# QuantumLiquids/PEPS

Measured on NVIDIA B200. Metric: vmc_samples_per_s, higher is better.
Workload: dtype f64

## Files before the change

### include/peps_b200.h

```cpp
#ifndef PEPS_B200_H
#define PEPS_B200_H
#include <stddef.h>
#include <stdint.h>

#ifdef __cplusplus
extern "C" {
#endif

typedef struct peps_ctx peps_ctx;

typedef struct {
  int32_t rows, cols;
  int32_t phys;
  int32_t D;
  int32_t walkers;
  int32_t device;
  int32_t dmin, dmax;
  double trunc_err;
} peps_config;

const char *peps_backend_name(void);

int peps_create(peps_ctx **out, const peps_config *cfg);
void peps_destroy(peps_ctx *ctx);
const char *peps_last_error(peps_ctx *ctx);

size_t peps_tps_size(peps_ctx *ctx);
size_t peps_tps_site_offset(peps_ctx *ctx, int32_t row, int32_t col);
int peps_set_tps(peps_ctx *ctx, const double *host_tps, size_t n);
int peps_get_tps(peps_ctx *ctx, double *host_tps, size_t n);
int peps_set_truncation(peps_ctx *ctx, int32_t dmin, int32_t dmax, double trunc_err);
int peps_set_compress_scheme(peps_ctx *ctx, int32_t scheme, double convergence_tol, int32_t iter_max);
int peps_set_jacobi(peps_ctx *ctx, double tol, int32_t inner_sweeps, int32_t max_sweeps);
int peps_set_deflation(peps_ctx *ctx, double eps);
int peps_set_chain_deflation(peps_ctx *ctx, double eps);
int peps_set_model_xxz(peps_ctx *ctx, double jz, double jxy, double pinning00);
int peps_set_model_j1j2_xxz(peps_ctx *ctx, double jz, double jxy, double jz2, double jxy2, double pinning00);
int peps_set_model_tfim(peps_ctx *ctx, double h);

int peps_set_model_term(peps_ctx *ctx, int32_t kind, int32_t T, const double *diag, const int32_t *target, const double *coef);
int peps_clear_model_terms(peps_ctx *ctx);
int peps_set_bond_pin(peps_ctx *ctx, int32_t site1, int32_t site2, int32_t T, const double *diag, const int32_t *target, const double *coef);

int peps_set_fermion(peps_ctx *ctx, const int32_t *phys_par, const int32_t *leg_par, size_t n_leg_par);

int peps_set_complex(peps_ctx *ctx);
int peps_set_tps_c(peps_ctx *ctx, const double *re, const double *im, size_t n);
int peps_get_planar(peps_ctx *ctx, int32_t what, double *re, double *im);

int peps_set_jastrow(peps_ctx *ctx, const double *v, const int32_t *density);
int peps_clear_jastrow(peps_ctx *ctx);

int peps_set_configs(peps_ctx *ctx, const int32_t *cfg);
int peps_get_configs(peps_ctx *ctx, int32_t *cfg);
int peps_seed_rng(peps_ctx *ctx, const uint32_t *seeds);
int peps_set_rng_state(peps_ctx *ctx, const uint32_t *mt, const int32_t *idx);
int peps_get_rng_state(peps_ctx *ctx, uint32_t *mt, int32_t *idx);

int peps_init_walkers(peps_ctx *ctx);
int peps_get_amplitudes(peps_ctx *ctx, double *amp);
int peps_normalize_state_order1(peps_ctx *ctx, double max_abs_override, double *site_factor_out);

int peps_sweep(peps_ctx *ctx, int32_t nsweeps, double *accept_rates);
int peps_sweep_full_space(peps_ctx *ctx, int32_t nsweeps, double *accept_rates);
int peps_sweep_three_site(peps_ctx *ctx, int32_t nsweeps, double *accept_rates);
int peps_set_updater(peps_ctx *ctx, int32_t kind);
int peps_energy_and_holes(peps_ctx *ctx, int32_t calc_holes, double *eloc, double *psi_list);
int peps_measure(peps_ctx *ctx, double *energy, double *e_h, double *e_v, double *e_dr, double *e_ur, double *row_corr);
int peps_measure_bond_term(peps_ctx *ctx, int32_t T, const double *diag, const int32_t *target, const double *coef, double *out_h, double *out_v);
int peps_measure_site_term(peps_ctx *ctx, int32_t T, const double *diag, const int32_t *target, const double *coef, double *out);
int64_t peps_structure_factor_pairs(peps_ctx *ctx);
int peps_measure_structure_factor(peps_ctx *ctx, double *out);
size_t peps_holes_stride(peps_ctx *ctx);
int peps_get_holes(peps_ctx *ctx, double *holes);

int peps_zero_accumulators(peps_ctx *ctx);
int peps_accumulate_ostar(peps_ctx *ctx);
int peps_get_accumulators(peps_ctx *ctx, double *ostar_sum, double *eloc_ostar_sum, size_t n);
double *peps_ostar_sum_device(peps_ctx *ctx);
double *peps_eloc_ostar_sum_device(peps_ctx *ctx);
int peps_sample(peps_ctx *ctx, int32_t sweeps_between_samples, double *eloc, double *accept_rates);

int peps_sr_reserve(peps_ctx *ctx, int64_t max_walker_samples);
int peps_sr_collect(peps_ctx *ctx, int32_t on);
int peps_sr_clear(peps_ctx *ctx);
int64_t peps_sr_count(peps_ctx *ctx);
int peps_sr_matvec(peps_ctx *ctx, const double *v_host, double mean_dot_v, double *out_host, size_t n);
int peps_sr_matvec_device(peps_ctx *ctx, const double *v_dev, double mean_dot_v, double *out_dev);
int peps_sr_matvec_c(peps_ctx *ctx, const double *v_host, double mean_dot_v_re, double mean_dot_v_im, double *out_host, size_t n);

typedef int (*peps_allreduce_fn)(void *user, double *device_buf, size_t n);
typedef struct {
  int32_t max_iter;
  double relative_tolerance, absolute_tolerance;
  int32_t residual_recompute_interval;
  double orthogonality_threshold;
} peps_cg_params;
int peps_sr_natural_gradient(peps_ctx *ctx, const double *gradient, const double *ostar_mean, int64_t total_samples,
                             double diag_shift, const peps_cg_params *params, const double *init_guess,
                             peps_allreduce_fn allreduce, void *user, double *x_out, int32_t *iterations,
                             double *residual_norm, int32_t *reason);

int peps_sr_minsr_natural_gradient(peps_ctx *ctx, int64_t total_samples, double diag_shift, double *x_out, double *energy_mean_out);
int peps_sr_minsr_tmatrix(peps_ctx *ctx, double *t_out, size_t n);
int peps_sr_minsr_gram_diag(peps_ctx *ctx, double *g_out, size_t n);

int peps_probe_trace_row(peps_ctx *ctx, int32_t row, double *psi);
int peps_probe_tnn_trace(peps_ctx *ctx, int32_t row, int32_t col, int32_t orient, const int32_t *cfg3, double *psi);
int peps_probe_plaquette_trace(peps_ctx *ctx, int32_t kind, int32_t row, int32_t col, int32_t dir, int32_t orient, double *psi);
int32_t peps_bmps_stack_size(peps_ctx *ctx, int32_t position);
int peps_get_bmps_tensor(peps_ctx *ctx, int32_t position, int32_t k, int32_t i, double *out, int32_t dims[3]);
int64_t peps_stat(peps_ctx *ctx, int32_t which);
int peps_profile_enable(peps_ctx *ctx, int32_t on);
int peps_profile_get(peps_ctx *ctx, double *ms, int64_t *launches, double *flops, int32_t reset);
int peps_sync(peps_ctx *ctx);
void *peps_stream(peps_ctx *ctx);

int peps_test_qr_r(int32_t device, int32_t W, int32_t m, int32_t n, const double *a, double *r_out);
int peps_test_truncate(int32_t device, int32_t W, int32_t nr, int32_t nc, int32_t dmin, int32_t dmax, double trunc_err,
                       const double *theta, double *b_out, int32_t *kept_out, int32_t *sweeps_out);
int peps_test_einsum(int32_t device, int32_t W, const char *spec, const int32_t *dims_a, int32_t rank_a,
                     const int32_t *dims_b, int32_t rank_b, const double *a, const double *b, double *c);

#ifdef __cplusplus
}
#endif
#endif
```

### peps_b200/_lib.py

```python
import ctypes as C
import os

HERE = os.path.dirname(os.path.abspath(__file__))
LIB_PATH = os.path.join(HERE, "libpeps_b200.so")


class PepsConfig(C.Structure):
    _fields_ = [("rows", C.c_int32), ("cols", C.c_int32), ("phys", C.c_int32), ("D", C.c_int32),
                ("walkers", C.c_int32), ("device", C.c_int32), ("dmin", C.c_int32), ("dmax", C.c_int32),
                ("trunc_err", C.c_double)]


class PepsCGParams(C.Structure):
    _fields_ = [("max_iter", C.c_int32), ("relative_tolerance", C.c_double), ("absolute_tolerance", C.c_double),
                ("residual_recompute_interval", C.c_int32), ("orthogonality_threshold", C.c_double)]


ALLREDUCE_FN = C.CFUNCTYPE(C.c_int, C.c_void_p, C.c_void_p, C.c_size_t)

_P = C.c_void_p
_D = C.POINTER(C.c_double)
_I = C.POINTER(C.c_int32)
_U = C.POINTER(C.c_uint32)

SIGNATURES = {
    "peps_backend_name": (C.c_char_p, []),
    "peps_create": (C.c_int, [C.POINTER(_P), C.POINTER(PepsConfig)]),
    "peps_destroy": (None, [_P]),
    "peps_last_error": (C.c_char_p, [_P]),
    "peps_tps_size": (C.c_size_t, [_P]),
    "peps_tps_site_offset": (C.c_size_t, [_P, C.c_int32, C.c_int32]),
    "peps_set_tps": (C.c_int, [_P, _D, C.c_size_t]),
    "peps_get_tps": (C.c_int, [_P, _D, C.c_size_t]),
    "peps_set_truncation": (C.c_int, [_P, C.c_int32, C.c_int32, C.c_double]),
    "peps_set_compress_scheme": (C.c_int, [_P, C.c_int32, C.c_double, C.c_int32]),
    "peps_set_jacobi": (C.c_int, [_P, C.c_double, C.c_int32, C.c_int32]),
    "peps_set_deflation": (C.c_int, [_P, C.c_double]),
    "peps_set_model_xxz": (C.c_int, [_P, C.c_double, C.c_double, C.c_double]),
    "peps_set_chain_deflation": (C.c_int, [_P, C.c_double]),
    "peps_set_model_j1j2_xxz": (C.c_int, [_P, C.c_double, C.c_double, C.c_double, C.c_double, C.c_double]),
    "peps_set_model_term": (C.c_int, [_P, C.c_int32, C.c_int32, _D, _I, _D]),
    "peps_clear_model_terms": (C.c_int, [_P]),
    "peps_set_bond_pin": (C.c_int, [_P, C.c_int32, C.c_int32, C.c_int32, _D, _I, _D]),
    "peps_measure_bond_term": (C.c_int, [_P, C.c_int32, _D, _I, _D, _D, _D]),
    "peps_measure_site_term": (C.c_int, [_P, C.c_int32, _D, _I, _D, _D]),
    "peps_set_fermion": (C.c_int, [_P, _I, _I, C.c_size_t]),
    "peps_set_jastrow": (C.c_int, [_P, _D, _I]),
    "peps_set_complex": (C.c_int, [_P]),
    "peps_set_tps_c": (C.c_int, [_P, _D, _D, C.c_size_t]),
    "peps_get_planar": (C.c_int, [_P, C.c_int32, _D, _D]),
    "peps_clear_jastrow": (C.c_int, [_P]),
    "peps_set_configs": (C.c_int, [_P, _I]),
    "peps_get_configs": (C.c_int, [_P, _I]),
    "peps_seed_rng": (C.c_int, [_P, _U]),
    "peps_set_rng_state": (C.c_int, [_P, _U, _I]),
    "peps_get_rng_state": (C.c_int, [_P, _U, _I]),
    "peps_init_walkers": (C.c_int, [_P]),
    "peps_get_amplitudes": (C.c_int, [_P, _D]),
    "peps_normalize_state_order1": (C.c_int, [_P, C.c_double, _D]),
    "peps_sweep": (C.c_int, [_P, C.c_int32, _D]),
    "peps_sweep_full_space": (C.c_int, [_P, C.c_int32, _D]),
    "peps_sweep_three_site": (C.c_int, [_P, C.c_int32, _D]),
    "peps_measure": (C.c_int, [_P, _D, _D, _D, _D, _D, _D]),
    "peps_set_updater": (C.c_int, [_P, C.c_int32]),
    "peps_set_model_tfim": (C.c_int, [_P, C.c_double]),
    "peps_energy_and_holes": (C.c_int, [_P, C.c_int32, _D, _D]),
    "peps_structure_factor_pairs": (C.c_int64, [_P]),
    "peps_measure_structure_factor": (C.c_int, [_P, _D]),
    "peps_holes_stride": (C.c_size_t, [_P]),
    "peps_get_holes": (C.c_int, [_P, _D]),
    "peps_zero_accumulators": (C.c_int, [_P]),
    "peps_accumulate_ostar": (C.c_int, [_P]),
    "peps_get_accumulators": (C.c_int, [_P, _D, _D, C.c_size_t]),
    "peps_ostar_sum_device": (C.c_void_p, [_P]),
    "peps_eloc_ostar_sum_device": (C.c_void_p, [_P]),
    "peps_sample": (C.c_int, [_P, C.c_int32, _D, _D]),
    "peps_sr_reserve": (C.c_int, [_P, C.c_int64]),
    "peps_sr_collect": (C.c_int, [_P, C.c_int32]),
    "peps_sr_clear": (C.c_int, [_P]),
    "peps_sr_count": (C.c_int64, [_P]),
    "peps_sr_matvec": (C.c_int, [_P, _D, C.c_double, _D, C.c_size_t]),
    "peps_sr_matvec_device": (C.c_int, [_P, C.c_void_p, C.c_double, C.c_void_p]),
    "peps_sr_matvec_c": (C.c_int, [_P, _D, C.c_double, C.c_double, _D, C.c_size_t]),
    "peps_sr_natural_gradient": (C.c_int, [_P, _D, _D, C.c_int64, C.c_double, C.POINTER(PepsCGParams), _D, ALLREDUCE_FN,
                                           C.c_void_p, _D, C.POINTER(C.c_int32), _D, C.POINTER(C.c_int32)]),
    "peps_sr_minsr_natural_gradient": (C.c_int, [_P, C.c_int64, C.c_double, _D, _D]),
    "peps_sr_minsr_tmatrix": (C.c_int, [_P, _D, C.c_size_t]),
    "peps_sr_minsr_gram_diag": (C.c_int, [_P, _D, C.c_size_t]),
    "peps_probe_trace_row": (C.c_int, [_P, C.c_int32, _D]),
    "peps_probe_tnn_trace": (C.c_int, [_P, C.c_int32, C.c_int32, C.c_int32, _I, _D]),
    "peps_probe_plaquette_trace": (C.c_int, [_P, C.c_int32, C.c_int32, C.c_int32, C.c_int32, C.c_int32, _D]),
    "peps_bmps_stack_size": (C.c_int32, [_P, C.c_int32]),
    "peps_get_bmps_tensor": (C.c_int, [_P, C.c_int32, C.c_int32, C.c_int32, _D, _I]),
    "peps_stat": (C.c_int64, [_P, C.c_int32]),
    "peps_sync": (C.c_int, [_P]),
    "peps_profile_enable": (C.c_int, [_P, C.c_int32]),
    "peps_profile_get": (C.c_int, [_P, _D, C.POINTER(C.c_int64), _D, C.c_int32]),
    "peps_stream": (C.c_void_p, [_P]),
    "peps_test_qr_r": (C.c_int, [C.c_int32, C.c_int32, C.c_int32, C.c_int32, _D, _D]),
    "peps_test_truncate": (C.c_int, [C.c_int32, C.c_int32, C.c_int32, C.c_int32, C.c_int32, C.c_int32, C.c_double,
                                     _D, _D, _I, _I]),
    "peps_test_einsum": (C.c_int, [C.c_int32, C.c_int32, C.c_char_p, _I, C.c_int32, _I, C.c_int32, _D, _D, _D]),
}


def bind(path):
    lib = C.CDLL(path)
    for name, (res, args) in SIGNATURES.items():
        fn = getattr(lib, name)
        fn.restype = res
        fn.argtypes = args
    return lib


_lib = None


def load():
    global _lib
    if _lib is None:
        if not os.path.exists(LIB_PATH):
            from . import build as _build
            _build.build_cuda()
        _lib = bind(LIB_PATH)
    return _lib
```

### peps_b200/csrc/backend.h

```cpp
#pragma once
#include <cstddef>
#include <cstdint>

namespace peps {

struct Operand {
  double *p = nullptr;
  long ws = 0;
  long bs = 0;
  const int32_t *gidx = nullptr;
  int gws = 0;
  long gs = 0;
};
inline Operand mkop(double *p, long ws, long bs = 0) {
  Operand o; o.p = p; o.ws = ws; o.bs = bs; return o;
}
inline Operand mkgather(double *p, const int32_t *gidx, int gws, long gs) {
  Operand o; o.p = p; o.gidx = gidx; o.gws = gws; o.gs = gs; return o;
}

struct GettDesc {
  int M = 0, N = 0, K = 0;
  const int32_t *am = nullptr, *ak = nullptr, *bk = nullptr, *bn = nullptr, *cm = nullptr, *cn = nullptr;
  int a_kfast = 0;
  int b_nfast = 1;
  int a_vec2 = 0, b_vec2 = 0, c_vec2 = 0;
  const int32_t *klo_m = nullptr, *klo_n = nullptr;
  double work = 1.0;
  const int32_t *m_cnt = nullptr, *n_cnt = nullptr;
  int m_scale = 0, n_scale = 0;
};

struct BeCtx;
BeCtx *be_ctx_create(int device);
void be_ctx_bind(BeCtx *c);
void be_ctx_destroy(BeCtx *c);
void be_init(int device);
const char *be_name();
void *be_malloc(size_t bytes);
void be_free(void *p);
void be_memset0(void *p, size_t bytes);
void be_h2d(void *dst, const void *src, size_t bytes);
void be_d2h(void *dst, const void *src, size_t bytes);
void be_d2d(void *dst, const void *src, size_t bytes);
void be_sync();
void *be_stream();
long be_launch_count();

enum KernelClass { KC_GETT = 0, KC_DOT, KC_PANEL, KC_JACOBI, KC_SMALL, KC_APPLY, KC_COUNT };
void be_profile_enable(int on);
void be_profile_collect(double *ms, long *launches, double *flops, int reset);

void be_gett(const GettDesc &d, Operand A, Operand B, Operand C, double alpha, double beta, int W, int NB);
void be_dot(int K, const int32_t *ak, const int32_t *bk, Operand A, Operand B, double *out, int W);

void be_fill(double *p, double v, long n);
void be_copy2d(double *dst, long wd, long ldd, const double *src, long ws, long lds, int rows, int cols, int W);
void be_set_identity(double *dst, long wd, int rows, int cols, int W);

struct PanelArgs {
  double *A; long ws; int lda;
  const int32_t *rowtab; int R; int skip0; int NI;
  int col0, pw, nbw;
  double *Vw, *Tw;
  int W;
  const int32_t *row_cnt = nullptr;
  int row_scale = 0;
  const int32_t *stopped = nullptr;
};
void be_panel_qr(const PanelArgs &a);
void be_trailing_check(const double *A, long ws, int lda, int row0, int nrows, int col0, int ncols, const double *colnorm2,
                       const int32_t *colorder, int n, double thresh2, double *acc, int32_t *stopped, int W);

struct TileMap { alignas(64) unsigned char blob[128]; };
bool be_make_tile_map(TileMap *tm, const double *A, long ws, int lda, int rows, int cols, int W, int box_rows, int box_cols);
struct ApplyArgs {
  double *A; long ws; int lda;
  const int32_t *rowtab; int R; int NI;
  int col1, ntrail, nbw;
  const double *Vw, *Tw;
  int W;
  const TileMap *tmap = nullptr;
  int row0 = 0;
  const TileMap *tmap_cols = nullptr;
  int notrans = 0;
  const int32_t *row_cnt = nullptr;
  int row_scale = 0;
  const int32_t *stopped = nullptr;
};
void be_apply_reflector(const ApplyArgs &a);

struct JacobiArgs {
  double *G; long ws; int ld; int nr_pad; int nc; int bs; int nblk; int round;
  double tol; int inner_sweeps; double *offmax; const int32_t *done; int W;
  int nactive = 0;
  const int32_t *bsec = nullptr;
  const int32_t *cwin = nullptr;
};
void be_jacobi_round(const JacobiArgs &a);
void be_jacobi_flags(double *offmax, int32_t *done, double tol, int W);
void be_sector_arrange(const double *src, long ws, int ld, int nc, const int32_t *count, int bs, int nblk, double *dst, long wd,
                       int32_t *bsec, const int32_t *cord_in, int32_t *cord_out, int32_t *cwin, int W);
void be_col_norms2(const double *G, long ws, int ld, int nr, int nc, double *norms2, int W);
void be_permute_cols(const double *src, long ws, int lds, int nr, int nc, const int32_t *order, int gather,
                     double *dst, long wd, int ldd, int W);
void be_row_norms2(const double *G, long ws, int ld, int nr, int nc, double *norms2, int W);
void be_rank_rows(const double *norms2, int nr, double defl2, int32_t *order, int32_t *count, int W);
void be_gather_rows(const double *src, long ws, int ld, int nc, int nr_src, const int32_t *order, const int32_t *count,
                    double *dst, long wd, int nr_dst, int W);
void be_select_truncate(const double *norms2, int nr, int nsv, int dmin, int dmax, double trunc_err, int tcap,
                        int32_t *order, int32_t *kept, int W);
void be_gather_rows_normalized(const double *G, long ws, int ld, int nc, const double *norms2, int nr,
                               const int32_t *order, const int32_t *kept, int tcap, double *B, long wb, int W);

void be_gather_rows_transposed(const double *src, long ws, int ld, int nc, int nr_src, const int32_t *order,
                               const int32_t *count, double *dst, long wd, int n2, int W);
struct SmallSvdArgs {
  const double *Rt; long ws; int ld; int n2; const int32_t *count;
  int nsv, dmin, dmax; double trunc_err; int tcap;
  double tol; int max_sweeps;
  double *out; long wo; int32_t *kept; int32_t *sweeps; int W;
};
constexpr int kSmallSvdMaxN = 128;
void be_svd_small(const SmallSvdArgs &a);
void be_transpose_permute(const double *C0, long wc, int nc, int tcap, const int32_t *order, double *B, long wb, int W);

void be_mt_seed(uint32_t *mt, int32_t *idx, const uint32_t *seeds, int W);
void be_nn_exchange_decide(int32_t *cfg, int nsites, int s1, int s2, const double *psi_b, double *amp,
                           uint32_t *mt, int32_t *idx, int32_t *accepted, int W, const double *jastrow = nullptr);
void be_jastrow_ratio(const int32_t *cfg, int nsites, int s1, int s2, const int32_t *dens, const double *v, double *ratio, int W);
void be_scale(double *x, const double *s, int W);
void be_xxz_bond_energy(const int32_t *cfg, int nsites, int s1, int s2, const double *psi_ex, const double *psi,
                        double jz, double jxy, double *eloc, int W);
void be_ratio_accumulate(const double *psi_ex, const double *psi, double coef, double *eloc, int W);
void be_xxz_onsite_energy(const int32_t *cfg, int nsites, double h00, double *eloc, int W);
void be_term_targets(const int32_t *cfg, int nsites, int s1, int s2, int phys, const int32_t *target, const double *coef, int T,
                     int t, int32_t *idx_a, int32_t *idx_b, double *coefw, int W);
void be_term_accumulate(const int32_t *cfg, int nsites, int s1, int s2, int phys, const double *diag, const double *coefw,
                        const double *psi_ex, const double *psi, double *eloc, int W);

void be_embed_complex(const double *Ar, const double *Ai, long wa, int m, int n, double *M, long wm, int W);
void be_split_r(const double *R, long wr, int rows, int n, double *outr, double *outi, long wo, int W);
void be_complex_basis(double *Bm, long wb, int tcap2, int n, const int32_t *kept2, double *Br, double *Bi, long wo, int tcap,
                      int32_t *keptc, int W);
void be_complex_combine(const double *d0, const double *d1, const double *d2, const double *d3, double *outr, double *outi, int W);
void be_nn_exchange_decide_c(int32_t *cfg, int nsites, int s1, int s2, const double *pbr, const double *pbi, double *ampr,
                             double *ampi, uint32_t *mt, int32_t *idx, int32_t *accepted, int W, const double *jastrow = nullptr);
void be_xxz_bond_energy_c(const int32_t *cfg, int nsites, int s1, int s2, const double *exr, const double *exi, const double *pr,
                          const double *pi, double jz, double jxy, double *er, double *ei, int W);
void be_ratio_accumulate_c(const double *exr, const double *exi, const double *pr, const double *pi, double coef, double *er,
                           double *ei, int W);
void be_term_accumulate_c(const int32_t *cfg, int nsites, int s1, int s2, int phys, const double *diag, const double *coefw,
                          const double *exr, const double *exi, const double *pr, const double *pi, double *er, double *ei, int W);
void be_accumulate_ostar_c(const double *hr, const double *hi, long hole_stride, const int32_t *hole_off, const int32_t *site_size,
                           const int32_t *tps_off, const int32_t *cfg, int nsites, const double *ampr, const double *ampi,
                           const double *er, const double *ei, double *osr, double *osi, double *eor, double *eoi, int W);

constexpr int FERMION_VARIANTS = 8;
void be_fermion_gather(const int32_t *cfg, int rows, int cols, int phys, const int32_t *phys_par, int32_t *gidx_h,
                       int32_t *gidx_v, int32_t *jw_h, int32_t *jw_v, int W);
#if defined(__CUDACC__)
#define PEPS_HD __host__ __device__
#else
#define PEPS_HD
#endif
PEPS_HD inline void fermion_target_one(const int32_t *c, const int32_t *jh, const int32_t *jv, int s1, int s2, int phys,
                                       const int32_t *par, int kind, const int32_t *target, const double *coef, int T, int t,
                                       int32_t &idx_a, int32_t &idx_b, double &coefw) {
  const int c1 = c[s1], c2 = c[s2], p = c1 * phys + c2;
  int tg;
  double cf;
  if (target) { tg = target[p * T + t]; cf = tg < 0 ? 0.0 : coef[p * T + t]; }
  else { tg = c1 != c2 ? c2 * phys + c1 : -1; cf = tg < 0 ? 0.0 : 1.0; }
  const int n1 = tg < 0 ? c1 : tg / phys, n2 = tg < 0 ? c2 : tg % phys;
  const int moved = (par[c1] ^ par[n1]) & (par[c2] ^ par[n2]);
  int va, vb, neg = 0;
  if (kind == 1) { va = 6 + jv[s1]; vb = 6 + (jv[s2] ^ moved); }
  else if (kind == 0 || !moved) { va = jh[s1]; vb = jh[s2] ^ moved; }
  else if (kind == 2) { va = 2 + jh[s1]; vb = jh[s2] ^ 1; neg = jh[s2]; }
  else { va = jh[s1]; vb = 4 + jh[s2]; neg = jh[s1]; }
  idx_a = va * phys + n1;
  idx_b = vb * phys + n2;
  coefw = neg ? -cf : cf;
}
void be_fermion_targets(const int32_t *cfg, int nsites, int s1, int s2, int phys, const int32_t *phys_par,
                        const int32_t *jw_h, const int32_t *jw_v, int kind, const int32_t *target, const double *coef,
                        int T, int t, int32_t *idx_a, int32_t *idx_b, double *coefw, int W);
void be_fermion_finish_holes(double *holes, long hole_stride, const int32_t *hole_off, const int32_t *site_size,
                             const double *gtps, const int64_t *gtps_off, const int32_t *gidx_h, const int32_t *jw_h,
                             int nsites, const double *sign, const double *amp, int W);

void be_fermion_finish_holes_c(double *hr, double *hi, long hole_stride, const int32_t *hole_off, const int32_t *site_size,
                               const double *gtps, long gtps_im_off, const int64_t *gtps_off, const int32_t *gidx_h,
                               const int32_t *jw_h, int nsites, const double *sign, const double *ampr, const double *ampi, int W);

void be_accumulate_ostar(const double *holes, long hole_stride, const int32_t *hole_off, const int32_t *site_size,
                         const int32_t *tps_off, const int32_t *cfg, int nsites, int phys, const double *amp,
                         const double *eloc, double *osum, double *eosum, int W);

void be_sr_store(const double *holes, long hole_stride, const double *amp, const int32_t *cfg, int nsites,
                 double *ostar, int32_t *cfgs, long first, int W);
void be_sr_store_c(const double *hr, const double *hi, long hole_stride, const double *ampr, const double *ampi, const int32_t *cfg,
                   int nsites, double *ostar, int32_t *cfgs, long first, long cap, int W);
void be_sr_dots(const double *ostar, const int32_t *cfgs, long hole_stride, const int32_t *hole_off,
                const int32_t *site_size, const int32_t *tps_off, int nsites, const double *v, double mean_dot_v,
                double *delta, long n);
void be_sr_accumulate(const double *ostar, const int32_t *cfgs, long hole_stride, const int32_t *hole_off,
                      const int32_t *site_size, const int32_t *tps_off, int nsites, int phys, const double *delta,
                      double *out, long n);

void be_sr_gram(const double *left, const double *right, const int32_t *cfgs, long hole_stride, const int32_t *hole_off,
                const int32_t *site_size, const int32_t *site_size_host, int nsites, long n, double lower_sign, double *G);
void be_minsr_centre(const double *G, const double *a, double c, double sign, long n, double scale, double *T);
void be_minsr_embed(const double *Tr, const double *Ti, long n, double shift, double *M);
void be_chol(double *M, long m, int32_t *info);
void be_chol_solve(const double *L, long m, double *b);


void be_vec_lincomb(double *out, double ca, const double *a, double cb, const double *b, long n);
void be_vec_dot(const double *a, const double *b, long n, double *result);

}
```

### peps_b200/csrc/backend_cuda.cu

```cuda
#include <cuda.h>
#include <cuda_runtime.h>
#include <cstdint>
#include <cstdio>
#include <cstdlib>
#include <cmath>
#include <stdexcept>
#include <algorithm>
#include <string>
#include <type_traits>
#include <unordered_map>
#include <map>
#include <mutex>
#include <utility>
#include <vector>
#include "backend.h"

namespace peps {

#define CUDA_CHECK(x)                                                                              \
  do {                                                                                             \
    cudaError_t e_ = (x);                                                                          \
    if (e_ != cudaSuccess)                                                                         \
      throw std::runtime_error(std::string("CUDA error: ") + cudaGetErrorString(e_) + " at " +     \
                               __FILE__ + ":" + std::to_string(__LINE__));                         \
  } while (0)

struct Profiler {
  bool on = false;
  std::vector<std::pair<cudaEvent_t, cudaEvent_t>> pending[KC_COUNT];
  std::vector<cudaEvent_t> pool;
  double ms[KC_COUNT] = {0}, flops[KC_COUNT] = {0};
  long launches[KC_COUNT] = {0};
  cudaEvent_t get() {
    if (!pool.empty()) { cudaEvent_t e = pool.back(); pool.pop_back(); return e; }
    cudaEvent_t e;
    CUDA_CHECK(cudaEventCreate(&e));
    return e;
  }
};
struct BeCtx {
  int device = 0;
  cudaStream_t stream = nullptr;
  long launches = 0;
  Profiler prof;
  double *dot_part = nullptr;
  double *vdot_part = nullptr;
  size_t dot_part_cap = 0;
  double *gram_part = nullptr;
  size_t gram_part_cap = 0;
  int32_t *gram_split = nullptr;
  int gram_split_cap = 0;
};
static thread_local BeCtx *g_cx = nullptr;
static thread_local int g_cur_device = -1;
static inline BeCtx &cx() {
  if (!g_cx) throw std::runtime_error("peps_b200: no backend context bound to this thread");
  return *g_cx;
}
#define g_stream (cx().stream)
#define g_prof (cx().prof)

BeCtx *be_ctx_create(int device) {
  int n = 0;
  cudaError_t e = cudaGetDeviceCount(&n);
  if (e != cudaSuccess || n == 0)
    throw std::runtime_error("peps_b200: no CUDA device available; the product has no CPU fallback");
  if (device < 0 || device >= n) throw std::invalid_argument("peps_b200: CUDA device ordinal out of range");
  CUDA_CHECK(cudaSetDevice(device));
  g_cur_device = device;
  BeCtx *c = new BeCtx();
  c->device = device;
  cudaError_t se = cudaStreamCreateWithFlags(&c->stream, cudaStreamNonBlocking);
  if (se != cudaSuccess) { delete c; throw std::runtime_error(std::string("CUDA error: ") + cudaGetErrorString(se)); }
  return c;
}
void be_ctx_bind(BeCtx *c) {
  if (c && g_cur_device != c->device) { CUDA_CHECK(cudaSetDevice(c->device)); g_cur_device = c->device; }
  g_cx = c;
}
void be_ctx_destroy(BeCtx *c) {
  if (!c) return;
  if (g_cur_device != c->device) { cudaSetDevice(c->device); g_cur_device = c->device; }
  cudaStreamSynchronize(c->stream);
  for (int k = 0; k < KC_COUNT; ++k)
    for (auto &pr : c->prof.pending[k]) { cudaEventDestroy(pr.first); cudaEventDestroy(pr.second); }
  for (cudaEvent_t ev : c->prof.pool) cudaEventDestroy(ev);
  if (c->dot_part) cudaFree(c->dot_part);
  if (c->vdot_part) cudaFree(c->vdot_part);
  if (c->gram_part) cudaFree(c->gram_part);
  if (c->gram_split) cudaFree(c->gram_split);
  cudaStreamDestroy(c->stream);
  if (g_cx == c) g_cx = nullptr;
  delete c;
}
void be_init(int device) {
  static thread_local std::unordered_map<int, BeCtx *> defaults;
  auto it = defaults.find(device);
  if (it == defaults.end()) it = defaults.emplace(device, be_ctx_create(device)).first;
  be_ctx_bind(it->second);
}

static inline void post_launch() {
  ++cx().launches;
  cudaError_t e = cudaGetLastError();
  if (e != cudaSuccess) throw std::runtime_error(std::string("kernel launch failed: ") + cudaGetErrorString(e));
}
template <class K>
static inline void ensure_smem(K kern, size_t smem) {
  static std::mutex mu;
  static std::map<std::pair<int, const void *>, size_t> table;
  std::lock_guard<std::mutex> lock(mu);
  size_t &have = table[{cx().device, (const void *)kern}];
  if (smem > have) {
    CUDA_CHECK(cudaFuncSetAttribute(kern, cudaFuncAttributeMaxDynamicSharedMemorySize, (int)smem));
    have = smem;
  }
}

struct LaunchScope {
  int c; cudaEvent_t s = nullptr;
  LaunchScope(int cls, double fl) : c(cls) {
    g_prof.launches[c] += 1;
    g_prof.flops[c] += fl;
    if (g_prof.on) { s = g_prof.get(); cudaEventRecord(s, g_stream); }
  }
  ~LaunchScope() {
    if (s) { cudaEvent_t e = g_prof.get(); cudaEventRecord(e, g_stream); g_prof.pending[c].push_back({s, e}); }
  }
};
void be_profile_enable(int on) { g_prof.on = on != 0; }
void be_profile_collect(double *ms, long *launches, double *flops, int reset) {
  CUDA_CHECK(cudaStreamSynchronize(g_stream));
  for (int c = 0; c < KC_COUNT; ++c) {
    for (auto &pr : g_prof.pending[c]) {
      float t = 0.f;
      cudaEventElapsedTime(&t, pr.first, pr.second);
      g_prof.ms[c] += t;
      g_prof.pool.push_back(pr.first);
      g_prof.pool.push_back(pr.second);
    }
    g_prof.pending[c].clear();
    if (ms) ms[c] = g_prof.ms[c];
    if (launches) launches[c] = g_prof.launches[c];
    if (flops) flops[c] = g_prof.flops[c];
    if (reset) { g_prof.ms[c] = 0; g_prof.launches[c] = 0; g_prof.flops[c] = 0; }
  }
}

const char *be_name() { return "cuda-sm_100a"; }
void *be_malloc(size_t bytes) {
  void *p = nullptr;
  CUDA_CHECK(cudaMalloc(&p, bytes ? bytes : 8));
  return p;
}
// ... 370 lines not shown
          if (beta != 0.0) v1 += beta * (*cq);
          *cq = v1;
        }
      }
    }
  }
}

static inline bool op_aligned2(const Operand &o) {
  return ((reinterpret_cast<uintptr_t>(o.p) & 15) == 0) && ((o.ws & 1) == 0) && ((o.bs & 1) == 0) && (o.gidx == nullptr || (o.gs & 1) == 0);
}

void be_gett(const GettDesc &d, Operand A, Operand B, Operand C, double alpha, double beta, int W, int NB) {
  if (d.M <= 0 || d.N <= 0 || W <= 0 || NB <= 0) return;
  LaunchScope scope(KC_GETT, 2.0 * d.M * d.N * d.K * (double)W * NB * d.work);
  static const bool use_large = []() { const char *e = std::getenv("PEPS_GETT_LARGE"); return e ? std::atoi(e) != 0 : true; }();
  if (use_large && d.M > 32 && d.N > 32 && d.K >= 8) {
    const int avec = d.a_vec2 && op_aligned2(A), bvec = d.b_vec2 && op_aligned2(B), cvec = d.c_vec2 && op_aligned2(C);
    const int tn = (d.N + GL_BN - 1) / GL_BN;
    const long ctas128 = (long)((d.M + 127) / 128) * tn * NB * W;
    const bool half = ctas128 < 2L * 148 || d.M <= 96;
    const int bm = half ? 64 : 128;
    dim3 grid(((d.M + bm - 1) / bm) * tn, NB, W);
    const bool akf = d.a_kfast != 0, bkf = d.b_nfast == 0;
    const size_t smem = gl_smem(bm, akf, bkf);
    auto go = [&](auto kern) {
      ensure_smem(kern, smem);
      kern<<<grid, GL_THREADS, smem, g_stream>>>(d, A, B, C, alpha, beta, avec, bvec, cvec);
    };
    if (half) {
      if (akf && bkf) go(gett_large_kernel<true, true, 2>);
      else if (akf) go(gett_large_kernel<true, false, 2>);
      else if (bkf) go(gett_large_kernel<false, true, 2>);
      else go(gett_large_kernel<false, false, 2>);
    } else {
      if (akf && bkf) go(gett_large_kernel<true, true, 4>);
      else if (akf) go(gett_large_kernel<true, false, 4>);
      else if (bkf) go(gett_large_kernel<false, true, 4>);
      else go(gett_large_kernel<false, false, 4>);
    }
    post_launch();
    return;
  }
  auto launch = [&](auto kern, int BM, int BN) {
    int tiles = ((d.M + BM - 1) / BM) * ((d.N + BN - 1) / BN);
    dim3 grid(tiles, NB, W);
    kern<<<grid, GETT_THREADS, 0, g_stream>>>(d, A, B, C, alpha, beta);
    post_launch();
  };
  if (d.M > 32 && d.N > 32) launch(gett_kernel<4, 4>, 64, 64);
  else if (d.M > 32) launch(gett_kernel<4, 1>, 64, 16);
  else if (d.N > 32) launch(gett_kernel<1, 4>, 64 / 4, 64);
  else launch(gett_kernel<2, 2>, 32, 32);
}

__global__ void dot_kernel(int K, int kchunk, const int32_t *ak, const int32_t *bk, Operand A, Operand B, double *part) {
  const int w = blockIdx.x, sidx = blockIdx.y;
  const double *Ab = operand_base(A, w, 0);
  const double *Bb = operand_base(B, w, 0);
  __shared__ double red[256];
  double s = 0.0;
  const int k1 = min(K, (sidx + 1) * kchunk);
  for (int k = sidx * kchunk + threadIdx.x; k < k1; k += blockDim.x) s += Ab[ak[k]] * Bb[bk[k]];
  red[threadIdx.x] = s;
  __syncthreads();
  for (int h = blockDim.x / 2; h > 0; h >>= 1) {
    if (threadIdx.x < h) red[threadIdx.x] += red[threadIdx.x + h];
    __syncthreads();
  }
  if (threadIdx.x == 0) part[(long)w * gridDim.y + sidx] = red[0];
}
__global__ void dot_finish_kernel(const double *part, int nsplit, double *out, int W) {
  const int w = blockIdx.x * blockDim.x + threadIdx.x;
  if (w >= W) return;
  double s = 0.0;
  for (int i = 0; i < nsplit; ++i) s += part[(long)w * nsplit + i];
  out[w] = s;
}
void be_dot(int K, const int32_t *ak, const int32_t *bk, Operand A, Operand B, double *out, int W) {
  LaunchScope scope(KC_DOT, 2.0 * K * W);
  const int nsplit = std::max(1, std::min(32, K / 4096));
  if (nsplit == 1) {
    dot_kernel<<<dim3(W, 1), 256, 0, g_stream>>>(K, K, ak, bk, A, B, out);
    post_launch();
    return;
  }
  double *&part = cx().dot_part;
  size_t &part_cap = cx().dot_part_cap;
  if ((size_t)W * 32 > part_cap) {
    if (part) { CUDA_CHECK(cudaStreamSynchronize(g_stream)); cudaFree(part); }
    part_cap = (size_t)W * 32;
    CUDA_CHECK(cudaMalloc(&part, sizeof(double) * part_cap));
  }
  const int kchunk = (K + nsplit - 1) / nsplit;
  dot_kernel<<<dim3(W, nsplit), 256, 0, g_stream>>>(K, kchunk, ak, bk, A, B, part);
  ++cx().launches;
  dot_finish_kernel<<<(W + 127) / 128, 128, 0, g_stream>>>(part, nsplit, out, W);
  post_launch();
}

__global__ void fill_kernel(double *p, double v, long n) {
  long i = blockIdx.x * (long)blockDim.x + threadIdx.x;
  long stride = (long)gridDim.x * blockDim.x;
  for (; i < n; i += stride) p[i] = v;
}
void be_fill(double *p, double v, long n) {
  if (n <= 0) return;
  int blocks = (int)((n + 255) / 256 < 148L * 8 ? (n + 255) / 256 : 148L * 8);
  LaunchScope scope(KC_SMALL, 0.0);
  fill_kernel<<<blocks, 256, 0, g_stream>>>(p, v, n);
  post_launch();
}
__global__ void copy2d_kernel(double *dst, long wd, long ldd, const double *src, long ws, long lds, int rows,
                              int cols) {
  const int w = blockIdx.y;
  long n = (long)rows * cols;
  for (long i = blockIdx.x * (long)blockDim.x + threadIdx.x; i < n; i += (long)gridDim.x * blockDim.x) {
    int r = (int)(i / cols), c = (int)(i % cols);
    dst[w * wd + r * ldd + c] = src[w * ws + r * lds + c];
  }
}
void be_copy2d(double *dst, long wd, long ldd, const double *src, long ws, long lds, int rows, int cols, int W) {
  long n = (long)rows * cols;
  if (n <= 0) return;
  int bx = (int)((n + 255) / 256 < 64 ? (n + 255) / 256 : 64);
  LaunchScope scope(KC_SMALL, 0.0);
  copy2d_kernel<<<dim3(bx, W), 256, 0, g_stream>>>(dst, wd, ldd, src, ws, lds, rows, cols);
  post_launch();
}
__global__ void identity_kernel(double *dst, long wd, int rows, int cols) {
  const int w = blockIdx.y;
  long n = (long)rows * cols;
  for (long i = blockIdx.x * (long)blockDim.x + threadIdx.x; i < n; i += (long)gridDim.x * blockDim.x) {
    int r = (int)(i / cols), c = (int)(i % cols);
    dst[w * wd + i] = (r == c) ? 1.0 : 0.0;
  }
}
void be_set_identity(double *dst, long wd, int rows, int cols, int W) {
  long n = (long)rows * cols;
  int bx = (int)((n + 255) / 256 < 64 ? (n + 255) / 256 : 64);
  LaunchScope scope(KC_SMALL, 0.0);
  identity_kernel<<<dim3(bx, W), 256, 0, g_stream>>>(dst, wd, rows, cols);
  post_launch();
}

__device__ __forceinline__ double warp_sum(double v) {
#pragma unroll
  for (int o = 16; o > 0; o >>= 1) v += __shfl_xor_sync(0xffffffffu, v, o);
  return v;
}

constexpr int PQR_THREADS = 256;

__global__ void __launch_bounds__(PQR_THREADS) panel_qr_kernel(PanelArgs a) {
  extern __shared__ double sm[];
  const int it = blockIdx.x, w = blockIdx.y;
  if (a.row_cnt && a.rowtab[(long)it * a.R] >= a.row_cnt[w] * a.row_scale) return;
  if (a.stopped && a.stopped[w]) return;
  const int R = a.R, pw = a.pw, nbw = a.nbw;
  const int skip = (it == 0) ? a.skip0 : 0;
  const int nact = R - skip;
  const int LDP = R + 1;
  double *P = sm;
  double *S = P + (size_t)nbw * LDP;
  double *T = S + nbw * nbw;
  double *tau = T + nbw * nbw;
  double *scal = tau + nbw;
  double *beta = scal + nbw;
  const int t = threadIdx.x, lane = t & 31, warp = t >> 5, nwarp = PQR_THREADS / 32;
  double *Aw = a.A + (long)w * a.ws;
  const int32_t *rows = a.rowtab + (long)it * R;

  for (int e = t; e < nact * pw; e += PQR_THREADS) {
    int r = e / pw, c = e % pw;
    P[c * LDP + r] = Aw[(long)rows[skip + r] * a.lda + a.col0 + c];
  }
  __syncthreads();

  for (int j = 0; j < pw; ++j) {
    double tj = 0.0, sj = 0.0, bj = 0.0;
    if (j < nact) {
      const double *x = P + j * LDP;
      double part = 0.0;
      for (int r = j + 1 + lane; r < nact; r += 32) part += x[r] * x[r];
      double xn2 = warp_sum(part);
      double alpha = x[j];
      bj = alpha;
      if (xn2 > 0.0) {
        double nrm = sqrt(alpha * alpha + xn2);
        bj = (alpha >= 0.0) ? -nrm : nrm;
        tj = (bj - alpha) / bj;
        sj = 1.0 / (alpha - bj);
      }
      if (tj != 0.0) {
        for (int c = j + 1 + warp; c < pw; c += nwarp) {
          double *y = P + c * LDP;
          double pr = 0.0;
          for (int r = j + 1 + lane; r < nact; r += 32) pr += x[r] * y[r];
          double wv = warp_sum(pr) * sj + y[j];
          double f = tj * wv;
          for (int r = j + 1 + lane; r < nact; r += 32) y[r] -= f * sj * x[r];
          if (lane == 0) y[j] -= f;
        }
      }
    }
    if (t == 0) { tau[j] = tj; scal[j] = sj; beta[j] = bj; }
    __syncthreads();
  }

  for (int e = t; e < nbw * nbw; e += PQR_THREADS) {
    int r = e / nbw, c = e % nbw;
    double v = 0.0;
    if (c < pw && r <= c && r < nact) v = (r == c) ? beta[c] : P[c * LDP + r];
    T[e] = v;
  }
  __syncthreads();
  for (int e = t; e < nact * pw; e += PQR_THREADS) {
    int r = e / pw, c = e % pw;
    double v = (r < nbw && r <= c) ? T[r * nbw + c] : 0.0;
    Aw[(long)rows[skip + r] * a.lda + a.col0 + c] = v;
  }
  __syncthreads();
  for (int e = t; e < nact * pw; e += PQR_THREADS) {
    int c = e / nact, r = e % nact;
    double v;
    if (r < c) v = 0.0;
    else if (r == c) v = 1.0;
    else v = P[c * LDP + r] * scal[c];
    P[c * LDP + r] = v;
  }
  __syncthreads();
  for (int pidx = warp; pidx < pw * pw; pidx += nwarp) {
    int ca = pidx / pw, cb = pidx % pw;
    if (ca >= cb) continue;
    const double *x = P + ca * LDP, *y = P + cb * LDP;
    double pr = 0.0;
    for (int r = cb + lane; r < nact; r += 32) pr += x[r] * y[r];
    pr = warp_sum(pr);
    if (lane == 0) S[ca * nbw + cb] = pr;
  }
  __syncthreads();
  for (int e = t; e < nbw * nbw; e += PQR_THREADS) T[e] = 0.0;
  __syncthreads();
  if (warp == 0) {
    for (int j = 0; j < pw; ++j) {
      double tj = tau[j];
      double v = 0.0;
      if (lane < j) {
        for (int b2 = lane; b2 < j; ++b2) v += T[lane * nbw + b2] * S[b2 * nbw + j];
        v *= -tj;
      }
      __syncwarp();
      if (lane < j) T[lane * nbw + j] = v;
      if (lane == j) T[j * nbw + j] = tj;
      __syncwarp();
    }
  }
  __syncthreads();
  double *Vo = a.Vw + ((long)w * a.NI + it) * (long)R * nbw;
  double *To = a.Tw + ((long)w * a.NI + it) * (long)nbw * nbw;
  for (int e = t; e < skip * nbw; e += PQR_THREADS) Vo[e] = 0.0;
  for (int e = t; e < nact * nbw; e += PQR_THREADS) {
    int r = e / nbw, c = e % nbw;
    Vo[(long)(skip + r) * nbw + c] = (c < pw) ? P[c * LDP + r] : 0.0;
  }
  for (int e = t; e < nbw * nbw; e += PQR_THREADS) To[e] = T[e];
}

static size_t panel_smem_bytes(int R, int nbw) {
  return ((size_t)nbw * (R + 1) + 2 * (size_t)nbw * nbw + 3 * nbw) * sizeof(double);
}

#ifdef PEPS_KERNEL_CLOCKS
__device__ long long g_panel_clk[8 + 32 * 8];
#define PANEL_CLK(i) do { if (blockIdx.x == 0 && blockIdx.y == 0 && threadIdx.x == 0) g_panel_clk[i] = clock64(); } while (0)
#define COL_CLK(j, k) do { if (blockIdx.x == 0 && blockIdx.y == 0 && lane == 0) g_panel_clk[8 + (j) * 8 + (k)] = clock64(); } while (0)
#else
#define PANEL_CLK(i) do { } while (0)
#define COL_CLK(j, k) do { } while (0)
#endif
template <int NBW, int RPL, int MINB>
__global__ void __launch_bounds__(PQR_THREADS, MINB) panel_qr_reg_kernel(PanelArgs a) {
  extern __shared__ double sm[];
  PANEL_CLK(0);
  constexpr int CPW = NBW / 8;
  constexpr int LDT = NBW + 1, LDSS = NBW + 1;
  constexpr int RP = RPL * 32;
  const int it = blockIdx.x, w = blockIdx.y;
  if (a.row_cnt && a.rowtab[(long)it * a.R] >= a.row_cnt[w] * a.row_scale) return;
  if (a.stopped && a.stopped[w]) return;
  const int R = a.R, pw = a.pw, nbw = a.nbw;
  const int skip = (it == 0) ? a.skip0 : 0;
  const int nact = R - skip;
  double *vcols = sm;
  double *S = vcols + (size_t)NBW * RP;
  double *Tt = S + NBW * LDSS;
  volatile double *tau_s = Tt + NBW * LDT;
  double *Rd = const_cast<double *>(tau_s) + NBW;
  long *roff = reinterpret_cast<long *>(Rd + NBW);
  volatile int *ready = reinterpret_cast<volatile int *>(roff + RP);
  const int t = threadIdx.x, lane = t & 31, warp = t >> 5;
  double *Aw = a.A + (long)w * a.ws;
  const int32_t *rows = a.rowtab + (long)it * R;
  for (int r = t; r < RP; r += PQR_THREADS) roff[r] = (r < nact) ? (long)rows[skip + r] * a.lda + a.col0 : 0;
  for (int e = t; e < NBW * LDSS; e += PQR_THREADS) S[e] = 0.0;
  for (int e = t; e < NBW * LDT; e += PQR_THREADS) Tt[e] = 0.0;
  if (t < NBW) { tau_s[t] = 0.0; Rd[t] = 0.0; ready[t] = 0; }
  __syncthreads();

  double *stage = vcols;
  constexpr int RPI = 32 / NBW;
  for (int r0 = warp * RPI; r0 < RP; r0 += 8 * RPI) {
    const int r = r0 + lane / NBW, c = lane % NBW;
    double *dstp = stage + (size_t)r * NBW + (c ^ (r & (NBW - 1)));
    if (r < nact && c < pw) {
      const unsigned saddr = (unsigned)__cvta_generic_to_shared(dstp);
      asm volatile("cp.async.ca.shared.global [%0], [%1], 8;\n" ::"r"(saddr), "l"(Aw + roff[r] + c));
    } else {
      *dstp = 0.0;
    }
  }
  asm volatile("cp.async.commit_group;\n" ::);
  asm volatile("cp.async.wait_group 0;\n" ::);
  __syncthreads();
  double P[CPW][RPL];
#pragma unroll
  for (int i = 0; i < RPL; ++i) {
    const int r = lane + 32 * i;
#pragma unroll
    for (int cc = 0; cc < CPW; ++cc) P[cc][i] = stage[(size_t)r * NBW + ((warp + 8 * cc) ^ (r & (NBW - 1)))];
  }
  __syncthreads();

  auto build = [&](int j, auto cj_c) {
    constexpr int CJ = decltype(cj_c)::value;
    double *vb = vcols + (size_t)j * RP;
    double n0 = 0.0, n1 = 0.0, n2 = 0.0, n3 = 0.0, alpha = 0.0;
#pragma unroll
    for (int i = 0; i < RPL; ++i) {
      const double v = P[CJ][i];
      const int r = lane + 32 * i;
      alpha = (r == j) ? v : alpha;
      const double vm = (r > j) ? v : 0.0;
      if ((i & 3) == 0) n0 = fma(vm, vm, n0); else if ((i & 3) == 1) n1 = fma(vm, vm, n1);
      else if ((i & 3) == 2) n2 = fma(vm, vm, n2); else n3 = fma(vm, vm, n3);
    }
    double xn2 = (n0 + n1) + (n2 + n3);
#pragma unroll
    for (int o = 16; o > 0; o >>= 1) {
      xn2 += __shfl_xor_sync(0xffffffffu, xn2, o);
      alpha += __shfl_xor_sync(0xffffffffu, alpha, o);
    }
    COL_CLK(j, 3);
    double bj = alpha, tj = 0.0, sj = 0.0;
    if (xn2 > 0.0) {
      const double s2 = alpha * alpha + xn2;
      const double rs = rsqrt(s2);
      const double nrm = s2 * rs;
      bj = (alpha >= 0.0) ? -nrm : nrm;
      const double inv_b = (alpha >= 0.0) ? -rs : rs;
      tj = 1.0 - alpha * inv_b;
      sj = 1.0 / (alpha - bj);
    }
    COL_CLK(j, 4);
#pragma unroll
    for (int i = 0; i < RPL; ++i) {
      const int r = lane + 32 * i;
      const double pm = P[CJ][i] * sj;
      const double v = (r > j) ? pm : ((r == j) ? 1.0 : 0.0);
      vb[r] = v;
      P[CJ][i] = (r >= j) ? v : P[CJ][i];
    }
    if (lane == 0) { tau_s[j] = tj; Rd[j] = bj; }
    COL_CLK(j, 5);
    __syncwarp();
    __threadfence_block();
    if (lane == 0) ready[j] = 1;
  };
  auto lookahead = [&](int jn, const double (&v)[RPL], double tj, auto cn_c) {
    constexpr int CN = decltype(cn_c)::value;
    double d0 = 0.0, d1 = 0.0, d2 = 0.0, d3 = 0.0;
#pragma unroll
    for (int i = 0; i < RPL; ++i) {
      const double q = v[i] * P[CN][i];
      if ((i & 3) == 0) d0 += q; else if ((i & 3) == 1) d1 += q; else if ((i & 3) == 2) d2 += q; else d3 += q;
    }
    const double f = tj * warp_sum((d0 + d1) + (d2 + d3));
    COL_CLK(jn, 1);
#pragma unroll
    for (int i = 0; i < RPL; ++i) P[CN][i] -= f * v[i];
    COL_CLK(jn, 2);
    build(jn, cn_c);
    COL_CLK(jn, 6);
  };

  PANEL_CLK(1);
  if (warp == 0 && pw > 0) build(0, std::integral_constant<int, 0>{});
  for (int j = 0; j < pw; ++j) {
    while (ready[j] == 0) __nanosleep(40);
    __threadfence_block();
    const double *vb = vcols + (size_t)j * RP;
    const double tj = tau_s[j];
    double v[RPL];
#pragma unroll
    for (int i = 0; i < RPL; ++i) v[i] = vb[lane + 32 * i];
    const int jn = j + 1;
    const bool own_next = (jn < pw) && (warp == (jn & 7));
    if (own_next) {
      COL_CLK(jn, 7);
      switch (jn >> 3) {
        case 0: lookahead(jn, v, tj, std::integral_constant<int, 0>{}); break;
        case 1: if constexpr (CPW > 1) lookahead(jn, v, tj, std::integral_constant<int, 1>{}); break;
        case 2: if constexpr (CPW > 2) lookahead(jn, v, tj, std::integral_constant<int, 2>{}); break;
        default: if constexpr (CPW > 3) lookahead(jn, v, tj, std::integral_constant<int, 3>{}); break;
      }
    }
    double d[CPW][2];
#pragma unroll
    for (int cc = 0; cc < CPW; ++cc) d[cc][0] = d[cc][1] = 0.0;
#pragma unroll
    for (int i = 0; i < RPL; ++i) {
#pragma unroll
      for (int cc = 0; cc < CPW; ++cc) d[cc][i & 1] += v[i] * P[cc][i];
    }
    double dot[CPW];
#pragma unroll
    for (int cc = 0; cc < CPW; ++cc) dot[cc] = d[cc][0] + d[cc][1];
#pragma unroll
    for (int o = 16; o > 0; o >>= 1) {
#pragma unroll
      for (int cc = 0; cc < CPW; ++cc) dot[cc] += __shfl_xor_sync(0xffffffffu, dot[cc], o);
    }
#pragma unroll
    for (int cc = 0; cc < CPW; ++cc) {
      const int c = warp + 8 * cc;
      if (c >= pw || c == j || (own_next && c == jn)) continue;
      if (c > j) {
        const double f = tj * dot[cc];
        if (f != 0.0) {
#pragma unroll
          for (int i = 0; i < RPL; ++i) P[cc][i] -= f * v[i];
        }
      } else if (lane == 0) {
// ... 2 lines not shown
    }
  }
  PANEL_CLK(2);
  __syncthreads();
  PANEL_CLK(3);

  {
    if (warp < NBW / 8 && lane < 8) {
      const int base = warp * 8;
      double trow[8];
#pragma unroll
      for (int j = 0; j < 8; ++j) {
        const double tj = (base + j < pw) ? tau_s[base + j] : 0.0;
        double acc = 0.0;
#pragma unroll
        for (int b2 = 0; b2 < j; ++b2) acc += trow[b2] * S[(base + b2) * LDSS + base + j];
        trow[j] = (j == lane) ? tj : ((j > lane) ? -tj * acc : 0.0);
      }
#pragma unroll
      for (int j = 0; j < 8; ++j) Tt[(base + lane) * LDT + base + j] = trow[j];
    }
    __syncthreads();
    double *X = vcols;
#pragma unroll 1
    for (int bs = 8; bs < NBW; bs *= 2) {
      const int nel = (NBW / (2 * bs)) * bs * bs;
      for (int e = t; e < nel; e += PQR_THREADS) {
        const int m = e / (bs * bs), aa = (e / bs) % bs, c = e % bs, base = m * 2 * bs;
        const double *Sr = S + (base + aa) * LDSS + base + bs, *Tc = Tt + (base + bs) * LDT + base + bs + c;
        double x0 = 0.0, x1 = 0.0;
        int k = 0;
        for (; k + 1 <= c; k += 2) { x0 += Sr[k] * Tc[k * LDT]; x1 += Sr[k + 1] * Tc[(k + 1) * LDT]; }
        if (k <= c) x0 += Sr[k] * Tc[k * LDT];
        X[(base + aa) * LDT + c] = x0 + x1;
      }
      __syncthreads();
      for (int e = t; e < nel; e += PQR_THREADS) {
        const int m = e / (bs * bs), aa = (e / bs) % bs, c = e % bs, base = m * 2 * bs;
        const double *Tr = Tt + (base + aa) * LDT + base, *Xc = X + base * LDT + c;
        double x0 = 0.0, x1 = 0.0;
        int k = aa;
        for (; k + 1 < bs; k += 2) { x0 += Tr[k] * Xc[k * LDT]; x1 += Tr[k + 1] * Xc[(k + 1) * LDT]; }
        if (k < bs) x0 += Tr[k] * Xc[k * LDT];
        Tt[(base + aa) * LDT + base + bs + c] = -(x0 + x1);
      }
      __syncthreads();
    }
  }
  PANEL_CLK(4);
#pragma unroll
  for (int i = 0; i < RPL; ++i) {
    const int r = lane + 32 * i;
#pragma unroll
    for (int cc = 0; cc < CPW; ++cc) stage[(size_t)r * NBW + ((warp + 8 * cc) ^ (r & (NBW - 1)))] = P[cc][i];
  }
  __syncthreads();
  double *Vo = a.Vw + ((long)w * a.NI + it) * (long)R * nbw;
  for (int e = t; e < skip * nbw; e += PQR_THREADS) Vo[e] = 0.0;
  for (int e = t; e < nact * NBW; e += PQR_THREADS) {
    const int r = e / NBW, c = e % NBW;
    const double pv = stage[(size_t)r * NBW + (c ^ (r & (NBW - 1)))];
    Vo[(long)(skip + r) * nbw + c] = (c < pw && r >= c) ? pv : 0.0;
    if (c < pw) Aw[roff[r] + c] = (r < c) ? pv : ((r == c) ? Rd[c] : 0.0);
  }
  double *To = a.Tw + ((long)w * a.NI + it) * (long)nbw * nbw;
  for (int e = t; e < NBW * NBW; e += PQR_THREADS) To[e] = Tt[(e / NBW) * LDT + (e % NBW)];
  PANEL_CLK(5);
}

template <int NBW, int RPL>
static size_t panel_reg_smem_bytes(int nact_max) {
  (void)nact_max;
  return ((size_t)(NBW + 1) * RPL * 32 + 2 * (size_t)NBW * (NBW + 1) + 2 * NBW) * sizeof(double) + NBW * sizeof(int) + 16;
}

void be_panel_qr(const PanelArgs &a) {
  LaunchScope scope(KC_PANEL, 4.0 * a.R * a.pw * a.pw * (double)a.NI * a.W);
  auto launch_reg = [&](auto kern, size_t smem) {
    ensure_smem(kern, smem);
    kern<<<dim3(a.NI, a.W), PQR_THREADS, smem, g_stream>>>(a);
  };
  const int R = a.R;
  if (a.nbw == 32 && R <= 128) launch_reg(panel_qr_reg_kernel<32, 4, 4>, panel_reg_smem_bytes<32, 4>(R));
  else if (a.nbw == 32 && R <= 256) launch_reg(panel_qr_reg_kernel<32, 8, 2>, panel_reg_smem_bytes<32, 8>(R));
  else if (a.nbw == 32 && R <= 512) launch_reg(panel_qr_reg_kernel<32, 16, 1>, panel_reg_smem_bytes<32, 16>(R));
  else if (a.nbw == 32 && R <= 576) launch_reg(panel_qr_reg_kernel<32, 18, 1>, panel_reg_smem_bytes<32, 18>(R));
  else if (a.nbw == 16 && R <= 512) launch_reg(panel_qr_reg_kernel<16, 16, 1>, panel_reg_smem_bytes<16, 16>(R));
  else if (a.nbw == 16 && R <= 1184) launch_reg(panel_qr_reg_kernel<16, 37, 1>, panel_reg_smem_bytes<16, 37>(R));
  else {
    size_t smem = panel_smem_bytes(a.R, a.nbw);
    ensure_smem(panel_qr_kernel, smem);
    panel_qr_kernel<<<dim3(a.NI, a.W), PQR_THREADS, smem, g_stream>>>(a);
  }
  post_launch();
#ifdef PEPS_KERNEL_CLOCKS
  static const int dbg = std::getenv("PEPS_PANEL_CLK") ? std::atoi(std::getenv("PEPS_PANEL_CLK")) : 0;
  static int shown = 0;
  if (dbg && a.nbw == 32 && R > 256 && R <= 512 && shown < dbg) {
    ++shown;
    long long h[8 + 32 * 8];
    CUDA_CHECK(cudaStreamSynchronize(g_stream));
    CUDA_CHECK(cudaMemcpyFromSymbol(h, g_panel_clk, sizeof(h)));
    if (shown == 1)
      for (int j = 2; j < 32; ++j) {
        const long long *c = h + 8 + j * 8, *pc = h + 8 + (j - 1) * 8;
        fprintf(stderr, "[col %2d] since prev publish: vload=%lld dot+sum=%lld upd=%lld norm=%lld rsq/div=%lld scale+sts=%lld fence=%lld | period=%lld\n",
                j, c[7] - pc[6], c[1] - c[7], c[2] - c[1], c[3] - c[2], c[4] - c[3], c[5] - c[4], c[6] - c[5], c[6] - pc[6]);
      }
    fprintf(stderr, "[panel clk] R=%d pw=%d NI=%d W=%d load=%lld cols=%lld wait=%lld T=%lld emit=%lld\n", R, a.pw, a.NI, a.W,
            h[1] - h[0], h[2] - h[1], h[3] - h[2], h[4] - h[3], h[5] - h[4]);
  }
#endif
}

#ifdef PEPS_KERNEL_CLOCKS
__device__ long long g_apply_clk[8];
#define APPLY_CLK(i) do { if (blockIdx.x == gridDim.x - 1 && blockIdx.y == gridDim.y - 1 && blockIdx.z == gridDim.z - 1 && threadIdx.x == 0) g_apply_clk[i] = clock64(); } while (0)
#else
#define APPLY_CLK(i) do { } while (0)
#endif
__device__ __forceinline__ void mbar_init(uint64_t *bar, unsigned count) {
  asm volatile("mbarrier.init.shared::cta.b64 [%0], %1;\n" ::"r"((unsigned)__cvta_generic_to_shared(bar)), "r"(count));
}
__device__ __forceinline__ void mbar_expect_tx(uint64_t *bar, unsigned bytes) {
  asm volatile("mbarrier.arrive.expect_tx.shared::cta.b64 _, [%0], %1;\n" ::"r"((unsigned)__cvta_generic_to_shared(bar)), "r"(bytes) : "memory");
}
__device__ __forceinline__ void mbar_wait(uint64_t *bar, unsigned parity) {
  asm volatile(
      "{\n.reg .pred p;\nWAIT_%=:\n"
      "mbarrier.try_wait.parity.shared::cta.b64 p, [%0], %1;\n"
      "@p bra DONE_%=;\nbra WAIT_%=;\nDONE_%=:\n}\n" ::"r"((unsigned)__cvta_generic_to_shared(bar)), "r"(parity) : "memory");
}
__device__ __forceinline__ void bulk_g2s(void *dst, const void *src, unsigned bytes, uint64_t *bar) {
  asm volatile("cp.async.bulk.shared::cluster.global.mbarrier::complete_tx::bytes [%0], [%1], %2, [%3];\n" ::"r"(
                   (unsigned)__cvta_generic_to_shared(dst)), "l"(src), "r"(bytes), "r"((unsigned)__cvta_generic_to_shared(bar)) : "memory");
}

__device__ __forceinline__ void bulk_s2g(void *dst, const void *src, unsigned bytes) {
  asm volatile("cp.async.bulk.global.shared::cta.bulk_group [%0], [%1], %2;\n" ::"l"(dst), "r"((unsigned)__cvta_generic_to_shared(src)),
               "r"(bytes) : "memory");
}

__device__ __forceinline__ void tma_load_3d(void *dst, const void *tmap, int x, int y, int z, uint64_t *bar) {
  asm volatile("cp.async.bulk.tensor.3d.shared::cluster.global.tile.mbarrier::complete_tx::bytes [%0], [%1, {%2, %3, %4}], [%5];\n" ::"r"(
                   (unsigned)__cvta_generic_to_shared(dst)), "l"(tmap), "r"(x), "r"(y), "r"(z), "r"((unsigned)__cvta_generic_to_shared(bar)) : "memory");
}

template <int NBW, int MINB, bool TM>
__global__ void __launch_bounds__(256, MINB) apply_reflector_kernel(ApplyArgs a, const __grid_constant__ TileMap tm) {
  extern __shared__ __align__(16) double sm[];
  APPLY_CLK(0);
  constexpr int TN = NBW, MT = NBW / 8, NT = NBW / 8, LDC = TN + 4, LDW = TN + 4, NTILE = MT * NT;
  const int ct = blockIdx.x, it = blockIdx.y, w = blockIdx.z;
  if (a.row_cnt && a.rowtab[(long)it * a.R] >= a.row_cnt[w] * a.row_scale) return;
  if (a.stopped && a.stopped[w]) return;
  const int R = a.R, R8 = (R + 7) & ~7, nbw = a.nbw;
  double *Cs = sm;
  auto csi = [&](int r, int c) -> size_t {
    if constexpr (TM) return ((size_t)(c >> 3) * R8 + r) * 8 + (c & 7);
    else return (size_t)r * LDC + c;
  };
  double *part = Cs + (size_t)R8 * LDC;
  double *Wsm = part + 4 * NTILE * 64;
  long *roff = reinterpret_cast<long *>(Wsm + NBW * LDW);
  uint64_t *bars = reinterpret_cast<uint64_t *>(roff + R8);
  const int t = threadIdx.x, lane = t & 31, warp = t >> 5;
  double *Aw = a.A + (long)w * a.ws;
  const int32_t *rows = a.rowtab + (long)it * R;
  const double *V = a.Vw + ((long)w * a.NI + it) * (long)R * nbw;
  const double *Tg = a.Tw + ((long)w * a.NI + it) * (long)nbw * nbw;
  const int cbase = a.col1 + ct * TN;
  const int ncols = min(TN, a.ntrail - ct * TN);
  const int kslice = ((R8 / 8) + 7) & ~7;
  const int k0 = min(R8, warp * kslice), k1 = min(R8, k0 + kslice);
  const bool wide = (((a.lda | cbase | ncols) & 1) == 0) && ((a.ws & 1) == 0) && ((reinterpret_cast<uintptr_t>(a.A) & 15) == 0);

  double tpre[(NBW * NBW + 255) / 256];
#pragma unroll
  for (int u = 0; u < (NBW * NBW + 255) / 256; ++u) tpre[u] = (t + u * 256 < NBW * NBW) ? __ldg(Tg + t + u * 256) : 0.0;

  if (lane == 0) mbar_init(&bars[warp], 1);
  if constexpr (!TM) { for (int r = k0 + lane; r < k1; r += 32) roff[r] = (r < R) ? (long)rows[r] * a.lda + cbase : -1; }
  APPLY_CLK(6);
  asm volatile("fence.mbarrier_init.release.cluster;\n" ::: "memory");
  __syncwarp();
  APPLY_CLK(7);
  if constexpr (TM) {
    if (lane == 0 && k1 > k0) {
      mbar_expect_tx(&bars[warp], (unsigned)((k1 - k0) * NBW * 8));
#pragma unroll
      for (int j = 0; j < NBW / 8; ++j)
        tma_load_3d(Cs + ((size_t)j * R8 + k0) * 8, &tm, cbase + 8 * j, a.row0 + it * R + k0, w, &bars[warp]);
    }
    APPLY_CLK(1);
    if (k1 > k0) mbar_wait(&bars[warp], 0);
  } else if (wide) {
    const int nvalid = max(0, min(k1, R) - k0);
    if (lane == 0) mbar_expect_tx(&bars[warp], (unsigned)(nvalid * ncols * 8));
    __syncwarp();
    for (int r = k0 + lane; r < k1; r += 32) {
      double *dstp = Cs + (size_t)r * LDC;
      if (r < R) {
        bulk_g2s(dstp, Aw + roff[r], (unsigned)(ncols * 8), &bars[warp]);
        for (int c = ncols; c < LDC; ++c) dstp[c] = 0.0;
      } else {
        for (int c = 0; c < LDC; ++c) dstp[c] = 0.0;
      }
    }
    APPLY_CLK(1);
    mbar_wait(&bars[warp], 0);
  } else {
    for (int r = k0; r < k1; ++r) {
      const long o = roff[r];
      double *dstp = Cs + (size_t)r * LDC + lane;
      if (lane < TN) {
        if (o >= 0 && lane < ncols) {
          const unsigned saddr = (unsigned)__cvta_generic_to_shared(dstp);
          asm volatile("cp.async.ca.shared.global [%0], [%1], 8;\n" ::"r"(saddr), "l"(Aw + o + lane));
        } else {
          *dstp = 0.0;
        }
      }
      if (lane < LDC - TN) Cs[(size_t)r * LDC + TN + lane] = 0.0;
    }
    asm volatile("cp.async.commit_group;\n" ::);
    APPLY_CLK(1);
    asm volatile("cp.async.wait_group 0;\n" ::);
  }
  __syncwarp();
  APPLY_CLK(2);

  double *Wraw = part;
  {
    double acc[MT][NT][2];
#pragma unroll
    for (int i = 0; i < MT; ++i)
#pragma unroll
      for (int j = 0; j < NT; ++j) acc[i][j][0] = acc[i][j][1] = 0.0;
#pragma unroll 4
    for (int k = k0; k < k1; k += 4) {
      const int kr = k + (lane & 3);
      double af[MT], bf[NT];
#pragma unroll
      for (int i = 0; i < MT; ++i) af[i] = (kr < R) ? __ldg(V + (long)kr * nbw + i * 8 + (lane >> 2)) : 0.0;
#pragma unroll
      for (int j = 0; j < NT; ++j) bf[j] = Cs[csi(kr, j * 8 + (lane >> 2))];
#pragma unroll
      for (int i = 0; i < MT; ++i)
#pragma unroll
        for (int j = 0; j < NT; ++j) dmma8x8x4(acc[i][j][0], acc[i][j][1], af[i], bf[j]);
    }
    APPLY_CLK(3);
    const int eo = (lane >> 2) * 8 + 2 * (lane & 3);
    if (warp >= 4) {
#pragma unroll
      for (int i = 0; i < MT; ++i)
#pragma unroll
        for (int j = 0; j < NT; ++j) {
          double *g = part + ((size_t)(warp - 4) * NTILE + i * NT + j) * 64 + eo;
          g[0] = acc[i][j][0]; g[1] = acc[i][j][1];
        }
    }
    __syncthreads();
    if (warp < 4) {
#pragma unroll
      for (int i = 0; i < MT; ++i)
#pragma unroll
        for (int j = 0; j < NT; ++j) {
          double *g = part + ((size_t)warp * NTILE + i * NT + j) * 64 + eo;
          acc[i][j][0] += g[0]; acc[i][j][1] += g[1];
        }
      __syncwarp();
#pragma unroll
      for (int i = 0; i < MT; ++i)
#pragma unroll
        for (int j = 0; j < NT; ++j) {
          double *g = part + ((size_t)warp * NTILE + i * NT + j) * 64 + eo;
          g[0] = acc[i][j][0]; g[1] = acc[i][j][1];
        }
    }
    __syncthreads();
    double wv[(NTILE * 64 + 255) / 256];
#pragma unroll
    for (int u = 0; u < (NTILE * 64 + 255) / 256; ++u) {
      const int e = t + u * 256;
      double v = 0.0;
      if (e < NTILE * 64) {
#pragma unroll
        for (int g = 0; g < 4; ++g) v += part[((size_t)g * NTILE + (e >> 6)) * 64 + (e & 63)];
      }
      wv[u] = v;
    }
    __syncthreads();
#pragma unroll
    for (int u = 0; u < (NTILE * 64 + 255) / 256; ++u) {
      const int e = t + u * 256;
      if (e < NTILE * 64) {
        const int tile = e >> 6, rr = (e >> 3) & 7, cc = e & 7;
        Wraw[((tile / NT) * 8 + rr) * LDW + (tile % NT) * 8 + cc] = wv[u];
      }
    }
  }
  {
    double *Tsm = Wraw + NBW * LDW;
#pragma unroll
    for (int u = 0; u < (NBW * NBW + 255) / 256; ++u) {
      const int e = t + u * 256;
      if (e < NBW * NBW) Tsm[(e / NBW) * LDW + (e % NBW)] = tpre[u];
    }
    __syncthreads();
    for (int e = t; e < NBW * TN; e += 256) {
      const int aa = e / TN, c = e % TN;
      double v0 = 0.0, v1 = 0.0;
      if (a.notrans) {
        for (int b2 = aa; b2 < NBW; ++b2) v0 += Tsm[aa * LDW + b2] * Wraw[b2 * LDW + c];
      } else {
        int b2 = 0;
        for (; b2 + 1 <= aa; b2 += 2) {
          v0 += Tsm[b2 * LDW + aa] * Wraw[b2 * LDW + c];
          v1 += Tsm[(b2 + 1) * LDW + aa] * Wraw[(b2 + 1) * LDW + c];
        }
        if (b2 <= aa) v0 += Tsm[b2 * LDW + aa] * Wraw[b2 * LDW + c];
      }
      Wsm[aa * LDW + c] = -(v0 + v1);
    }
    __syncthreads();
  }

  APPLY_CLK(4);
  {
    double bw[NBW / 4][NT];
#pragma unroll
    for (int ks = 0; ks < NBW / 4; ++ks)
#pragma unroll
      for (int j = 0; j < NT; ++j) bw[ks][j] = Wsm[(ks * 4 + (lane & 3)) * LDW + j * 8 + (lane >> 2)];
    double afn[NBW / 4];
    auto fetch = [&](int rt) {
      const int r = rt * 8 + (lane >> 2);
      const double *vt = V + (long)r * nbw + (lane & 3);
#pragma unroll
      for (int ks = 0; ks < NBW / 4; ++ks) afn[ks] = (r < R) ? __ldg(vt + ks * 4) : 0.0;
    };
    if (k0 < k1) fetch(k0 / 8);
    for (int rt = k0 / 8; rt < k1 / 8; ++rt) {
      const int r = rt * 8 + (lane >> 2);
      double af[NBW / 4];
#pragma unroll
      for (int ks = 0; ks < NBW / 4; ++ks) af[ks] = afn[ks];
      if (rt + 1 < k1 / 8) fetch(rt + 1);
      double acc[NT][2];
#pragma unroll
      for (int j = 0; j < NT; ++j) {
        acc[j][0] = Cs[csi(r, j * 8 + 2 * (lane & 3))];
        acc[j][1] = Cs[csi(r, j * 8 + 2 * (lane & 3) + 1)];
      }
#pragma unroll
      for (int ks = 0; ks < NBW / 4; ++ks)
#pragma unroll
        for (int j = 0; j < NT; ++j) dmma8x8x4(acc[j][0], acc[j][1], af[ks], bw[ks][j]);
      if (r < R) {
        double *dst;
        if constexpr (TM) dst = Aw + (long)(a.row0 + it * R + r) * a.lda + cbase; else dst = Aw + roff[r];
#pragma unroll
        for (int j = 0; j < NT; ++j) {
          const int c = j * 8 + 2 * (lane & 3);
          if (wide) {
            if (c < ncols) *reinterpret_cast<double2 *>(dst + c) = make_double2(acc[j][0], acc[j][1]);
          } else {
            if (c < ncols) dst[c] = acc[j][0];
            if (c + 1 < ncols) dst[c + 1] = acc[j][1];
          }
        }
      }
    }
  }
  APPLY_CLK(5);
}

constexpr int AC_LDV = 36, AC_LDT = 36;
static size_t apply_cols_smem_bytes(int R) {
  return ((size_t)R * AC_LDV + 32 * AC_LDT + 8 * ((size_t)R * 8 + 256)) * sizeof(double) + 9 * sizeof(uint64_t);
}
__global__ void __launch_bounds__(256, 1) apply_cols_kernel(ApplyArgs a, const __grid_constant__ TileMap tm, int nchunk, int cper) {
  extern __shared__ __align__(128) double acs[];
  const int R = a.R;
  double *Vs = acs;
  double *Ts = Vs + (size_t)R * AC_LDV;
  double *wbase = Ts + 32 * AC_LDT;
  const int wstride = R * 8 + 256;
  const int t = threadIdx.x, lane = t & 31, warp = t >> 5, fr = lane >> 2, fk = lane & 3;
  double *Cw = wbase + (size_t)warp * wstride;
  double *Ww = Cw + (size_t)R * 8;
  uint64_t *bars = reinterpret_cast<uint64_t *>(wbase + (size_t)8 * wstride);
  const int cs = blockIdx.x, it = blockIdx.y, w = blockIdx.z;
  if (a.row_cnt && a.row0 + it * R >= a.row_cnt[w] * a.row_scale) return;
  if (a.stopped && a.stopped[w]) return;
  const double *V = a.Vw + ((long)w * a.NI + it) * (long)R * 32;
  const double *Tg = a.Tw + ((long)w * a.NI + it) * 1024L;
  double *Aw = a.A + (long)w * a.ws;
  const int row_base = a.row0 + it * R;
  const int c_lo = cs * cper, c_hi = min(nchunk, c_lo + cper);
  if (lane == 0) mbar_init(&bars[warp], 1);
  if (t == 0) mbar_init(&bars[8], 1);
  asm volatile("fence.mbarrier_init.release.cluster;\n" ::: "memory");
  __syncthreads();
  if (t == 0) mbar_expect_tx(&bars[8], (unsigned)(R * 256));
  int chunk = c_lo + warp;
  if (chunk < c_hi && lane == 0) {
    mbar_expect_tx(&bars[warp], (unsigned)(R * 64));
    tma_load_3d(Cw, &tm, a.col1 + 8 * chunk, row_base, w, &bars[warp]);
  }
  __syncthreads();
  for (int r = t; r < R; r += 256) bulk_g2s(Vs + (size_t)r * AC_LDV, V + (long)r * 32, 256u, &bars[8]);
  for (int e = t; e < 1024; e += 256) Ts[(e >> 5) * AC_LDT + (e & 31)] = __ldg(Tg + e);
  __syncthreads();
  mbar_wait(&bars[8], 0);
  unsigned ph = 0;
  for (; chunk < c_hi; chunk += 8) {
    mbar_wait(&bars[warp], ph);
    ph ^= 1;
    double acc[4][2];
#pragma unroll
    for (int i = 0; i < 4; ++i) acc[i][0] = acc[i][1] = 0.0;
#pragma unroll 4
    for (int k = 0; k < R; k += 4) {
      const int kr = k + fk;
      const double bf = Cw[kr * 8 + fr];
      const double *vr = Vs + (size_t)kr * AC_LDV + fr;
#pragma unroll
      for (int i = 0; i < 4; ++i) dmma8x8x4(acc[i][0], acc[i][1], vr[8 * i], bf);
    }
#pragma unroll
    for (int i = 0; i < 4; ++i) *reinterpret_cast<double2 *>(Ww + (i * 8 + fr) * 8 + 2 * fk) = make_double2(acc[i][0], acc[i][1]);
    __syncwarp();
#pragma unroll
    for (int i = 0; i < 4; ++i) acc[i][0] = acc[i][1] = 0.0;
#pragma unroll
    for (int ks = 0; ks < 8; ++ks) {
      const double bf = Ww[(ks * 4 + fk) * 8 + fr];
#pragma unroll
      for (int i = 0; i < 4; ++i) {
        const double af = a.notrans ? Ts[(i * 8 + fr) * AC_LDT + ks * 4 + fk] : Ts[(ks * 4 + fk) * AC_LDT + i * 8 + fr];
        dmma8x8x4(acc[i][0], acc[i][1], af, bf);
      }
    }
    __syncwarp();
#pragma unroll
    for (int i = 0; i < 4; ++i) *reinterpret_cast<double2 *>(Ww + (i * 8 + fr) * 8 + 2 * fk) = make_double2(-acc[i][0], -acc[i][1]);
    __syncwarp();
    double bw[8];
#pragma unroll
    for (int ks = 0; ks < 8; ++ks) bw[ks] = Ww[(ks * 4 + fk) * 8 + fr];
    const int gcol = a.col1 + 8 * chunk + 2 * fk;
    const bool colok = gcol < a.col1 + a.ntrail;
    for (int rt = 0; rt < R / 8; rt += 2) {
      const int r0 = rt * 8 + fr, r1 = r0 + 8;
      double2 c0 = *reinterpret_cast<const double2 *>(Cw + r0 * 8 + 2 * fk);
      double2 c1 = *reinterpret_cast<const double2 *>(Cw + r1 * 8 + 2 * fk);
      const double *v0 = Vs + (size_t)r0 * AC_LDV + fk, *v1 = Vs + (size_t)r1 * AC_LDV + fk;
#pragma unroll
      for (int ks = 0; ks < 8; ++ks) {
        dmma8x8x4(c0.x, c0.y, v0[4 * ks], bw[ks]);
        dmma8x8x4(c1.x, c1.y, v1[4 * ks], bw[ks]);
      }
      if (colok) {
        *reinterpret_cast<double2 *>(Aw + (long)(row_base + r0) * a.lda + gcol) = c0;
        *reinterpret_cast<double2 *>(Aw + (long)(row_base + r1) * a.lda + gcol) = c1;
      }
    }
    __syncwarp();
    if (chunk + 8 < c_hi && lane == 0) {
      asm volatile("fence.proxy.async.shared::cta;\n" ::: "memory");
      mbar_expect_tx(&bars[warp], (unsigned)(R * 64));
      tma_load_3d(Cw, &tm, a.col1 + 8 * (chunk + 8), row_base, w, &bars[warp]);
    }
  }
}

template <int NBW>
static size_t apply_smem_bytes(int R) {
  int R8 = (R + 7) & ~7;
  return ((size_t)R8 * (NBW + 4) + 4 * (size_t)(NBW / 8) * (NBW / 8) * 64 + (size_t)NBW * (NBW + 4) + (size_t)R8 + 8) * sizeof(double);
}
bool be_make_tile_map(TileMap *tm, const double *A, long ws, int lda, int rows, int cols, int W, int box_rows, int box_cols) {
  typedef CUresult (*EncodeFn)(CUtensorMap *, CUtensorMapDataType, cuuint32_t, void *, const cuuint64_t *, const cuuint64_t *,
                               const cuuint32_t *, const cuuint32_t *, CUtensorMapInterleave, CUtensorMapSwizzle,
                               CUtensorMapL2promotion, CUtensorMapFloatOOBfill);
  static EncodeFn encode = []() -> EncodeFn {
    if (const char *e = std::getenv("PEPS_TILE_MAPS")) if (std::atoi(e) == 0) return nullptr;
    void *fn = nullptr;
    cudaDriverEntryPointQueryResult q;
    if (cudaGetDriverEntryPoint("cuTensorMapEncodeTiled", &fn, cudaEnableDefault, &q) != cudaSuccess || q != cudaDriverEntryPointSuccess) return nullptr;
    return (EncodeFn)fn;
  }();
  static_assert(sizeof(CUtensorMap) <= sizeof(TileMap), "TileMap too small");
  if (!encode) return false;
  if ((lda & 1) || (ws & 1) || (reinterpret_cast<uintptr_t>(A) & 15) || box_rows < 1 || box_rows > 256 || box_cols < 2 ||
      box_cols > 256 || (box_cols & 1))
    return false;
  cuuint64_t gdim[3] = {(cuuint64_t)cols, (cuuint64_t)rows, (cuuint64_t)W};
  cuuint64_t gstr[2] = {(cuuint64_t)lda * 8, (cuuint64_t)ws * 8};
  cuuint32_t box[3] = {(cuuint32_t)box_cols, (cuuint32_t)box_rows, 1};
  cuuint32_t estr[3] = {1, 1, 1};
  CUresult rc = encode(reinterpret_cast<CUtensorMap *>(tm), CU_TENSOR_MAP_DATA_TYPE_FLOAT64, 3, const_cast<double *>(A), gdim, gstr, box, estr,
                       CU_TENSOR_MAP_INTERLEAVE_NONE, CU_TENSOR_MAP_SWIZZLE_NONE, CU_TENSOR_MAP_L2_PROMOTION_NONE,
                       CU_TENSOR_MAP_FLOAT_OOB_FILL_NONE);
  return rc == CUDA_SUCCESS;
}

void be_apply_reflector(const ApplyArgs &a) {
  if (a.ntrail <= 0) return;
  LaunchScope scope(KC_APPLY, 4.0 * a.R * a.nbw * (double)a.ntrail * a.NI * a.W);
  static const TileMap no_map{};
  static const bool use_cols = []() { const char *e = std::getenv("PEPS_APPLY_COLS"); return e ? std::atoi(e) != 0 : true; }();
  if (use_cols && a.tmap_cols != nullptr && a.nbw == 32 && a.R <= 256 && a.R % 16 == 0 && (a.col1 & 1) == 0 && (a.lda & 1) == 0) {
    const int nchunk = (a.ntrail + 7) / 8;
    const int csplit = std::max(1, std::min(8, (nchunk + 12) / 24));
    const int cper = (nchunk + csplit - 1) / csplit;
    const size_t smem = apply_cols_smem_bytes(a.R);
    ensure_smem(apply_cols_kernel, smem);
    apply_cols_kernel<<<dim3((nchunk + cper - 1) / cper, a.NI, a.W), 256, smem, g_stream>>>(a, *a.tmap_cols, nchunk, cper);
    post_launch();
    return;
  }
  auto launch = [&](auto kern, size_t smem, int tn, const TileMap &tmap) {
    ensure_smem(kern, smem);
    kern<<<dim3((a.ntrail + tn - 1) / tn, a.NI, a.W), 256, smem, g_stream>>>(a, tmap);
  };
  const bool tile = a.tmap != nullptr && a.nbw == 32 && a.R % 64 == 0 && (a.col1 & 1) == 0;
  const bool small = apply_smem_bytes<32>(a.R) <= 112 * 1024;
  if (a.nbw == 32 && tile && small) launch(apply_reflector_kernel<32, 2, true>, apply_smem_bytes<32>(a.R), 32, *a.tmap);
  else if (a.nbw == 32 && tile) launch(apply_reflector_kernel<32, 1, true>, apply_smem_bytes<32>(a.R), 32, *a.tmap);
  else if (a.nbw == 32 && small) launch(apply_reflector_kernel<32, 2, false>, apply_smem_bytes<32>(a.R), 32, no_map);
  else if (a.nbw == 32) launch(apply_reflector_kernel<32, 1, false>, apply_smem_bytes<32>(a.R), 32, no_map);
  else if (a.nbw == 16) launch(apply_reflector_kernel<16, 1, false>, apply_smem_bytes<16>(a.R), 16, no_map);
  else if (a.nbw == 8) launch(apply_reflector_kernel<8, 1, false>, apply_smem_bytes<8>(a.R), 8, no_map);
  else throw std::runtime_error("be_apply_reflector: unsupported panel width");
  post_launch();
#ifdef PEPS_KERNEL_CLOCKS
  static const int dbg = std::getenv("PEPS_APPLY_CLK") ? std::atoi(std::getenv("PEPS_APPLY_CLK")) : 0;
  static int shown = 0;
  if (dbg && a.nbw == 32 && a.R == 512 && a.ntrail >= 256 && shown < dbg) {
    ++shown;
    long long h[8];
    CUDA_CHECK(cudaStreamSynchronize(g_stream));
    CUDA_CHECK(cudaMemcpyFromSymbol(h, g_apply_clk, sizeof(h)));
    fprintf(stderr, "[apply clk] R=%d ntrail=%d NI=%d W=%d roff=%lld fence=%lld issue=%lld wait=%lld A=%lld reduce+T=%lld C=%lld\n", a.R, a.ntrail, a.NI, a.W,
            h[6] - h[0], h[7] - h[6], h[1] - h[7], h[2] - h[1], h[3] - h[2], h[4] - h[3], h[5] - h[4]);
  }
#endif
}

__global__ void trailing_norm_kernel(const double *A, long ws, int lda, int row0, int nrows, int col0, int ncols, double *acc,
                                     const int32_t *stopped) {
  const int w = blockIdx.y;
  if (stopped[w]) return;
  const double *Aw = A + (long)w * ws;
  const int lane = threadIdx.x & 31, warp = threadIdx.x >> 5, nwarp = blockDim.x >> 5;
  double s0 = 0.0, s1 = 0.0;
  for (int r = row0 + blockIdx.x * nwarp + warp; r < nrows; r += gridDim.x * nwarp) {
    const double *x = Aw + (long)r * lda;
    int c = col0 + lane;
    for (; c + 32 < ncols; c += 64) { const double a = x[c], b = x[c + 32]; s0 = fma(a, a, s0); s1 = fma(b, b, s1); }
    if (c < ncols) { const double a = x[c]; s0 = fma(a, a, s0); }
  }
  double s = warp_sum(s0 + s1);
  __shared__ double red[8];
  if (lane == 0) red[warp] = s;
  __syncthreads();
  if (threadIdx.x == 0) {
    double t = 0.0;
    for (int i = 0; i < nwarp; ++i) t += red[i];
    if (t != 0.0) atomicAdd(acc + w, t);
  }
}
__global__ void trailing_decide_kernel(const double *colnorm2, const int32_t *colorder, int n, double thresh2, double *acc,
                                       int32_t *stopped, int W) {
  const int w = blockIdx.x * blockDim.x + threadIdx.x;
  if (w >= W || stopped[w]) return;
  stopped[w] = (acc[w] <= thresh2 * colnorm2[(long)w * n + colorder[(long)w * n]]) ? 1 : 0;
  acc[w] = 0.0;
}
void be_trailing_check(const double *A, long ws, int lda, int row0, int nrows, int col0, int ncols, const double *colnorm2,
                       const int32_t *colorder, int n, double thresh2, double *acc, int32_t *stopped, int W) {
  if (nrows <= row0 || ncols <= col0) return;
  LaunchScope scope(KC_SMALL, 0.0);
  const int bx = std::max(1, std::min(16, (nrows - row0 + 63) / 64));
  trailing_norm_kernel<<<dim3(bx, W), 256, 0, g_stream>>>(A, ws, lda, row0, nrows, col0, ncols, acc, stopped);
  ++cx().launches;
  trailing_decide_kernel<<<(W + 127) / 128, 128, 0, g_stream>>>(colnorm2, colorder, n, thresh2, acc, stopped, W);
  post_launch();
}

constexpr int JAC_THREADS = 256;
constexpr int JAC_KGROUPS = 4;

__host__ __device__ __forceinline__ void rr_pair(int nblk, int round, int q, int &I, int &J) {
  const int n1 = nblk - 1;
  if (q == 0) { I = n1; J = round % n1; }
  else { I = (round + q) % n1; J = (round - q + n1) % n1; }
}

__device__ __forceinline__ void jacobi_cs(double app, double aqq, double apq, double tol2, double &c, double &s) {
  const double d = aqq - app, b2 = 2.0 * apq;
  const double m = fmax(fabs(d), fabs(b2));
  const int ex = ((__double2hiint(m) >> 20) & 0x7ff) - 1023;
  const double scale = __hiloint2double((1023 - ex) << 20, 0);
  const float df = (float)(d * scale), bf = (float)(b2 * scale);
  float rf;
  asm("sqrt.approx.ftz.f32 %0, %1;" : "=f"(rf) : "f"(fmaf(df, df, bf * bf)));
  float tf = __fdividef(bf, fabsf(df) + rf);
  tf = (df >= 0.0f) ? tf : -tf;
  float yf;
  asm("rsqrt.approx.ftz.f32 %0, %1;" : "=f"(yf) : "f"(fmaf(tf, tf, 1.0f)));
  const double t = (double)tf;
  const double hx = -0.5 * fma(t, t, 1.0);
  double y = (double)yf;
  y = y * fma(hx, y * y, 1.5);
  y = y * fma(hx, y * y, 1.5);
  const bool rot = (apq * apq > tol2 * fabs(app * aqq)) && (apq != 0.0);
  c = rot ? y : 1.0;
  s = rot ? y * t : 0.0;
}

__device__ __forceinline__ int jac_mu(int s, int NP) {
  if (s == 0) return 0;
  if (s < NP - 1) return s + 1;
  if (s == NP - 1) return 2 * NP - 1;
  if (s == NP) return 1;
  return s - 1;
}
__device__ __forceinline__ int jac_mu_inv(int s, int NP) {
  if (s == 0) return 0;
  if (s == 1) return NP;
  if (s < NP) return s - 1;
  if (s < 2 * NP - 1) return s + 1;
  return NP - 1;
}

#ifdef PEPS_KERNEL_CLOCKS
__device__ long long g_jac_clk[32];
#define JAC_CLK(i) do { if (blockIdx.x == gridDim.x - 1 && blockIdx.y == gridDim.y - 1 && threadIdx.x == 0) g_jac_clk[i] = clock64(); } while (0)
#define JAC_CLK_T(tid, i) do { if (blockIdx.x == gridDim.x - 1 && blockIdx.y == gridDim.y - 1 && threadIdx.x == (tid)) g_jac_clk[i] = clock64(); } while (0)
#else
#define JAC_CLK(i) do { } while (0)
#define JAC_CLK_T(tid, i) do { } while (0)
#endif
template <int N2>
__global__ void __launch_bounds__(JAC_THREADS) jacobi_round_kernel(JacobiArgs a) {
  extern __shared__ __align__(16) double sm[];
  JAC_CLK(0);
  constexpr int T2 = N2 / 8;
  constexpr int NT = T2 * (T2 + 1) / 2;
  constexpr int LG = N2 + 1;
  constexpr int NP = N2 / 2;
  constexpr int bs = N2 / 2;
  const int w = blockIdx.y;
  if (a.done[w]) return;
  const int LDS = ((a.nc + 7) & ~7) + 4;
  double *Ps = sm;
  double *Gpart = Ps + (size_t)N2 * LDS;
  double *Gm = Gpart + JAC_KGROUPS * NT * 64;
  double *Wm = Gm + 2 * N2 * LG;
  double *coef = Wm + 2 * N2 * LG;
  int *perm = (int *)(coef + 4 * N2);
  __shared__ double red[JAC_THREADS / 32];
  __shared__ int tile_p[NT], tile_q[NT];
  const int t = threadIdx.x, lane = t & 31, warp = t >> 5, nwarp = JAC_THREADS / 32;

  int I, J;
  rr_pair(a.nblk, a.round, blockIdx.x, I, J);
  int c0 = 0, nc = a.nc;
  if (a.bsec) {
    const int sI = a.bsec[(long)w * a.nblk + I], sJ = a.bsec[(long)w * a.nblk + J];
    if (sI != sJ || sI == 2) return;
    if (a.cwin) {
      c0 = a.cwin[(long)w * 4 + 2 * sI]; nc = a.cwin[(long)w * 4 + 2 * sI + 1];
      if (nc <= 0) return;
    }
  }
  const int ncp = (nc + 7) & ~7;
  const int lo = min(I, J), hi = max(I, J);
  double *Gw = a.G + (long)w * a.ws + c0;
  const double tol2 = a.tol * a.tol;

  if (t < NT) {
    int idx = 0;
    for (int p = 0; p < T2; ++p)
      for (int q = p; q < T2; ++q) { if (idx == t) { tile_p[t] = p; tile_q[t] = q; } ++idx; }
  }
  JAC_CLK(1);
  const bool wide = ((nc & 1) == 0) && ((c0 & 1) == 0) && ((a.ld & 1) == 0) && ((a.ws & 1) == 0) && ((reinterpret_cast<uintptr_t>(a.G) & 15) == 0);
  __shared__ uint64_t ld_bar;
  if (wide) {
    if (t == 0) {
      mbar_init(&ld_bar, 1);
      asm volatile("fence.mbarrier_init.release.cluster;\n" ::: "memory");
      mbar_expect_tx(&ld_bar, (unsigned)(N2 * nc * 8));
    }
    __syncthreads();
    if (t < N2) {
      const int grow = (t < bs) ? lo * bs + t : hi * bs + (t - bs);
      bulk_g2s(Ps + (size_t)t * LDS, Gw + (long)grow * a.ld, (unsigned)(nc * 8), &ld_bar);
    }
    for (int e = t; e < N2 * (LDS - nc); e += JAC_THREADS) Ps[(size_t)(e / (LDS - nc)) * LDS + nc + e % (LDS - nc)] = 0.0;
    mbar_wait(&ld_bar, 0);
  } else {
    for (int r = warp; r < N2; r += nwarp) {
      const int grow = (r < bs) ? lo * bs + r : hi * bs + (r - bs);
      for (int c = lane; c < LDS; c += 32) Ps[(size_t)r * LDS + c] = (c < nc) ? Gw[(long)grow * a.ld + c] : 0.0;
    }
  }
  __syncthreads();
  JAC_CLK(2);

  {
    const int kg = warp >> 1, half = warp & 1;
    const int kq = ((ncp / JAC_KGROUPS) + 3) & ~3;
    const int k0 = kg * kq, k1 = min(ncp, k0 + kq);
    constexpr int MAXT = (NT + 1) / 2;
    double acc[MAXT][2];
    const double *ap[MAXT], *bp[MAXT];
#pragma unroll
    for (int i = 0; i < MAXT; ++i) {
      acc[i][0] = acc[i][1] = 0.0;
      int ti = 2 * i + half;
      int tp = (ti < NT) ? tile_p[ti] : 0, tq = (ti < NT) ? tile_q[ti] : 0;
      ap[i] = Ps + (size_t)(tp * 8 + (lane >> 2)) * LDS + (lane & 3);
      bp[i] = Ps + (size_t)(tq * 8 + (lane >> 2)) * LDS + (lane & 3);
    }
    for (int k = k0; k < k1; k += 4) {
#pragma unroll
      for (int i = 0; i < MAXT; ++i)
        if (2 * i + half < NT) dmma8x8x4(acc[i][0], acc[i][1], ap[i][k], bp[i][k]);
    }
#pragma unroll
    for (int i = 0; i < MAXT; ++i) {
      int ti = 2 * i + half;
      if (ti < NT) {
        double *g = Gpart + ((size_t)kg * NT + ti) * 64 + (lane >> 2) * 8 + 2 * (lane & 3);
        g[0] = acc[i][0]; g[1] = acc[i][1];
      }
    }
  }
// ... 1761 lines not shown
```

### peps_b200/csrc/c_api.cpp

```cpp
#include <cmath>
#include <cstring>
#include <memory>
#include <string>
#include <vector>
#include "../../include/peps_b200.h"
#include <cstdio>
#include <cstdlib>
#include <algorithm>
#include "engine.h"

using namespace peps;

struct peps_ctx {
  std::unique_ptr<Engine> eng;
  std::string err;
};
static thread_local std::string g_err;

#define GUARD(ctx, ...)                                    \
  try {                                                    \
    if (ctx) (ctx)->eng->bind();                           \
    __VA_ARGS__;                                           \
    return 0;                                              \
  } catch (const std::exception &e) {                      \
// ... 82 lines not shown
  GUARD(ctx, {
    Engine &e = *ctx->eng;
    double mx = max_abs_override;
    if (!(mx > 0.0)) {
      std::vector<double> a((size_t)e.walkers()), ai((size_t)e.walkers());
      e.get_planar(0, a.data(), ai.data());
      mx = 0.0;
      for (size_t k = 0; k < a.size(); ++k) mx = std::max(mx, std::hypot(a[k], ai[k]));
    }
    if (!(mx > 0.0) || !std::isfinite(mx)) throw std::runtime_error("peps_normalize_state_order1: amplitudes are zero or not finite");
    double scale = 1.0 / mx;
    double f = std::pow(scale, 1.0 / double(e.rows() * e.cols()));
    e.scale_tps(f);
    e.init_walkers();
    if (site_factor_out) *site_factor_out = f;
  })
}

int peps_sweep(peps_ctx *ctx, int32_t n, double *acc) { GUARD(ctx, ctx->eng->sweep(n, acc)) }
int peps_set_updater(peps_ctx *ctx, int32_t kind) { GUARD(ctx, ctx->eng->set_updater(kind)) }
int peps_sweep_three_site(peps_ctx *ctx, int32_t n, double *acc) { GUARD(ctx, ctx->eng->sweep_three_site(n, acc)) }
int peps_sweep_full_space(peps_ctx *ctx, int32_t n, double *acc) { GUARD(ctx, ctx->eng->sweep_full_space(n, acc)) }
int peps_energy_and_holes(peps_ctx *ctx, int32_t calc_holes, double *eloc, double *psi_list) {
  GUARD(ctx, ctx->eng->energy_and_holes(calc_holes != 0, eloc, psi_list))
}
int peps_measure(peps_ctx *ctx, double *energy, double *e_h, double *e_v, double *e_dr, double *e_ur, double *row_corr) {
  GUARD(ctx, ctx->eng->measure(energy, e_h, e_v, e_dr, e_ur, row_corr))
}
int64_t peps_structure_factor_pairs(peps_ctx *ctx) { return ctx->eng->structure_factor_pairs(); }
int peps_measure_bond_term(peps_ctx *ctx, int32_t T, const double *diag, const int32_t *target, const double *coef, double *out_h, double *out_v) {
  GUARD(ctx, ctx->eng->measure_bond_term(T, diag, target, coef, out_h, out_v))
}
int peps_measure_site_term(peps_ctx *ctx, int32_t T, const double *diag, const int32_t *target, const double *coef, double *out) {
  GUARD(ctx, ctx->eng->measure_site_term(T, diag, target, coef, out))
}
int peps_set_bond_pin(peps_ctx *ctx, int32_t site1, int32_t site2, int32_t T, const double *diag, const int32_t *target, const double *coef) {
  GUARD(ctx, ctx->eng->set_bond_pin(site1, site2, T, diag, target, coef))
}
int peps_measure_structure_factor(peps_ctx *ctx, double *out) { GUARD(ctx, ctx->eng->measure_structure_factor(out)) }
size_t peps_holes_stride(peps_ctx *ctx) { return (size_t)ctx->eng->holes_stride(); }
int peps_get_holes(peps_ctx *ctx, double *h) { GUARD(ctx, ctx->eng->get_holes(h)) }
int peps_zero_accumulators(peps_ctx *ctx) { GUARD(ctx, ctx->eng->zero_accumulators()) }
int peps_accumulate_ostar(peps_ctx *ctx) { GUARD(ctx, ctx->eng->accumulate_ostar()) }
int peps_get_accumulators(peps_ctx *ctx, double *o, double *eo, size_t n) {
  GUARD(ctx, { if (n != ctx->eng->tps_size()) throw std::invalid_argument("peps_get_accumulators: size mismatch"); ctx->eng->get_accumulators(o, eo); })
}
double *peps_ostar_sum_device(peps_ctx *ctx) { return ctx->eng->osum_device(); }
double *peps_eloc_ostar_sum_device(peps_ctx *ctx) { return ctx->eng->eosum_device(); }
int peps_sample(peps_ctx *ctx, int32_t sweeps, double *eloc, double *acc) {
  GUARD(ctx, {
    ctx->eng->step_sweep(sweeps, acc);
    ctx->eng->energy_and_holes(true, eloc, nullptr);
    ctx->eng->accumulate_ostar();
  })
}
int peps_sr_reserve(peps_ctx *ctx, int64_t n) { GUARD(ctx, ctx->eng->sr_reserve((long)n)) }
int peps_sr_collect(peps_ctx *ctx, int32_t on) { GUARD(ctx, ctx->eng->sr_collect(on != 0)) }
int peps_sr_clear(peps_ctx *ctx) { GUARD(ctx, ctx->eng->sr_clear()) }
int64_t peps_sr_count(peps_ctx *ctx) { return ctx->eng->sr_count(); }
int peps_sr_matvec(peps_ctx *ctx, const double *v, double mean_dot_v, double *out, size_t n) {
  GUARD(ctx, { if (n != ctx->eng->tps_size()) throw std::invalid_argument("peps_sr_matvec: size mismatch"); ctx->eng->sr_matvec_host(v, mean_dot_v, out); })
}
int peps_sr_matvec_c(peps_ctx *ctx, const double *v, double mean_re, double mean_im, double *out, size_t n) {
  GUARD(ctx, { if (n != 2 * ctx->eng->tps_size()) throw std::invalid_argument("peps_sr_matvec_c: size mismatch (planar vectors of 2 * peps_tps_size() doubles)"); ctx->eng->sr_matvec_host_c(v, mean_re, mean_im, out); })
}
int peps_sr_matvec_device(peps_ctx *ctx, const double *v, double mean_dot_v, double *out) { GUARD(ctx, ctx->eng->sr_matvec_device(v, mean_dot_v, out)) }
int peps_sr_natural_gradient(peps_ctx *ctx, const double *gradient, const double *ostar_mean, int64_t total_samples, double diag_shift,
                             const peps_cg_params *prm, const double *init_guess, peps_allreduce_fn allreduce, void *user, double *x_out,
                             int32_t *iterations, double *residual_norm, int32_t *reason) {
  GUARD(ctx, {
    if (!gradient || !ostar_mean || !x_out) throw std::invalid_argument("peps_sr_natural_gradient: null argument");
    Engine::CGParams p;
    if (prm) { p.max_iter = prm->max_iter; p.rel_tol = prm->relative_tolerance; p.abs_tol = prm->absolute_tolerance;
               p.recompute = prm->residual_recompute_interval; p.ortho = prm->orthogonality_threshold; }
    Engine::CGOutcome o = ctx->eng->sr_natural_gradient(gradient, ostar_mean, (long)total_samples, diag_shift, p, init_guess, allreduce, user, x_out);
    if (iterations) *iterations = o.iterations;
    if (residual_norm) *residual_norm = o.residual_norm;
    if (reason) *reason = o.reason;
  })
}
int peps_sr_minsr_natural_gradient(peps_ctx *ctx, int64_t total_samples, double diag_shift, double *x_out, double *energy_mean_out) {
  GUARD(ctx, {
    if (!x_out) throw std::invalid_argument("peps_sr_minsr_natural_gradient: null x_out");
    ctx->eng->sr_minsr_natural_gradient((long)total_samples, diag_shift, x_out, energy_mean_out);
  })
}
int peps_sr_minsr_tmatrix(peps_ctx *ctx, double *t_out, size_t n) {
  GUARD(ctx, {
    const size_t N = (size_t)ctx->eng->sr_count(), want = N * N * (ctx->eng->is_complex() ? 2 : 1);
    if (n != want) throw std::invalid_argument("peps_sr_minsr_tmatrix: size mismatch (N * N doubles, 2 * N * N in a complex context, N = peps_sr_count)");
    ctx->eng->sr_minsr_tmatrix(t_out, nullptr);
  })
}
int peps_sr_minsr_gram_diag(peps_ctx *ctx, double *g_out, size_t n) {
  GUARD(ctx, {
    if (n != (size_t)ctx->eng->sr_count()) throw std::invalid_argument("peps_sr_minsr_gram_diag: size mismatch (peps_sr_count doubles)");
    ctx->eng->sr_minsr_tmatrix(nullptr, g_out);
  })
}
int peps_probe_trace_row(peps_ctx *ctx, int32_t row, double *psi) { GUARD(ctx, ctx->eng->probe_trace_row(row, psi)) }
int peps_probe_tnn_trace(peps_ctx *ctx, int32_t row, int32_t col, int32_t orient, const int32_t *cfg3, double *psi) {
  GUARD(ctx, {
    const int n = orient == 0 ? ctx->eng->cols() : ctx->eng->rows(), i0 = orient == 0 ? col : row;
    if (orient < 0 || orient > 1 || row < 0 || col < 0 || row >= ctx->eng->rows() || col >= ctx->eng->cols() || i0 + 2 >= n)
      throw std::invalid_argument("peps_probe_tnn_trace: the three sites do not fit the lattice");
    ctx->eng->probe_tnn_trace(row, col, orient, cfg3, psi);
  })
}
int peps_probe_plaquette_trace(peps_ctx *ctx, int32_t kind, int32_t row, int32_t col, int32_t dir, int32_t orient, double *psi) {
  GUARD(ctx, {
    Engine &e = *ctx->eng;
    const int span = kind == 0 ? 2 : 3;
    const int h = orient == 0 ? 2 : span, wd = orient == 0 ? span : 2;
    if (kind < 0 || kind > 1 || dir < 0 || dir > 1 || orient < 0 || orient > 1 || row < 0 || col < 0 || row + h > e.rows() || col + wd > e.cols())
      throw std::invalid_argument("peps_probe_plaquette_trace: the plaquette does not fit the lattice");
    e.probe_plaquette_trace(kind, row, col, dir, orient, psi);
  })
}
int32_t peps_bmps_stack_size(peps_ctx *ctx, int32_t pos) { return ctx->eng->bmps_stack_size(pos); }
int peps_get_bmps_tensor(peps_ctx *ctx, int32_t pos, int32_t k, int32_t i, double *out, int32_t dims[3]) {
  GUARD(ctx, { int d[3]; ctx->eng->bmps_tensor(pos, k, i, out, d); for (int a = 0; a < 3; ++a) dims[a] = d[a]; })
}
int64_t peps_stat(peps_ctx *ctx, int32_t which) { return ctx->eng->stat(which); }
int peps_sync(peps_ctx *ctx) { GUARD(ctx, be_sync()) }
int peps_profile_enable(peps_ctx *ctx, int32_t on) { GUARD(ctx, be_profile_enable(on)) }
int peps_profile_get(peps_ctx *ctx, double *ms, int64_t *launches, double *flops, int32_t reset) {
  GUARD(ctx, {
    long l[KC_COUNT];
    be_profile_collect(ms, l, flops, reset);
    if (launches) for (int c = 0; c < KC_COUNT; ++c) launches[c] = l[c];
  })
}
void *peps_stream(peps_ctx *ctx) {
  try { ctx->eng->bind(); return be_stream(); } catch (...) { return nullptr; }
}

int peps_test_qr_r(int32_t device, int32_t W, int32_t m, int32_t n, const double *a, double *r_out) {
  peps_ctx *nullctx = nullptr;
  GUARD(nullctx, {
    be_init(device);
    Pool pool; Planner planner; LinalgCtx cx;
    cx.W = W; cx.pool = &pool; cx.planner = &planner;
    QRLayout L = qr_layout(m, n);
    double *A = (double *)pool.get(sizeof(double) * (size_t)W * L.m_pad * n);
    be_memset0(A, sizeof(double) * (size_t)W * L.m_pad * n);
    double *tmp = (double *)pool.get(sizeof(double) * (size_t)W * m * n);
    be_h2d(tmp, a, sizeof(double) * (size_t)W * m * n);
    be_copy2d(A, (long)L.m_pad * n, n, tmp, (long)m * n, n, m, n, W);
    caqr(cx, A, (long)L.m_pad * n, m, n, L);
    int kk = std::min(m, n);
    double *R = (double *)pool.get(sizeof(double) * (size_t)W * kk * n);
    be_copy2d(R, (long)kk * n, n, A, (long)L.m_pad * n, n, kk, n, W);
    be_d2h(r_out, R, sizeof(double) * (size_t)W * kk * n);
  })
}

int peps_test_truncate(int32_t device, int32_t W, int32_t nr, int32_t nc, int32_t dmin, int32_t dmax, double trunc_err,
                       const double *theta, double *b_out, int32_t *kept_out, int32_t *sweeps_out) {
  peps_ctx *nullctx = nullptr;
  GUARD(nullctx, {
    be_init(device);
    Pool pool; Planner planner; LinalgCtx cx;
    cx.W = W; cx.pool = &pool; cx.planner = &planner;
    if (const char *e = std::getenv("PEPS_PRESORT_COLS")) cx.presort_columns = std::atoi(e) != 0;
    if (const char *e = std::getenv("PEPS_SMALL_SVD")) cx.small_svd = std::atoi(e) != 0;
    if (const char *e = std::getenv("PEPS_QR_EARLY_STOP")) cx.qr_early_stop = std::atoi(e) != 0;
    if (const char *e = std::getenv("PEPS_Z2_SECTORS")) cx.z2_sectors = std::atoi(e) != 0;
    cx.offmax = (double *)pool.get(sizeof(double) * W);
    cx.done = (int32_t *)pool.get(sizeof(int32_t) * W);
    int brows = truncate_buffer_rows(nr, nc);
    double *G = (double *)pool.get(sizeof(double) * (size_t)W * brows * nc);
    be_memset0(G, sizeof(double) * (size_t)W * brows * nc);
    double *tmp = (double *)pool.get(sizeof(double) * (size_t)W * nr * nc);
    be_h2d(tmp, theta, sizeof(double) * (size_t)W * nr * nc);
    be_copy2d(G, (long)brows * nc, nc, tmp, (long)nr * nc, nc, nr, nc, W);
    int tcap = std::min(dmax, std::min(nr, nc));
    double *B = (double *)pool.get(sizeof(double) * (size_t)W * tcap * nc);
    int32_t *kept = (int32_t *)pool.get(sizeof(int32_t) * W);
    truncate_rows(cx, G, (long)brows * nc, nr, nc, dmin, dmax, trunc_err, tcap, B, (long)tcap * nc, kept);
    be_d2h(b_out, B, sizeof(double) * (size_t)W * tcap * nc);
    be_d2h(kept_out, kept, sizeof(int32_t) * W);
    if (sweeps_out) *sweeps_out = (int32_t)cx.jacobi_sweeps;
  })
}

int peps_test_einsum(int32_t device, int32_t W, const char *spec, const int32_t *dims_a, int32_t rank_a,
                     const int32_t *dims_b, int32_t rank_b, const double *a, const double *b, double *c) {
  peps_ctx *nullctx = nullptr;
  GUARD(nullctx, {
    be_init(device);
    Pool pool; Planner planner;
    int da[6], db[6];
    long na = 1, nb = 1;
    for (int i = 0; i < rank_a; ++i) { da[i] = dims_a[i]; na *= da[i]; }
    for (int i = 0; i < rank_b; ++i) { db[i] = dims_b[i]; nb *= db[i]; }
    const Plan &pl = planner.get(spec, da, rank_a, db, rank_b);
    double *A = (double *)pool.get(sizeof(double) * (size_t)W * na);
    double *Bp = (double *)pool.get(sizeof(double) * (size_t)W * nb);
    double *C = (double *)pool.get(sizeof(double) * (size_t)W * pl.outn);
    be_h2d(A, a, sizeof(double) * (size_t)W * na);
    be_h2d(Bp, b, sizeof(double) * (size_t)W * nb);
    be_gett(pl.d, mkop(A, na), mkop(Bp, nb), mkop(C, pl.outn), 1.0, 0.0, W, 1);
    if (const char *e = std::getenv("PEPS_EINSUM_TIME")) {
      const int reps = std::max(1, std::atoi(e));
      be_profile_enable(1);
      double ms[KC_COUNT]; long ln[KC_COUNT]; double fl[KC_COUNT];
      be_profile_collect(ms, ln, fl, 1);
      for (int r = 0; r < reps; ++r) be_gett(pl.d, mkop(A, na), mkop(Bp, nb), mkop(C, pl.outn), 1.0, 0.0, W, 1);
      be_sync();
      be_profile_collect(ms, ln, fl, 1);
      be_profile_enable(0);
      std::fprintf(stderr, "[einsum] %s W=%d M=%d K=%d N=%d: %.1f us per call, %.2f TFLOP/s\n", spec, W, pl.d.M, pl.d.K, pl.d.N,
                   1e3 * ms[KC_GETT] / reps, fl[KC_GETT] / (ms[KC_GETT] * 1e9));
    }
    be_d2h(c, C, sizeof(double) * (size_t)W * pl.outn);
  })
}

}
```

### peps_b200/csrc/engine.cpp

```cpp
#include "engine.h"
#include <algorithm>
#include <array>
#include <cmath>
#include <complex>
#include <cstdio>
#include <cstdlib>
#include <limits>
#include <type_traits>

namespace peps {

Engine::Engine(const EngineConfig &c)
    : rows_(c.rows), cols_(c.cols), phys_(c.phys), D_(c.D), W_(c.walkers), nsites_(c.rows * c.cols),
      dmin_(c.dmin), dmax_(c.dmax), terr_(c.trunc_err) {
  if (rows_ < 2 || cols_ < 2) throw std::invalid_argument("Engine: lattice must be at least 2x2");
  if (W_ < 1 || phys_ < 1 || D_ < 1) throw std::invalid_argument("Engine: bad sizes");
  bectx_ = be_ctx_create(c.device);
  be_ctx_bind(bectx_);
  row_mod_.assign((size_t)rows_, 1);
  col_mod_.assign((size_t)cols_, 1);
  la_.W = W_; la_.pool = &pool_; la_.planner = &planner_;
  if (const char *e = std::getenv("PEPS_DEFLATION_EPS")) la_.deflation_eps = std::atof(e);
  if (const char *e = std::getenv("PEPS_BMPS_MEMO")) memo_on_ = std::atoi(e) != 0;
  if (const char *e = std::getenv("PEPS_PRESORT_COLS")) la_.presort_columns = std::atoi(e) != 0;
  if (const char *e = std::getenv("PEPS_CHAIN_EPS")) chain_eps_ = std::atof(e);
  if (const char *e = std::getenv("PEPS_SMALL_SVD")) la_.small_svd = std::atoi(e) != 0;
  if (const char *e = std::getenv("PEPS_QR_EARLY_STOP")) la_.qr_early_stop = std::atoi(e) != 0;
  if (const char *e = std::getenv("PEPS_QR_STOP_STRIDE")) la_.qr_stop_stride = std::max(1, std::atoi(e));
  la_.offmax = (double *)be_malloc(sizeof(double) * W_);
  la_.done = (int32_t *)be_malloc(sizeof(int32_t) * W_);
  tps_off_h_.resize((size_t)nsites_);
  site_size_h_.resize((size_t)nsites_);
  site_dims_h_.resize((size_t)nsites_);
  hole_off_h_.resize((size_t)nsites_);
  long off = 0, hoff = 0;
  for (int r = 0; r < rows_; ++r)
    for (int cc = 0; cc < cols_; ++cc) {
      int s = r * cols_ + cc;
      std::array<int, 4> d = {cc == 0 ? 1 : D_, r == rows_ - 1 ? 1 : D_, cc == cols_ - 1 ? 1 : D_, r == 0 ? 1 : D_};
      site_dims_h_[(size_t)s] = d;
      site_size_h_[(size_t)s] = d[0] * d[1] * d[2] * d[3];
      tps_off_h_[(size_t)s] = off;
      hole_off_h_[(size_t)s] = hoff;
      off += (long)phys_ * site_size_h_[(size_t)s];
      hoff += site_size_h_[(size_t)s];
    }
  tps_total_ = off;
  hole_stride_ = hoff;
  tps_ = (double *)be_malloc(sizeof(double) * tps_total_);
  gtps_ = tps_;
  gtps_total_ = tps_total_;
  gtps_off_h_ = tps_off_h_;
  osum_ = (double *)be_malloc(sizeof(double) * tps_total_);
  eosum_ = (double *)be_malloc(sizeof(double) * tps_total_);
  be_memset0(osum_, sizeof(double) * tps_total_);
  be_memset0(eosum_, sizeof(double) * tps_total_);
  std::vector<int32_t> t32((size_t)nsites_), h32((size_t)nsites_);
  for (int s = 0; s < nsites_; ++s) { t32[(size_t)s] = (int32_t)tps_off_h_[(size_t)s]; h32[(size_t)s] = (int32_t)hole_off_h_[(size_t)s]; }
  tps_off_d_ = (int32_t *)be_malloc(sizeof(int32_t) * nsites_);
  site_size_d_ = (int32_t *)be_malloc(sizeof(int32_t) * nsites_);
  hole_off_d_ = (int32_t *)be_malloc(sizeof(int32_t) * nsites_);
  be_h2d(tps_off_d_, t32.data(), sizeof(int32_t) * nsites_);
  be_h2d(site_size_d_, site_size_h_.data(), sizeof(int32_t) * nsites_);
  be_h2d(hole_off_d_, h32.data(), sizeof(int32_t) * nsites_);
  cfg_ = (int32_t *)be_malloc(sizeof(int32_t) * (size_t)W_ * nsites_);
  be_memset0(cfg_, sizeof(int32_t) * (size_t)W_ * nsites_);
  amp_ = (double *)be_malloc(sizeof(double) * W_);
  mt_ = (uint32_t *)be_malloc(sizeof(uint32_t) * (size_t)W_ * 624);
  mtidx_ = (int32_t *)be_malloc(sizeof(int32_t) * W_);
  accepted_ = (int32_t *)be_malloc(sizeof(int32_t) * W_);
  eloc_ = (double *)be_malloc(sizeof(double) * W_);
  psi_tmp_ = (double *)be_malloc(sizeof(double) * W_);
  psi_row_ = (double *)be_malloc(sizeof(double) * W_);
  kept_ = (int32_t *)be_malloc(sizeof(int32_t) * W_);
  holes_ = (double *)be_malloc(sizeof(double) * (size_t)W_ * hole_stride_);
  be_memset0(holes_, sizeof(double) * (size_t)W_ * hole_stride_);
  be_memset0(amp_, sizeof(double) * W_);
  be_memset0(eloc_, sizeof(double) * W_);
  std::vector<uint32_t> seeds((size_t)W_);
  for (int w = 0; w < W_; ++w) seeds[(size_t)w] = 5489u + (uint32_t)w;
  seed_rng(seeds.data());
}

Engine::~Engine() {
  be_ctx_bind(bectx_);
  be_sync();
  for (int p = 0; p < 4; ++p) {
    for (auto &b : bmps_[p]) release(b);
    for (auto &t : bten_[p]) release(t);
    for (auto &t : bten2_[p]) release(t);
  }
  for (void *p : {(void *)tps_, (void *)osum_, (void *)eosum_, (void *)tps_off_d_, (void *)site_size_d_, (void *)hole_off_d_,
                  (void *)cfg_, (void *)amp_, (void *)mt_, (void *)mtidx_, (void *)accepted_, (void *)eloc_, (void *)psi_tmp_,
                  (void *)psi_row_, (void *)kept_, (void *)holes_, (void *)la_.offmax, (void *)la_.done, (void *)sr_ostar_,
                  (void *)sr_cfgs_, (void *)sr_delta_, (void *)sr_eloc_, (void *)psi_list_d_, (void *)term_ia_, (void *)term_ib_, (void *)term_cw_, (void *)idx_const_, (void *)idx_flip_, (void *)psi_alt_, (void *)bond_rec_, (void *)idx_perm_,
                  (void *)(fermion_ ? gtps_ : nullptr), (void *)gtps_off_d_, (void *)gidx_[0], (void *)gidx_[1], (void *)jw_[0],
                  (void *)jw_[1], (void *)phys_par_d_, (void *)fsign_, (void *)psi_loc_, (void *)jastrow_v_, (void *)jr_, (void *)dens_d_, (void *)sr_desc2_, (void *)fs_target_d_, (void *)fs_coef_d_, (void *)site_rec_})
    be_free(p);
  for (auto &t : term_) { be_free(t.diag); be_free(t.target); be_free(t.coef); }
  be_free(pin_.diag); be_free(pin_.target); be_free(pin_.coef);
  pool_.release_all();
  planner_.release_all();
  be_ctx_destroy(bectx_);
}

void Engine::site_dims(int r, int c, int out[4]) const {
  for (int i = 0; i < 4; ++i) out[i] = site_dims_h_[(size_t)(r * cols_ + c)][(size_t)i];
}
void Engine::set_tps(const double *host) {
  be_h2d(tps_, host, sizeof(double) * tps_total_);
  if (complex_) be_memset0(tps_ + tps_total_, sizeof(double) * tps_total_);
  tps_loaded_ = true;
  if (fermion_) {
    dress_plane(host, gtps_);
    if (complex_) be_memset0(gtps_ + gtps_total_, sizeof(double) * gtps_total_);
  }
  touch_all();
}
void Engine::dress_plane(const double *host, double *dst) {
  {
    std::vector<double> g((size_t)(tps_total_ * FERMION_VARIANTS));
    static const int vmask[FERMION_VARIANTS] = {0, 8, 4, 12, 6, 14, 0, 1};
    for (int site = 0; site < nsites_; ++site) {
      const auto &d = site_dims_h_[(size_t)site];
      const int sz = site_size_h_[(size_t)site];
      const std::vector<int32_t> *par = &leg_par_h_[(size_t)site * 4];
      for (int v = 0; v < FERMION_VARIANTS; ++v) {
        const bool vert = v >= 6;
        int e = 0;
        for (int l = 0; l < d[0]; ++l)
          for (int dd = 0; dd < d[1]; ++dd)
            for (int r = 0; r < d[2]; ++r)
              for (int u = 0; u < d[3]; ++u, ++e) {
                const int pl = par[0][(size_t)l], pd = par[1][(size_t)dd], pr = par[2][(size_t)r], pu = par[3][(size_t)u];
                int q = vert ? (pl & pd) ^ (pl & pr) ^ (pl & pu) ^ pl ^ pd : (pl & pd) ^ (pl & pr) ^ (pd & pr) ^ pl ^ pd;
                if (vmask[v] & 1) q ^= pl;
                if (vmask[v] & 2) q ^= pd;
                if (vmask[v] & 4) q ^= pr;
                if (vmask[v] & 8) q ^= pu;
                const double sg = q ? -1.0 : 1.0;
                for (int p = 0; p < phys_; ++p)
                  g[(size_t)(gtps_off_h_[(size_t)site] + ((long)v * phys_ + p) * sz + e)] =
                      sg * host[tps_off_h_[(size_t)site] + (long)p * sz + e];
              }
      }
    }
    be_h2d(dst, g.data(), sizeof(double) * g.size());
  }
}
void Engine::get_tps(double *host) { be_d2h(host, tps_, sizeof(double) * tps_total_); }
void Engine::scale_tps(double f) {
  std::vector<double> h((size_t)tps_total_ * (complex_ ? 2 : 1));
  be_d2h(h.data(), tps_, sizeof(double) * h.size());
  for (auto &x : h) x *= f;
  if (complex_) set_tps_c(h.data(), h.data() + tps_total_);
  else set_tps(h.data());
}
void Engine::set_configs(const int32_t *host) {
  for (size_t i = 0; i < (size_t)W_ * nsites_; ++i)
    if (host[i] < 0 || host[i] >= phys_)
      throw std::invalid_argument("set_configs: entry " + std::to_string(host[i]) + " of walker " + std::to_string(i / nsites_) +
                                  " is outside [0, phys = " + std::to_string(phys_) + ")");
  be_h2d(cfg_, host, sizeof(int32_t) * (size_t)W_ * nsites_);
  refresh_gather();
  touch_all();
}
void Engine::get_configs(int32_t *host) { be_d2h(host, cfg_, sizeof(int32_t) * (size_t)W_ * nsites_); }
void Engine::seed_rng(const uint32_t *seeds) {
  uint32_t *d = (uint32_t *)pool_.get(sizeof(uint32_t) * W_);
  be_h2d(d, seeds, sizeof(uint32_t) * W_);
  be_mt_seed(mt_, mtidx_, d, W_);
  be_sync();
  pool_.put(d);
}
void Engine::set_rng_state(const uint32_t *mt, const int32_t *idx) {
  be_h2d(mt_, mt, sizeof(uint32_t) * (size_t)W_ * 624);
  be_h2d(mtidx_, idx, sizeof(int32_t) * W_);
}
void Engine::get_rng_state(uint32_t *mt, int32_t *idx) {
  be_d2h(mt, mt_, sizeof(uint32_t) * (size_t)W_ * 624);
  be_d2h(idx, mtidx_, sizeof(int32_t) * W_);
// ... 11 lines not shown
    case 6: return be_launch_count();
    case 7: return (long)pool_.total_bytes();
    case 8: return la_.rows_in;
    case 9: return la_.rows_kept;
    case 10: return la_.jacobi_rounds;
    case 11: return n_memo_hits_;
    case 12: return chain_rows_in_;
    case 13: return chain_rows_kept_;
    case 14: return la_.small_svd_calls;
    default: return -1;
  }
}

BT Engine::alloc(std::initializer_list<int> dims) {
  BT t;
  t.rank = (int)dims.size();
  long n = 1;
  int i = 0;
  for (int d : dims) { t.d[i++] = d; n *= d; }
  t.n = n;
  t.p = (double *)pool_.get(sizeof(double) * (size_t)W_ * n * (complex_ ? 2 : 1));
  return t;
}
BT Engine::ones111() {
  BT t = alloc({1, 1, 1});
  be_fill(t.p, 1.0, W_);
  if (complex_) be_memset0(imag(t), sizeof(double) * W_);
  return t;
}
void Engine::release(BT &t) {
  if (t.p) pool_.put(t.p);
  t.p = nullptr;
}
void Engine::release(BMPSv &v) {
  for (auto &t : v) release(t);
  v.clear();
}
TRef Engine::ref(const BT &t) const {
  TRef r;
  r.op = mkop(t.p, t.n);
  if (complex_) r.opi = mkop(imag(t), t.n);
  r.rank = t.rank;
  for (int i = 0; i < t.rank; ++i) r.d[i] = t.d[i];
  return r;
}
TRef Engine::site_ref(int site, int cfg_site) const {
  TRef r;
  if (fermion_ && cfg_site != site) throw std::logic_error("fermion mode: exchanged tensors need explicit dressed slices");
  r.op = mkgather(gtps_ + gtps_off_h_[(size_t)site], (fermion_ ? gidx_[gmode_] : cfg_) + cfg_site, nsites_, site_size_h_[(size_t)site]);
  if (complex_) r.opi = mkgather(gtps_ + gtps_total_ + gtps_off_h_[(size_t)site], (fermion_ ? gidx_[gmode_] : cfg_) + cfg_site, nsites_, site_size_h_[(size_t)site]);
  r.rank = 4;
  for (int i = 0; i < 4; ++i) r.d[i] = site_dims_h_[(size_t)site][(size_t)i];
  return r;
}
template <class H>
static GettDesc with_hints(GettDesc d, const H *h) {
  if (h) {
    d.klo_m = h->klo_m; d.klo_n = h->klo_n; d.work = h->work;
    d.m_cnt = h->m_cnt; d.m_scale = h->m_scale; d.n_cnt = h->n_cnt; d.n_scale = h->n_scale;
  }
  return d;
}
TRef Engine::site_ref_idx(int site, const int32_t *idx, int stride) const {
  TRef r;
  r.op = mkgather(gtps_ + gtps_off_h_[(size_t)site], idx, stride, site_size_h_[(size_t)site]);
  if (complex_) r.opi = mkgather(gtps_ + gtps_total_ + gtps_off_h_[(size_t)site], idx, stride, site_size_h_[(size_t)site]);
  r.rank = 4;
  for (int i = 0; i < 4; ++i) r.d[i] = site_dims_h_[(size_t)site][(size_t)i];
  return r;
}
BT Engine::einsum(const std::string &spec, const TRef &a, const TRef &b, const KHints *h, bool conj_b) {
  const Plan &pl = planner_.get(spec, a.d, a.rank, b.d, b.rank);
  BT out;
  out.rank = (int)pl.outdims.size();
  for (int i = 0; i < out.rank; ++i) out.d[i] = pl.outdims[(size_t)i];
  out.n = pl.outn;
  out.p = (double *)pool_.get(sizeof(double) * (size_t)W_ * out.n * (complex_ ? 2 : 1));
  if (!complex_) {
    be_gett(with_hints(pl.d, h), a.op, b.op, mkop(out.p, out.n), 1.0, 0.0, W_, 1);
    return out;
  }
  const double sb = conj_b ? -1.0 : 1.0;
  const Operand cr = mkop(out.p, out.n), ci = mkop(imag(out), out.n);
  be_gett(pl.d, a.op, b.op, cr, 1.0, 0.0, W_, 1);
  be_gett(pl.d, a.opi, b.opi, cr, -sb, 1.0, W_, 1);
  be_gett(pl.d, a.op, b.opi, ci, sb, 0.0, W_, 1);
  be_gett(pl.d, a.opi, b.op, ci, 1.0, 1.0, W_, 1);
  return out;
}
void Engine::einsum_into(const std::string &spec, const TRef &a, const TRef &b, Operand c, const long *sc, double alpha,
                         double beta, const KHints *h, const Operand *c_im) {
  const Plan &pl = planner_.get(spec, a.d, a.rank, b.d, b.rank, nullptr, nullptr, sc);
  if (!complex_) { be_gett(with_hints(pl.d, h), a.op, b.op, c, alpha, beta, W_, 1); return; }
  if (!c_im || alpha != 1.0 || beta != 0.0) throw std::logic_error("einsum_into: this contraction is not available for complex states");
  be_gett(pl.d, a.op, b.op, c, 1.0, 0.0, W_, 1);
  be_gett(pl.d, a.opi, b.opi, c, -1.0, 1.0, W_, 1);
  be_gett(pl.d, a.op, b.opi, *c_im, 1.0, 0.0, W_, 1);
  be_gett(pl.d, a.opi, b.op, *c_im, 1.0, 1.0, W_, 1);
}
const Engine::KHints &Engine::r_hints(int which, int k, int e, int a, int p, int b) {
  std::array<int, 6> key = {which, k, e, a, p, b};
  auto it = hints_.find(key);
  if (it != hints_.end()) return it->second;
  std::vector<int32_t> tab;
  int K = 0;
  if (which == 0) {
    K = a;
    tab.resize((size_t)e * k);
    for (int ee = 0; ee < e; ++ee)
      for (int kk = 0; kk < k; ++kk) tab[(size_t)kk * e + ee] = std::min(a, std::max(0, kk - ee * a));
  } else if (which == 1) {
    K = e * p;
    tab.resize((size_t)k * b);
    for (int kk = 0; kk < k; ++kk)
      for (int bb = 0; bb < b; ++bb) tab[(size_t)kk * b + bb] = std::min(K, p * (kk / a));
  } else {
    K = e * a;
    tab.resize((size_t)k);
    for (int kk = 0; kk < k; ++kk) tab[(size_t)kk] = std::min(K, kk);
  }
  KHints h;
  const int32_t *dev = planner_.upload(tab);
  double done = 0.0, total = 0.0;
  for (size_t t0 = 0; t0 < tab.size(); t0 += 64) {
    int lo = K;
    for (size_t i = t0; i < std::min(tab.size(), t0 + 64); ++i) lo = std::min(lo, (int)tab[i]);
    done += K - std::min(K, lo / 16 * 16);
    total += K;
  }
  h.work = total > 0 ? done / total : 1.0;
  if (which == 0) h.klo_n = dev; else h.klo_m = dev;
  return hints_.emplace(key, h).first->second;
}
std::string Engine::site_labels(int post, char pre, char toward, char next, char away) {
  std::string s(4, '?');
  s[(size_t)((post + 3) % 4)] = pre;
  s[(size_t)post] = toward;
  s[(size_t)((post + 1) % 4)] = next;
  s[(size_t)((post + 2) % 4)] = away;
  return s;
}
std::vector<int> Engine::slice_sites(int num, int orient) const {
  std::vector<int> v;
  if (orient == HORIZONTAL) for (int c = 0; c < cols_; ++c) v.push_back(num * cols_ + c);
  else for (int r = 0; r < rows_; ++r) v.push_back(r * cols_ + num);
  return v;
}

Engine::BMPSv Engine::absorb(const BMPSv &mps, const std::vector<int> &sites_in, int post) {
  if (scheme_ != 0 && mps.size() > 2) return absorb_variational(mps, sites_in, post, scheme_ == 2);
  return absorb_svd(mps, sites_in, post);
}
template <class Write>
Engine::ChainStep Engine::chain_step(int m_in, int n_in, Write &&write, const int32_t *rc, int o, int rk, double eps,
                                     bool reduce_tall) {
  ChainStep out;
  int m = complex_ ? 2 * m_in : m_in;
  const int n = complex_ ? 2 * n_in : n_in, kk = std::min(m, n);
  QRLayout L;
  if (!reduce_tall || m <= qr_max_rows()) L = qr_layout(m, n);
  else { L.m_pad = m; L.nb = 32; }
  long wsA = (long)L.m_pad * n;
  auto padded = [&] {
    double *p = (double *)pool_.get(sizeof(double) * (size_t)W_ * wsA);
    if (L.m_pad > m) be_memset0(p, sizeof(double) * (size_t)W_ * wsA);
    return p;
  };
  double *A;
  if (!complex_) {
    A = padded();
    write(mkop(A, wsA), nullptr);
  } else {
    const long wa = (long)m_in * n_in;
    double *Ar = (double *)pool_.get(sizeof(double) * (size_t)W_ * wa), *Ai = (double *)pool_.get(sizeof(double) * (size_t)W_ * wa);
    const Operand ci = mkop(Ai, wa);
    write(mkop(Ar, wa), &ci);
    A = padded();
    be_embed_complex(Ar, Ai, wa, m_in, n_in, A, wsA, W_);
    pool_.put(Ar); pool_.put(Ai);
    rc = nullptr; o = 0; rk *= 2;
  }
  auto reduce = [&](double *&Ap) {
    if (!reduce_tall) return;
    while (m > qr_max_rows()) {
      const int nchunk = (m + qr_max_rows() - 1) / qr_max_rows();
      const int chunk = ((m + nchunk - 1) / nchunk + 31) / 32 * 32;
      int stacked = 0;
      for (int c = 0; c * chunk < m; ++c) stacked += std::min(std::min(chunk, m - c * chunk), n);
      QRLayout Ls;
      if (stacked <= qr_max_rows()) Ls = qr_layout(stacked, n);
      else { Ls.m_pad = stacked; Ls.nb = 32; }
      const long wsS = (long)Ls.m_pad * n;
      double *S = (double *)pool_.get(sizeof(double) * (size_t)W_ * wsS);
      be_memset0(S, sizeof(double) * (size_t)W_ * wsS);
      int off = 0;
      for (int c = 0; c * chunk < m; ++c) {
        const int rows_c = std::min(chunk, m - c * chunk), kkc = std::min(rows_c, n);
        QRLayout Lc = qr_layout(rows_c, n);
        const long wsC = (long)Lc.m_pad * n;
        double *buf = (double *)pool_.get(sizeof(double) * (size_t)W_ * wsC);
        if (Lc.m_pad > rows_c) be_memset0(buf, sizeof(double) * (size_t)W_ * wsC);
        be_copy2d(buf, wsC, n, Ap + (long)c * chunk * n, wsA, n, rows_c, n, W_);
        caqr(la_, buf, wsC, rows_c, n, Lc);
        be_copy2d(S + (long)off * n, wsS, n, buf, wsC, n, kkc, n, W_);
        off += kkc;
        pool_.put(buf);
      }
      pool_.put(Ap);
      Ap = S; wsA = wsS; m = stacked; L = Ls; rc = nullptr; o = 0;
    }
  };
  double *R;
  long wsR;
  int rows;
  const bool deflate = eps > 0.0 && kk >= 16;
  if (deflate) {
    double *cn2 = (double *)pool_.get(sizeof(double) * (size_t)W_ * std::max(n, kk));
    int32_t *ord = (int32_t *)pool_.get(sizeof(int32_t) * (size_t)W_ * std::max(n, kk));
    int32_t *cord = (int32_t *)pool_.get(sizeof(int32_t) * (size_t)W_ * n);
    int32_t *cnt = (int32_t *)pool_.get(sizeof(int32_t) * (size_t)W_);
    be_col_norms2(A, wsA, n, m, n, cn2, W_);
    be_rank_rows(cn2, n, 0.0, cord, cnt, W_);
    double *Ap = padded();
    be_permute_cols(A, wsA, n, m, n, cord, 1, Ap, wsA, n, W_);
    pool_.put(A);
    reduce(Ap);
    QRStop st;
    st.colnorm2 = cn2; st.colorder = cord; st.eps = eps; st.first_col = std::max(0, std::min(rk, kk) - 96);
    caqr(la_, Ap, wsA, m, n, L, rc, o, &st);
    be_row_norms2(Ap, wsA, n, kk, n, cn2, W_);
    be_rank_rows(cn2, kk, eps * eps, ord, cnt, W_);
    std::vector<int32_t> ch((size_t)W_);
    be_d2h(ch.data(), cnt, sizeof(int32_t) * W_);
    rows = 1;
    for (int w = 0; w < W_; ++w) rows = std::max(rows, (int)ch[(size_t)w]);
    const int gran = kk >= 128 ? 32 : 8;
    rows = std::min(kk, (rows + gran - 1) / gran * gran);
    chain_rows_in_ += kk; chain_rows_kept_ += rows;
    wsR = (long)rows * n;
    double *Rg = (double *)pool_.get(sizeof(double) * (size_t)W_ * wsR);
    be_gather_rows(Ap, wsA, n, n, kk, ord, cnt, Rg, wsR, rows, W_);
    R = (double *)pool_.get(sizeof(double) * (size_t)W_ * wsR);
    be_permute_cols(Rg, wsR, n, rows, n, cord, 0, R, wsR, n, W_);
    out.cnt = cnt;
    for (void *p : {(void *)cn2, (void *)ord, (void *)cord, (void *)Ap, (void *)Rg}) pool_.put(p);
  } else {
    reduce(A);
    caqr(la_, A, wsA, m, n, L, rc, o);
    R = A; wsR = wsA; rows = kk;
    out.tri = true;
  }
  if (complex_) {
    out.r = alloc({rows, n_in});
    be_split_r(R, wsR, rows, n_in, out.r.p, imag(out.r), out.r.n, W_);
    pool_.put(R);
    if (out.cnt) pool_.put(out.cnt);
    out.cnt = nullptr; out.tri = false;
  } else if (!deflate) {
    out.r = alloc({rows, n});
    be_copy2d(out.r.p, out.r.n, n, R, wsR, n, rows, n, W_);
    pool_.put(R);
  } else {
    out.r.p = R; out.r.rank = 2; out.r.d[0] = rows; out.r.d[1] = n; out.r.n = wsR;
  }
  return out;
}

template <class Theta>
BT Engine::truncated_right_vectors(int rows, int cols, Theta &&theta, int dmin, int dmax, double terr) {
  constexpr bool held = std::is_same<typename std::decay<Theta>::type, BT>::value;
  if (rows >= cols && cols <= dmin) {
    BT B = alloc({cols, cols});
    be_set_identity(B.p, B.n, cols, cols, W_);
    if (complex_) be_memset0(imag(B), sizeof(double) * (size_t)W_ * B.n);
    return B;
  }
  const int tcap = std::min(dmax, std::min(rows, cols));
  BT B = alloc({tcap, cols});
  if (!complex_) {
    const int brows = truncate_buffer_rows(rows, cols);
    const long ws = (long)brows * cols;
    double *G = (double *)pool_.get(sizeof(double) * (size_t)W_ * ws);
    if (brows > rows) be_memset0(G, sizeof(double) * (size_t)W_ * ws);
    if constexpr (held) be_copy2d(G, ws, cols, theta.p, theta.n, cols, rows, cols, W_);
    else theta(mkop(G, ws), nullptr);
    truncate_rows(la_, G, ws, rows, cols, dmin, dmax, terr, tcap, B.p, B.n, kept_);
    pool_.put(G);
    return B;
  }
  double *Tr, *Ti;
  long wt;
  if constexpr (held) {
    Tr = theta.p; Ti = imag(theta); wt = theta.n;
  } else {
    wt = (long)rows * cols;
    Tr = (double *)pool_.get(sizeof(double) * (size_t)W_ * wt); Ti = (double *)pool_.get(sizeof(double) * (size_t)W_ * wt);
    const Operand ci = mkop(Ti, wt);
    theta(mkop(Tr, wt), &ci);
  }
  const int rows2 = 2 * rows, cols2 = 2 * cols;
  const int brows2 = truncate_buffer_rows(rows2, cols2);
  const long ws2 = (long)brows2 * cols2;
  double *GM = (double *)pool_.get(sizeof(double) * (size_t)W_ * ws2);
  if (brows2 > rows2) be_memset0(GM, sizeof(double) * (size_t)W_ * ws2);
  be_embed_complex(Tr, Ti, wt, rows, cols, GM, ws2, W_);
  if constexpr (!held) { pool_.put(Tr); pool_.put(Ti); }
  const int dmax2 = (int)std::min<long>(2L * dmax, std::numeric_limits<int>::max()), dmin2 = (int)std::min<long>(2L * dmin, dmax2);
  const int tcap2 = std::min(dmax2, std::min(rows2, cols2));
  double *Bm = (double *)pool_.get(sizeof(double) * (size_t)W_ * tcap2 * cols2);
  truncate_rows(la_, GM, ws2, rows2, cols2, dmin2, dmax2, terr, tcap2, Bm, (long)tcap2 * cols2, kept_);
  be_complex_basis(Bm, (long)tcap2 * cols2, tcap2, cols, kept_, B.p, imag(B), B.n, tcap, kept_, W_);
  pool_.put(GM); pool_.put(Bm);
  return B;
}

Engine::BMPSv Engine::absorb_svd(const BMPSv &mps, const std::vector<int> &sites_in, int post) {
  ++n_absorb_;
  const int N = (int)mps.size();
  std::vector<int> sites(sites_in);
  if (post == RIGHT || post == UP) std::reverse(sites.begin(), sites.end());
  const std::string sl = site_labels(post, 'e', 'p', 'f', 'o');
  auto sdim = [&](int site, char l) { return site_dims_h_[(size_t)site][sl.find(l)]; };
  std::vector<BT> r((size_t)N);
  std::vector<char> r_tri((size_t)N, 0);
  std::vector<int32_t *> r_cnt((size_t)N, nullptr);
  r[0] = ones111();
  for (int i = 0; i < N - 1; ++i) {
    const int site = sites[(size_t)i];
    TRef sref = tn_site(site);
    const bool tri = r_tri[(size_t)i] != 0;
    const int rk = r[(size_t)i].d[0], re = r[(size_t)i].d[1], ra = r[(size_t)i].d[2];
    const int pd = mps[(size_t)i].d[1], bd = mps[(size_t)i].d[2];
    const int32_t *rc = r_cnt[(size_t)i];
    KHints h1, h2;
    if (tri) { h1 = r_hints(0, rk, re, ra, pd, bd); h2 = r_hints(1, rk, re, ra, pd, bd); }
    if (rc) { h1.n_cnt = rc; h1.n_scale = re; h2.m_cnt = rc; h2.m_scale = bd; }
    BT tmp1 = einsum("apb,kea->kepb", ref(mps[(size_t)i]), ref(r[(size_t)i]), (tri || rc) ? &h1 : nullptr);
    const int k = r[(size_t)i].d[0], o = sdim(site, 'o'), f = sdim(site, 'f'), b = mps[(size_t)i].d[2];
    ChainStep cs = chain_step(k * o, f * b, [&](Operand c, const Operand *c_im) {
      einsum_into("kepb," + sl + "->kofb", ref(tmp1), sref, c, nullptr, 1.0, 0.0, (tri || rc) ? &h2 : nullptr, c_im);
      release(tmp1);
    }, rc, o, rk, chain_eps_, true);
    BT &rn = r[(size_t)i + 1] = cs.r;
    rn.rank = 3; rn.d[1] = f; rn.d[2] = b;
    r_cnt[(size_t)i + 1] = cs.cnt;
    r_tri[(size_t)i + 1] = cs.tri ? 1 : 0;
  }
  BMPSv res((size_t)N);
  BT E = ones111();
  for (int i = N - 1; i >= 1; --i) {
    const int site = sites[(size_t)i];
    BT Y = einsum("apb,fbj->apfj", ref(mps[(size_t)i]), ref(E));
    BT X = einsum("apfj," + sl + "->eaoj", ref(Y), tn_site(site));
    release(Y);
    const bool tri = r_tri[(size_t)i] != 0;
    const int32_t *rc = r_cnt[(size_t)i];
    BT B = truncated_right_vectors(r[(size_t)i].d[0], X.d[2] * X.d[3], [&](Operand c, const Operand *c_im) {
      KHints h3;
      if (tri) h3 = r_hints(2, r[(size_t)i].d[0], r[(size_t)i].d[1], r[(size_t)i].d[2], 0, 0);
      if (rc) { h3.m_cnt = rc; h3.m_scale = 1; }
      einsum_into("kea,eaoj->koj", ref(r[(size_t)i]), ref(X), c, nullptr, 1.0, 0.0, (tri || rc) ? &h3 : nullptr, c_im);
    }, dmin_, dmax_, terr_);
    B.rank = 3; B.d[1] = X.d[2]; B.d[2] = X.d[3];
    BT En = einsum("eaoj,toj->eat", ref(X), ref(B), nullptr, true);
    release(X);
    release(E);
    E = En;
    res[(size_t)i] = B;
  }
  {
    const int site = sites[0];
    BT Y = einsum("apb,fbj->apfj", ref(mps[0]), ref(E));
    BT X = einsum("apfj," + sl + "->eaoj", ref(Y), tn_site(site));
    release(Y);
    release(E);
    BT first = X;
    first.rank = 3;
    first.d[0] = 1; first.d[1] = X.d[2]; first.d[2] = X.d[3];
    res[0] = first;
  }
  for (auto &t : r) release(t);
  for (int32_t *c : r_cnt) if (c) pool_.put(c);
  return res;
}

Engine::BMPSv Engine::compress_mps(const BMPSv &mps, int dmin, int dmax, double terr) {
  const int N = (int)mps.size();
  std::vector<BT> r((size_t)N);
  r[0] = alloc({1, 1});
  be_fill(r[0].p, 1.0, W_);
  if (complex_) be_memset0(imag(r[0]), sizeof(double) * W_);
  for (int i = 0; i < N - 1; ++i) {
    r[(size_t)i + 1] = chain_step(r[(size_t)i].d[0] * mps[(size_t)i].d[1], mps[(size_t)i].d[2], [&](Operand c, const Operand *c_im) {
      einsum_into("ka,apb->kpb", ref(r[(size_t)i]), ref(mps[(size_t)i]), c, nullptr, 1.0, 0.0, nullptr, c_im);
    }, nullptr, 0, 0, 0.0, false).r;
  }
  BMPSv res((size_t)N);
  BT E = alloc({1, 1});
  be_fill(E.p, 1.0, W_);
  if (complex_) be_memset0(imag(E), sizeof(double) * W_);
  for (int i = N - 1; i >= 1; --i) {
    BT X = einsum("apb,bj->apj", ref(mps[(size_t)i]), ref(E));
    BT B = truncated_right_vectors(r[(size_t)i].d[0], X.d[1] * X.d[2], [&](Operand c, const Operand *c_im) {
      einsum_into("ka,apj->kpj", ref(r[(size_t)i]), ref(X), c, nullptr, 1.0, 0.0, nullptr, c_im);
    }, dmin, dmax, terr);
    B.rank = 3; B.d[1] = X.d[1]; B.d[2] = X.d[2];
    BT En = einsum("apj,tpj->at", ref(X), ref(B), nullptr, true);
    release(X); release(E);
    E = En;
    res[(size_t)i] = B;
  }
  res[0] = einsum("apb,bj->apj", ref(mps[0]), ref(E));
  release(E);
  for (auto &t : r) release(t);
  return res;
}
Engine::BMPSv Engine::absorb_variational(const BMPSv &mps, const std::vector<int> &sites_in, int post, bool one_site) {
  const int N = (int)mps.size();
  std::vector<int> sites(sites_in);
  if (post == RIGHT || post == UP) std::reverse(sites.begin(), sites.end());
  const std::string sli = site_labels(post, 'e', 'p', 'f', 'o'), slj = site_labels(post, 'f', 'q', 'g', 'u');
  BMPSv small = compress_mps(mps, 1, 2, 0.0);
  const int dmin0 = dmin_, dmax0 = dmax_; const double terr0 = terr_;
  if (one_site) { dmin_ = dmax_; terr_ = 0.0; }
  BMPSv res = absorb_svd(small, sites_in, post);
  dmin_ = dmin0; dmax_ = dmax0; terr_ = terr0;
  release(small);
  std::vector<BT> lenvs, renvs;
  lenvs.push_back(ones111());
  renvs.push_back(ones111());
  auto right2 = [&](int j, const BT &renv) {
    BT r1 = einsum("bqc,cgj->bqgj", ref(mps[(size_t)j]), ref(renv));
    BT r2 = einsum("bqgj," + slj + "->fbuj", ref(r1), tn_site(sites[(size_t)j]));
    release(r1);
    return r2;
  };
  auto left2 = [&](int i2, const BT &lenv) {
    BT l1 = einsum("kea,apb->kepb", ref(lenv), ref(mps[(size_t)i2]));
    BT l2 = einsum("kepb," + sli + "->kofb", ref(l1), tn_site(sites[(size_t)i2]));
    release(l1);
    return l2;
  };
  for (int i = N - 1; i > 1; --i) {
    BT r2 = right2(i, renvs.back());
    renvs.push_back(einsum("fbuj,tuj->bft", ref(r2), ref(res[(size_t)i]), nullptr, true));
    release(r2);
  }
  auto row_norms2 = [&](const BT &x, int rows, int nc, std::vector<double> &h) {
    double *n2 = (double *)pool_.get(sizeof(double) * (size_t)W_ * rows);
    h.assign((size_t)W_ * rows, 0.0);
    be_row_norms2(x.p, x.n, nc, rows, nc, n2, W_);
    be_d2h(h.data(), n2, sizeof(double) * h.size());
    if (complex_) {
      std::vector<double> hi(h.size());
      be_row_norms2(imag(x), x.n, nc, rows, nc, n2, W_);
      be_d2h(hi.data(), n2, sizeof(double) * hi.size());
      for (size_t q = 0; q < h.size(); ++q) h[q] += hi[q];
    }
    pool_.put(n2);
  };
  std::vector<double> s_last;
  int s_last_t = -1;
  auto sweep_two_site = [&](int d0, int d1, bool track) -> double {
    for (int i = 0; i < N - 2; ++i) {
      BT l2 = left2(i, lenvs.back()), r2 = right2(i + 1, renvs.back());
      BT thT = einsum("kofb,fbuj->ujko", ref(l2), ref(r2));
      BT U = truncated_right_vectors(thT.d[0] * thT.d[1], thT.d[2] * thT.d[3], thT, d0, d1, terr_);
      BT Ut = U; Ut.rank = 3; Ut.d[0] = U.d[0]; Ut.d[1] = l2.d[0]; Ut.d[2] = l2.d[1];
      lenvs.push_back(einsum("kofb,tko->tfb", ref(l2), ref(Ut), nullptr, true));
      release(thT); release(l2); release(r2); release(U);
      release(renvs.back()); renvs.pop_back();
    }
    double diff = 0.0;
    for (int i = N - 2; i > 0; --i) {
      BT l2 = left2(i, lenvs.back()), r2 = right2(i + 1, renvs.back());
      BT th = einsum("kofb,fbuj->kouj", ref(l2), ref(r2));
      BT V = truncated_right_vectors(th.d[0] * th.d[1], th.d[2] * th.d[3], th, d0, d1, terr_);
      BT Vt = V; Vt.rank = 3; Vt.d[0] = V.d[0]; Vt.d[1] = r2.d[2]; Vt.d[2] = r2.d[3];
      if (track && i == 1) {
        BT us = einsum("kouj,tuj->tko", ref(th), ref(Vt), nullptr, true);
        const int t = us.d[0], nc = us.d[1] * us.d[2];
        std::vector<double> h;
        row_norms2(us, t, nc, h);
        release(us);
        for (auto &x : h) x = std::sqrt(x);
        if (s_last_t == t) {
          for (int w = 0; w < W_; ++w) {
            double d = 0.0;
            for (int q = 0; q < t; ++q) d += std::fabs(h[(size_t)w * t + q] - s_last[(size_t)w * t + q]);
            diff = std::max(diff, d / h[(size_t)w * t]);
          }
        } else {
          diff = std::numeric_limits<double>::infinity();
        }
        s_last = h; s_last_t = t;
      }
      release(res[(size_t)i + 1]);
      res[(size_t)i + 1] = Vt;
      renvs.push_back(einsum("fbuj,tuj->bft", ref(r2), ref(Vt), nullptr, true));
      release(th); release(l2); release(r2);
      release(lenvs.back()); lenvs.pop_back();
    }
    return diff;
  };
  auto finish_two_site = [&](bool keep_renv) {
    BT l2 = left2(0, lenvs.back()), r2 = right2(1, renvs.back());
    BT th = einsum("kofb,fbuj->kouj", ref(l2), ref(r2));
    BT V = truncated_right_vectors(th.d[0] * th.d[1], th.d[2] * th.d[3], th, dmin_, dmax_, terr_);
    BT Vt = V; Vt.rank = 3; Vt.d[0] = V.d[0]; Vt.d[1] = r2.d[2]; Vt.d[2] = r2.d[3];
    release(res[0]); release(res[1]);
    res[0] = einsum("kouj,tuj->kot", ref(th), ref(Vt), nullptr, true);
    res[1] = Vt;
    if (keep_renv) renvs.push_back(einsum("fbuj,tuj->bft", ref(r2), ref(Vt), nullptr, true));
    release(th); release(l2); release(r2);
  };
  if (!one_site) {
    for (int it = 0; it < var_iter_; ++it) {
      const double diff = sweep_two_site(dmin_, dmax_, true);
      if (it > 0 && diff < var_tol_) break;
    }
    finish_two_site(false);
  } else {
    sweep_two_site(dmax_, dmax_, false);
    finish_two_site(true);
    double last = 0.0;
    for (int it = 0; it < var_iter_; ++it) {
      for (int i = 0; i < N - 1; ++i) {
        BT l2 = left2(i, lenvs.back());
        BT aT = einsum("kofb,bft->tko", ref(l2), ref(renvs.back()));
        const int t = aT.d[0], nc = aT.d[1] * aT.d[2];
        BT Q = truncated_right_vectors(t, nc, aT, std::min(t, nc), std::min(t, nc), 0.0);
        BT Qt = Q; Qt.rank = 3; Qt.d[0] = Q.d[0]; Qt.d[1] = l2.d[0]; Qt.d[2] = l2.d[1];
        lenvs.push_back(einsum("kofb,tko->tfb", ref(l2), ref(Qt), nullptr, true));
        release(aT); release(l2); release(Q);
        release(renvs.back()); renvs.pop_back();
      }
      double r_norm = 0.0;
      for (int i = N - 1; i > 0; --i) {
        BT r2 = right2(i, renvs.back());
        BT a = einsum("fbuj,kfb->kuj", ref(r2), ref(lenvs.back()));
        const int k = a.d[0], nc = a.d[1] * a.d[2];
        if (i == 1) {
          std::vector<double> h;
          row_norms2(a, k, nc, h);
          for (int w = 0; w < W_; ++w) { double s2 = 0; for (int q = 0; q < k; ++q) s2 += h[(size_t)w * k + q]; r_norm = std::max(r_norm, std::sqrt(s2)); }
        }
        BT Q = truncated_right_vectors(k, nc, a, std::min(k, nc), std::min(k, nc), 0.0);
        BT Qt = Q; Qt.rank = 3; Qt.d[0] = Q.d[0]; Qt.d[1] = r2.d[2]; Qt.d[2] = r2.d[3];
// ... 1731 lines not shown
```

### peps_b200/csrc/engine.h

```cpp
#pragma once
#include <array>
#include <memory>
#include <string>
#include <vector>
#include "linalg.h"
#include "tensor.h"
#include <map>
#include <stdexcept>

namespace peps {

enum Pos { LEFT = 0, DOWN = 1, RIGHT = 2, UP = 3 };
enum Orient { HORIZONTAL = 0, VERTICAL = 1 };
inline int opposite(int p) { return (p + 2) % 4; }

struct TRef {
  Operand op;
  Operand opi;
  int rank = 0;
  int d[6] = {1, 1, 1, 1, 1, 1};
};

struct EngineConfig {
  int rows = 0, cols = 0, phys = 2, D = 0, walkers = 0, device = 0;
// ... 33 lines not shown
  void sweep_full_space(int nsweeps, double *accept_rate_host);
  void sweep_three_site(int nsweeps, double *accept_rate_host);
  void set_updater(int kind) { if (kind < 0 || kind > 2) throw std::invalid_argument("unknown updater"); updater_ = kind; }
  void step_sweep(int nsweeps, double *accept_rate_host) {
    if (updater_ == 1) sweep_full_space(nsweeps, accept_rate_host);
    else if (updater_ == 2) sweep_three_site(nsweeps, accept_rate_host);
    else sweep(nsweeps, accept_rate_host);
  }
  void energy_and_holes(bool calc_holes, double *eloc_host, double *psi_list_host);
  void measure(double *energy, double *e_h, double *e_v, double *e_dr, double *e_ur, double *row_corr);
  long structure_factor_pairs() const { return (long)cols_ * cols_ * (rows_ * (rows_ - 1) / 2); }
  void measure_structure_factor(double *out_host);
  void zero_accumulators();
  void accumulate_ostar();
  void get_accumulators(double *osum_host, double *eosum_host);
  double *osum_device() { return osum_; }
  double *eosum_device() { return eosum_; }
  void sr_reserve(long max_samples);
  void sr_clear() { sr_count_ = 0; }
  void sr_collect(bool on) { sr_on_ = on; }
  long sr_count() const { return sr_count_; }
  void sr_matvec_device(const double *v_dev, double mean_dot_v, double *out_dev);
  void sr_matvec_host(const double *v, double mean_dot_v, double *out);
  void sr_matvec_host_c(const double *v, double mean_re, double mean_im, double *out);
  struct CGParams { int max_iter = 100; double rel_tol = 1e-4, abs_tol = 0.0; int recompute = 20; double ortho = 0.5; };
  struct CGOutcome { int iterations = 0; double residual_norm = 0.0; int reason = 0; long matvecs = 0; };
  typedef int (*AllReduceFn)(void *user, double *device_buf, size_t n);
  CGOutcome sr_natural_gradient(const double *gradient_host, const double *ostar_mean_host, long total_samples,
                                double diag_shift, const CGParams &prm, const double *init_guess_host, AllReduceFn allreduce,
                                void *user, double *x_host);
  void sr_minsr_natural_gradient(long total_samples, double diag_shift, double *x_host, double *energy_mean_host);
  void sr_minsr_tmatrix(double *t_host, double *gdiag_host);
  void set_model_xxz(double jz, double jxy, double h00) {
    if (phys_ != 2) throw std::invalid_argument("spin-1/2 XXZ / J1-J2 models need phys = 2");
    jz_ = jz; jxy_ = jxy; h00_ = h00;
  }
  void set_deflation(double eps) { la_.deflation_eps = eps; touch_all(); }
  void set_chain_deflation(double eps) { chain_eps_ = eps; touch_all(); }
  void set_model_nnn(double jz2, double jxy2) { jz2_ = jz2; jxy2_ = jxy2; }
  void set_model_tfim(double h) {
    if (phys_ != 2) throw std::invalid_argument("the transverse-field Ising model needs phys = 2");
    tfim_ = true; tfim_h_ = h;
  }
  void set_model_kind_xxz() { tfim_ = false; }
  void set_model_term(int kind, int T, const double *diag, const int32_t *target, const double *coef);
  void clear_model_terms();
  void measure_bond_term(int T, const double *diag, const int32_t *target, const double *coef, double *out_h, double *out_v);
  void measure_site_term(int T, const double *diag, const int32_t *target, const double *coef, double *out);
  void set_bond_pin(int s1, int s2, int T, const double *diag, const int32_t *target, const double *coef);
  void set_fermion(const int32_t *phys_par, const int32_t *leg_par);
  void set_complex();
  bool is_complex() const { return complex_; }
  void set_tps_c(const double *re, const double *im);
  void dress_plane(const double *host, double *dst);
  void get_planar(int what, double *re, double *im);
  void set_jastrow(const double *v, const int32_t *density);
  void clear_jastrow() { jastrow_on_ = false; }
  bool fermion() const { return fermion_; }

  int bmps_stack_size(int pos) const { return (int)bmps_[pos].size(); }
  long bmps_tensor(int pos, int k, int i, double *out_host, int dims[3]);
  void probe_trace_row(int row, double *psi_host);
  void get_holes(double *host);
  long holes_stride() const { return hole_stride_; }
  int walkers() const { return W_; }
  int rows() const { return rows_; }
  int cols() const { return cols_; }
  long stat(int which) const;
  const char *backend() const { return be_name(); }
  void bind() const { be_ctx_bind(bectx_); }

  void contractor_init();
  void grow_bmps_step(int pos);
  void grow_full_bmps(int pos);
  void delete_inner_bmps(int pos);
  void generate_bmps_approach(int post) { delete_inner_bmps(post); grow_full_bmps(opposite(post)); }
  void grow_bmps_for_row(int row);
  void grow_bmps_for_col(int col);
  void shift_bmps_window(int pos);
  void init_bten(int pos);
  void grow_full_bten(int pos, int slice, int remain, bool init);
  void grow_bten_step(int post);
  void shift_bten_window(int pos);
  void nn_trace(int ra, int ca, int rb, int cb, int orient, int cfg_site_a, int cfg_site_b, double *psi_out);
  void punch_hole(int r, int c, int orient);
  void one_site_trace(int r, int c, const int32_t *idx, int stride, double *psi_out);
  void tnn_trace_idx(int r, int c, int orient, const int32_t *idx0, const int32_t *idx1, const int32_t *idx2, int stride,
                     double *psi_out);
  void probe_tnn_trace(int r, int c, int orient, const int32_t *cfg3_host, double *psi_host);
  void nn_trace_idx(int ra, int ca, int rb, int cb, int orient, const int32_t *idx_a, const int32_t *idx_b, int stride,
                    double *psi_out);
  void init_bten2(int pos);
  void grow_full_bten2(int pos, int slice1, int remain, bool init);
  void grow_bten2_step(int post, int slice1);
  void shift_bten2_window(int pos, int slice1);
  void nnn_trace(int row1, int col1, int dir, double *psi_out, int orient = HORIZONTAL);
  void sqrt5_trace(int row1, int col1, int dir, int orient, double *psi_out);
  void probe_plaquette_trace(int kind, int row1, int col1, int dir, int orient, double *psi_host);

 private:
  using BMPSv = std::vector<BT>;
  BT alloc(std::initializer_list<int> dims);
  BT ones111();
  void release(BT &t);
  void release(BMPSv &v);
  TRef ref(const BT &t) const;
  TRef site_ref(int site, int cfg_site) const;
  TRef site_ref_idx(int site, const int32_t *idx, int stride) const;
  void energy_and_holes_tfim(bool calc_holes, double *eloc_host, double *psi_list_host);
  void energy_and_holes_tables(bool calc_holes, double *eloc_host, double *psi_list_host);
  void energy_and_holes_fermion(bool calc_holes, double *eloc_host, double *psi_list_host);
  template <class Start, class Visit, class End>
  void line_pass(int orient, int reach, Start &&start, Visit &&visit, End &&end);
  template <class Start, class Step>
  void sweep_lines(int reach, Start &&start, Step &&step);
  template <class Visit>
  void nnn_row_pass(int row, Visit &&visit);
  struct PsiList {
    Engine &e;
    double *host;
    int n = 0;
    PsiList(Engine &e, double *host);
    void record(const double *psi);
    void download();
  };
  template <class Body>
  void with_term_table(int kind, int T, const double *diag, const int32_t *target, const double *coef, Body &&body);
  void refresh_gather();
  void require_boson(const char *what) const {
    if (fermion_) throw std::logic_error(std::string(what) + " is not available in fermion mode");
  }
  bool fermion_ = false, tps_loaded_ = false;
  bool complex_ = false;
  double *imag(const BT &t) const { return t.p + (long)W_ * t.n; }
  size_t sw() const { return (size_t)W_ * (complex_ ? 2 : 1); }
  void ratio_acc(const double *psi_ex, const double *psi, double coef, double *dst) {
    if (complex_) be_ratio_accumulate_c(psi_ex, psi_ex + W_, psi, psi + W_, coef, dst, dst + W_, W_);
    else be_ratio_accumulate(psi_ex, psi, coef, dst, W_);
  }
  void term_acc(int s1, int s2, const double *diag, const double *coefw, const double *psi_ex, const double *psi, double *dst) {
    if (complex_)
      be_term_accumulate_c(cfg_, nsites_, s1, s2, phys_, diag, coefw, psi_ex, psi_ex ? psi_ex + W_ : nullptr, psi, psi + W_, dst, dst + W_, W_);
    else be_term_accumulate(cfg_, nsites_, s1, s2, phys_, diag, coefw, psi_ex, psi, dst, W_);
  }
  void exchange_decide(int s1, int s2, const double *psi_b, const double *jastrow) {
    if (complex_) be_nn_exchange_decide_c(cfg_, nsites_, s1, s2, psi_b, psi_b + W_, amp_, amp_ + W_, mt_, mtidx_, accepted_, W_, jastrow);
    else be_nn_exchange_decide(cfg_, nsites_, s1, s2, psi_b, amp_, mt_, mtidx_, accepted_, W_, jastrow);
  }
  void require_real(const char *what) const {
    if (complex_) throw std::logic_error(std::string(what) + " is not available for complex states");
  }
  struct ChainStep { BT r; int32_t *cnt = nullptr; bool tri = false; };
  template <class Write>
  ChainStep chain_step(int m, int n, Write &&write, const int32_t *rc, int o, int rk, double eps, bool reduce_tall);
  void bond_energy(int s1, int s2, const double *psi_ex, const double *psi, double jz, double jxy, double *target);
  bool jastrow_on_ = false, tables_exchange_only_ = true;
  double *jastrow_v_ = nullptr, *jr_ = nullptr;
  int32_t *dens_d_ = nullptr;
  const double *jastrow_for(int s1, int s2) {
    if (!jastrow_on_) return nullptr;
    be_jastrow_ratio(cfg_, nsites_, s1, s2, dens_d_, jastrow_v_, jr_, W_);
    return jr_;
  }
  mutable int gmode_ = HORIZONTAL;
  void mode_for_bmps(int pos) const { gmode_ = (pos == UP || pos == DOWN) ? HORIZONTAL : VERTICAL; }
  void mode_for_bten(int pos) const { gmode_ = (pos == LEFT || pos == RIGHT) ? HORIZONTAL : VERTICAL; }
  double *gtps_ = nullptr;
  long gtps_total_ = 0;
  std::vector<long> gtps_off_h_;
  int64_t *gtps_off_d_ = nullptr;
  int32_t *gidx_[2] = {nullptr, nullptr};
  int32_t *jw_[2] = {nullptr, nullptr};
  int32_t *phys_par_d_ = nullptr;
  std::vector<int32_t> phys_par_h_;
  std::vector<std::vector<int32_t>> leg_par_h_;
  double *fsign_ = nullptr;
  double *psi_loc_ = nullptr;
  struct TermTable { bool set = false; int T = 0; double *diag = nullptr; int32_t *target = nullptr; double *coef = nullptr; };
  TermTable term_[3];
  double *site_rec_ = nullptr;
  bool rec_sites_ = false;
  TermTable pin_;
  int pin_s1_ = -1, pin_s2_ = -1;
  void upload_table(TermTable &t, int np, int T, const double *diag, const int32_t *target, const double *coef);
  void check_two_site_table(int T, const int32_t *target) const;
  static void free_table(TermTable &t);
  bool tables_on_ = false;
  int32_t *term_ia_ = nullptr, *term_ib_ = nullptr;
  double *term_cw_ = nullptr;
  void nnn_trace_refs(int row1, int col1, int orient, const TRef &t11, const TRef &t21, const TRef &t12, const TRef &t22,
                      double *psi_out);
  struct KHints {
    const int32_t *klo_m = nullptr, *klo_n = nullptr; double work = 1.0;
    const int32_t *m_cnt = nullptr, *n_cnt = nullptr; int m_scale = 0, n_scale = 0;
  };
  const KHints &r_hints(int which, int k, int e, int a, int p, int b);
  BT einsum(const std::string &spec, const TRef &a, const TRef &b, const KHints *h = nullptr, bool conj_b = false);
  void einsum_into(const std::string &spec, const TRef &a, const TRef &b, Operand c, const long *sc = nullptr,
                   double alpha = 1.0, double beta = 0.0, const KHints *h = nullptr, const Operand *c_im = nullptr);
  BMPSv absorb(const BMPSv &mps, const std::vector<int> &sites, int post);
  BMPSv absorb_svd(const BMPSv &mps, const std::vector<int> &sites, int post);
  BMPSv absorb_variational(const BMPSv &mps, const std::vector<int> &sites, int post, bool one_site);
  BMPSv compress_mps(const BMPSv &mps, int dmin, int dmax, double terr);
  template <class Theta>
  BT truncated_right_vectors(int rows, int cols, Theta &&theta, int dmin, int dmax, double terr);
  int scheme_ = 0;
  double var_tol_ = 1e-12;
  int var_iter_ = 10;
  BT bten_step(const BT &bten, const BT &mps1, const TRef &site, const BT &mps2, int post);
  BT bten2_step(const BT &bten2, const BT &mps1, const TRef &site1, const TRef &site2, const BT &mps2, int post);
  void bten2_operands(int post, int slice1, int bten_size, const BT *&mps1, const BT *&mps2, int &site1, int &site2) const;
  const BT &bten2_at_slice(int pos, int logical) const;
  void reverse_dot(const BT &a, const BT &b, double *out);
  std::vector<int> slice_sites(int num, int orient) const;
  const BMPSv &bmps_at_slice(int pos, int logical) const;
  const BT &bten_at_slice(int pos, int logical) const;
  void bten_operands(int post, int slice, int bten_size, const BT *&mps1, const BT *&mps2, int &site) const;
  static std::string site_labels(int post, char pre, char toward, char next, char away);

  BeCtx *bectx_ = nullptr;
  int rows_, cols_, phys_, D_, W_, nsites_;
  int dmin_, dmax_;
  double terr_;
  double jz_ = 1.0, jxy_ = 1.0, h00_ = 0.0, jz2_ = 0.0, jxy2_ = 0.0;
  int updater_ = 0;
  double *bond_rec_ = nullptr;
  int override_site_ = -1;
  const int32_t *override_idx_ = nullptr;
  int override_stride_ = 0;
  TRef tn_site(int site) const {
    return site == override_site_ ? site_ref_idx(site, override_idx_, override_stride_) : site_ref(site, site);
  }
  void ensure_idx_const();
  void upload_flipped_configs();
  void row_corr_hook(int row);
  bool rec_bonds_ = false;
  double *bond_target(int kind, int row, int col);
  bool tfim_ = false;
  double tfim_h_ = 0.0;
  int32_t *idx_const_ = nullptr;
  int32_t *idx_flip_ = nullptr;
  int32_t *fs_target_d_ = nullptr;
  double *fs_coef_d_ = nullptr;
  int32_t *idx_perm_ = nullptr;
  double *psi_alt_ = nullptr;
  int psi_alt_slots_ = 0;
  void ensure_psi_alt(int slots) {
    if (slots <= psi_alt_slots_) return;
    be_sync();
    be_free(psi_alt_);
    psi_alt_ = (double *)be_malloc(sizeof(double) * (size_t)slots * sw());
    psi_alt_slots_ = slots;
  }
  Pool pool_;
  Planner planner_;
  LinalgCtx la_;

  double *tps_ = nullptr;
  long tps_total_ = 0;
  std::vector<long> tps_off_h_;
  std::vector<int> site_size_h_;
  std::vector<std::array<int, 4>> site_dims_h_;
  int32_t *tps_off_d_ = nullptr, *site_size_d_ = nullptr, *hole_off_d_ = nullptr;

  int32_t *cfg_ = nullptr;
  double *amp_ = nullptr;
  uint32_t *mt_ = nullptr;
  int32_t *mtidx_ = nullptr;
  int32_t *accepted_ = nullptr;
  double *eloc_ = nullptr;
  double *psi_tmp_ = nullptr;
  double *psi_row_ = nullptr;
  double *psi_list_d_ = nullptr;
  double *holes_ = nullptr;
  long hole_stride_ = 0;
  std::vector<long> hole_off_h_;
  double *osum_ = nullptr, *eosum_ = nullptr;
  int32_t *kept_ = nullptr;

  double *sr_ostar_ = nullptr;
  int32_t *sr_cfgs_ = nullptr;
  double *sr_delta_ = nullptr;
  double *sr_eloc_ = nullptr;
  void minsr_centred_t(double *tr, double *ti, double *obar, double *gdiag_host);
  int32_t *sr_desc2_ = nullptr;
  void sr_matvec_device_c(const double *v_dev, double mean_re, double mean_im, double *out_dev);
  long sr_cap_ = 0, sr_count_ = 0;
  bool sr_on_ = false;

  std::map<std::array<int, 6>, KHints> hints_;
  std::map<std::array<int, 7>, std::pair<const int32_t *, const int32_t *>> rdot_tabs_;
  std::vector<BMPSv> bmps_[4];
  struct Memo { BMPSv v; long stamp; };
  std::vector<long> stamp_[4];
  std::map<int, Memo> memo_[4];
  std::vector<long> row_mod_, col_mod_;
  long epoch_ = 1, n_memo_hits_ = 0;
  bool memo_on_ = true;
  bool slices_unchanged_since(int pos, int k, long stamp) const;
  void touch_site(int site);
  void touch_all();
  void purge_memo();
  void park_or_release_top(int pos);
  void push_grown(int pos, int mpo_num, int orient);
  std::vector<BT> bten_[4];
  std::vector<BT> bten2_[4];
  long n_absorb_ = 0, n_bten_ = 0, n_trace_ = 0;
// ... 6 lines not shown
```

### peps_b200/csrc/linalg.h

```cpp
#pragma once
#include <cstdio>
#include <algorithm>
#include <cstdlib>
#include <vector>
#include "tensor.h"

namespace peps {

struct LinalgCtx {
  int W = 0;
  Pool *pool = nullptr;
  Planner *planner = nullptr;
  double *offmax = nullptr;
  int32_t *done = nullptr;
  std::vector<int32_t> done_host;
  long jacobi_sweeps = 0, jacobi_calls = 0, qr_calls = 0;
  long jacobi_rounds = 0;
  long rows_in = 0, rows_kept = 0;
  double deflation_eps = 1e-13;
  bool presort_columns = true;
  bool qr_early_stop = true;
  bool z2_sectors = false;
  int qr_stop_stride = 3;
  bool small_svd = true;
  long small_svd_calls = 0;
  double jacobi_tol = 1e-14;
  int jacobi_inner_sweeps = 1;
  int jacobi_max_sweeps = 40;
};

constexpr size_t kPanelSmemBudget = 150 * 1024;
constexpr size_t kJacobiSmemBudget = 168 * 1024;

struct QRLayout { int nb = 0, rb = 0, nrb = 0, m_pad = 0; };
inline int qr_max_rows() {
  const char *e = std::getenv("PEPS_QR_MAX_ROWS");
  const int v = e ? std::atoi(e) : 8192;
  return (v < 64 || v > 8192) ? 8192 : v;
}

inline int round_up(int x, int m) { return (x + m - 1) / m * m; }

inline int qr_pref_rb() {
  static int v = -1;
  if (v < 0) {
    const char *e = std::getenv("PEPS_QR_RB");
    v = e ? std::atoi(e) : 256;
    if (v < 32 || v % 32 != 0) v = 256;
  }
  return v;
}

inline QRLayout qr_layout(int m, int n) {
  (void)n;
  QRLayout L;
  const int nb = 32;
  const int rbmax = (int)(kPanelSmemBudget / (sizeof(double) * nb)) / nb * nb;
  int rb0 = std::min(std::min(rbmax, round_up(m, nb)), std::max(nb, qr_pref_rb() / nb * nb));
  int nrb = (m + rb0 - 1) / rb0;
  const int nrb_max = rbmax / nb;
  if (nrb > nrb_max) nrb = nrb_max;
  int rb = round_up((m + nrb - 1) / nrb, nb);
  if (rb > rbmax) throw std::runtime_error("qr_layout: matrix too tall for a two-stage CAQR (needs a deeper tree)");
  L.nb = nb; L.rb = rb; L.nrb = (m + rb - 1) / rb; L.m_pad = L.nrb * rb;
  return L;
}

inline GettDesc make_desc(Planner &pl, const std::vector<int32_t> &am, const std::vector<int32_t> &ak,
                          const std::vector<int32_t> &bk, const std::vector<int32_t> &bn,
                          const std::vector<int32_t> &cm, const std::vector<int32_t> &cn, int a_kfast, int b_nfast) {
  GettDesc d;
  d.M = (int)am.size(); d.K = (int)ak.size(); d.N = (int)bn.size();
  d.am = pl.upload(am); d.ak = pl.upload(ak); d.bk = pl.upload(bk); d.bn = pl.upload(bn);
  d.cm = pl.upload(cm); d.cn = pl.upload(cn);
  d.a_kfast = a_kfast; d.b_nfast = b_nfast;
  return d;
}

inline std::vector<int32_t> iota_scaled(int n, int scale, int base = 0) {
  std::vector<int32_t> v((size_t)n);
  for (int i = 0; i < n; ++i) v[(size_t)i] = base + i * scale;
  return v;
}

struct QRStop {
  const double *colnorm2 = nullptr;
  const int32_t *colorder = nullptr;
  double eps = 0.0;
  int first_col = 0;
};

inline void caqr(LinalgCtx &cx, double *A, long ws, int m, int n, const QRLayout &L, const int32_t *row_cnt = nullptr,
                 int row_scale = 0, const QRStop *stop = nullptr) {
  const int W = cx.W, nb = L.nb, rb = L.rb, nrb = L.nrb, lda = n;
  const int kk = std::min(m, n);
  ++cx.qr_calls;
  if (m <= 1) return;
  Planner &pl = *cx.planner;
  double *Vw = (double *)cx.pool->get(sizeof(double) * (size_t)W * nrb * rb * nb);
  double *Tw = (double *)cx.pool->get(sizeof(double) * (size_t)W * nrb * nb * nb);
  std::vector<int32_t> rowtab1((size_t)nrb * rb);
  for (int b = 0; b < nrb; ++b)
    for (int s = 0; s < rb; ++s) rowtab1[(size_t)b * rb + s] = b * rb + s;
  const int32_t *rowtab1_d = pl.upload(rowtab1);
  TileMap tmap;
  const bool have_tmap = (rb % 64 == 0) && nb == 32 && be_make_tile_map(&tmap, A, ws, lda, L.m_pad, n, W, rb / 8, 8);
  TileMap tmapc;
  const bool have_tmapc = rb <= 256 && rb % 16 == 0 && nb == 32 && be_make_tile_map(&tmapc, A, ws, lda, L.m_pad, n, W, rb, 8);
  const int npanel = (kk + nb - 1) / nb;
  const bool stopping = stop && stop->eps > 0.0 && cx.qr_early_stop && npanel > 2;
  int32_t *stopped = nullptr;
  double *stop_acc = nullptr;
  if (stopping) {
    stopped = (int32_t *)cx.pool->get(sizeof(int32_t) * (size_t)W);
    stop_acc = (double *)cx.pool->get(sizeof(double) * (size_t)W);
    be_memset0(stopped, sizeof(int32_t) * (size_t)W);
    be_memset0(stop_acc, sizeof(double) * (size_t)W);
  }
  for (int p = 0; p < npanel; ++p) {
    const int col0 = p * nb, pw = std::min(nb, kk - col0), c1 = col0 + pw, ntrail = n - c1;
    const int b0 = col0 / rb, nact = nrb - b0;
    PanelArgs pa;
    pa.A = A; pa.ws = ws; pa.lda = lda; pa.rowtab = rowtab1_d + (size_t)b0 * rb; pa.R = rb; pa.skip0 = col0 - b0 * rb; pa.NI = nact;
    pa.col0 = col0; pa.pw = pw; pa.nbw = nb; pa.Vw = Vw; pa.Tw = Tw; pa.W = W;
    pa.row_cnt = row_cnt; pa.row_scale = row_scale;
    pa.stopped = stopped;
    be_panel_qr(pa);
    if (ntrail > 0) {
      ApplyArgs ap;
      ap.A = A; ap.ws = ws; ap.lda = lda; ap.rowtab = pa.rowtab; ap.R = rb; ap.NI = nact; ap.col1 = c1; ap.ntrail = ntrail;
      ap.nbw = nb; ap.Vw = Vw; ap.Tw = Tw; ap.W = W;
      if (have_tmap) { ap.tmap = &tmap; ap.row0 = b0 * rb; }
      if (have_tmapc) { ap.tmap_cols = &tmapc; ap.row0 = b0 * rb; }
      ap.row_cnt = row_cnt; ap.row_scale = row_scale; ap.stopped = stopped;
      be_apply_reflector(ap);
    }
    if (nact > 1) {
      const int R2 = nact * pw;
      std::vector<int32_t> rowtab2((size_t)R2);
      for (int b = 0; b < nact; ++b)
        for (int i = 0; i < pw; ++i) rowtab2[(size_t)b * pw + i] = (b0 + b) * rb + (b == 0 ? pa.skip0 : 0) + i;
      PanelArgs p2 = pa;
      p2.rowtab = pl.upload(rowtab2); p2.R = R2; p2.skip0 = 0; p2.NI = 1; p2.row_cnt = nullptr;
      be_panel_qr(p2);
      if (ntrail > 0) {
        ApplyArgs ap;
        ap.A = A; ap.ws = ws; ap.lda = lda; ap.rowtab = p2.rowtab; ap.R = R2; ap.NI = 1; ap.col1 = c1; ap.ntrail = ntrail;
        ap.nbw = nb; ap.Vw = Vw; ap.Tw = Tw; ap.W = W; ap.stopped = stopped;
        be_apply_reflector(ap);
      }
    }
    if (stopping && ntrail > 0 && c1 < m && c1 >= stop->first_col && p + 1 < npanel && (p % cx.qr_stop_stride) == cx.qr_stop_stride - 1)
      be_trailing_check(A, ws, lda, c1, m, c1, n, stop->colnorm2, stop->colorder, n, 0.01 * stop->eps * stop->eps, stop_acc, stopped, W);
  }
  if (stopping) { cx.pool->put(stopped); cx.pool->put(stop_acc); }
  cx.pool->put(Vw);
  cx.pool->put(Tw);
}

struct JacobiLayout { int bs = 0, nblk = 0, nr_pad = 0; };

inline int jacobi_max_bs() {
  static int v = -1;
  if (v < 0) {
    const char *e = std::getenv("PEPS_JACOBI_BS");
    v = e ? std::atoi(e) : 16;
    if (v != 4 && v != 8 && v != 16) v = 16;
  }
  return v;
}

inline JacobiLayout jacobi_layout(int nr, int nc) {
  JacobiLayout J;
  int ncp = round_up(nc, 8);
  for (int bs : {16, 8, 4}) {
    if (bs > jacobi_max_bs()) continue;
    size_t bytes = (size_t)2 * bs * (ncp + 4) * sizeof(double);
    if (bytes > kJacobiSmemBudget && bs != 4) continue;
    if (bytes > kJacobiSmemBudget) throw std::runtime_error("jacobi_layout: rows too long for the shared-memory panel");
    if (bs > 4 && nr <= bs) continue;
    J.bs = bs;
    break;
  }
  int nblk = (nr + J.bs - 1) / J.bs;
  if (nblk < 2) nblk = 2;
  if (nblk & 1) ++nblk;
  J.nblk = nblk; J.nr_pad = nblk * J.bs;
  return J;
}

inline int truncate_buffer_rows(int nr, int nc) {
  return nr > 1 ? std::max(nr, qr_layout(nr, nc).m_pad) : nr;
}

inline void truncate_rows(LinalgCtx &cx, double *G, long ws, int nr, int nc, int dmin, int dmax, double trunc_err,
                          int tcap, double *B, long wb, int32_t *kept) {
  const int W = cx.W;
  const int nsv = std::min(nr, nc);
  const bool presort = cx.presort_columns && nr > 1 && nc > 1;
  double *Gin = G;
  int32_t *cord = nullptr;
  if (presort) {
    const int brows = truncate_buffer_rows(nr, nc);
    double *cn2 = (double *)cx.pool->get(sizeof(double) * (size_t)W * nc);
    int32_t *ccnt = (int32_t *)cx.pool->get(sizeof(int32_t) * (size_t)W);
    cord = (int32_t *)cx.pool->get(sizeof(int32_t) * (size_t)W * nc);
    be_col_norms2(G, ws, nc, nr, nc, cn2, W);
    be_rank_rows(cn2, nc, 0.0, cord, ccnt, W);
    G = (double *)cx.pool->get(sizeof(double) * (size_t)W * brows * nc);
    if (brows > nr) be_memset0(G, sizeof(double) * (size_t)W * brows * nc);
    be_permute_cols(Gin, ws, nc, nr, nc, cord, 1, G, (long)brows * nc, nc, W);
    ws = (long)brows * nc;
    cx.pool->put(ccnt);
    QRStop st;
    st.colnorm2 = cn2; st.colorder = cord; st.eps = cx.deflation_eps; st.first_col = std::max(0, std::min(dmax, nsv) - 32);
    if (nr > 1) caqr(cx, G, ws, nr, nc, qr_layout(nr, nc), nullptr, 0, &st);
    cx.pool->put(cn2);
  } else if (nr > 1) {
    caqr(cx, G, ws, nr, nc, qr_layout(nr, nc));
  }
  const int kk = nsv;
  double *n2a = (double *)cx.pool->get(sizeof(double) * (size_t)W * kk);
  int32_t *ord = (int32_t *)cx.pool->get(sizeof(int32_t) * (size_t)W * kk);
  int32_t *cnt = (int32_t *)cx.pool->get(sizeof(int32_t) * (size_t)W);
  be_row_norms2(G, ws, nc, kk, nc, n2a, W);
  be_rank_rows(n2a, kk, cx.deflation_eps * cx.deflation_eps, ord, cnt, W);
  cx.done_host.resize((size_t)W);
  be_d2h(cx.done_host.data(), cnt, sizeof(int32_t) * W);
  int nr_eff = 1;
  for (int w = 0; w < W; ++w) nr_eff = std::max(nr_eff, (int)cx.done_host[(size_t)w]);
  cx.rows_in += kk; cx.rows_kept += nr_eff;
  if (cx.small_svd && nr_eff >= 2 && round_up(nr_eff, 8) <= kSmallSvdMaxN && round_up(nc, 32) <= (int)(kPanelSmemBudget / (sizeof(double) * 32)) / 32 * 32) {
    ++cx.jacobi_calls; ++cx.small_svd_calls;
    const int n2 = round_up(nr_eff, 8), nb = 32;
    const int rb = round_up(nc, 32), kk2 = std::min(nc, n2), npanel = (kk2 + nb - 1) / nb;
    const long wsT = (long)rb * n2, wsC = (long)rb * tcap;
    double *GT = (double *)cx.pool->get(sizeof(double) * (size_t)W * wsT);
    be_memset0(GT, sizeof(double) * (size_t)W * wsT);
    be_gather_rows_transposed(G, ws, nc, nc, kk, ord, cnt, GT, wsT, n2, W);
    double *Vall = (double *)cx.pool->get(sizeof(double) * (size_t)npanel * W * rb * nb);
    double *Tall = (double *)cx.pool->get(sizeof(double) * (size_t)npanel * W * nb * nb);
    const int32_t *rowtab = cx.planner->upload(iota_scaled(rb, 1));
    TileMap tmT, tmC;
    const bool mapT = (rb % 64 == 0) && be_make_tile_map(&tmT, GT, wsT, n2, rb, n2, W, rb / 8, 8);
    for (int p = 0; p < npanel; ++p) {
      const int col0 = p * nb, pw = std::min(nb, kk2 - col0), c1 = col0 + pw, ntrail = n2 - c1;
      PanelArgs pa;
      pa.A = GT; pa.ws = wsT; pa.lda = n2; pa.rowtab = rowtab; pa.R = rb; pa.skip0 = col0; pa.NI = 1;
      pa.col0 = col0; pa.pw = pw; pa.nbw = nb; pa.Vw = Vall + (size_t)p * W * rb * nb; pa.Tw = Tall + (size_t)p * W * nb * nb; pa.W = W;
      be_panel_qr(pa);
      if (ntrail > 0) {
        ApplyArgs ap;
        ap.A = GT; ap.ws = wsT; ap.lda = n2; ap.rowtab = rowtab; ap.R = rb; ap.NI = 1; ap.col1 = c1; ap.ntrail = ntrail;
        ap.nbw = nb; ap.Vw = pa.Vw; ap.Tw = pa.Tw; ap.W = W;
        if (mapT) { ap.tmap = &tmT; ap.row0 = 0; }
        be_apply_reflector(ap);
      }
    }
    double *C0 = (double *)cx.pool->get(sizeof(double) * (size_t)W * wsC);
    be_memset0(C0, sizeof(double) * (size_t)W * wsC);
    SmallSvdArgs sa;
    sa.Rt = GT; sa.ws = wsT; sa.ld = n2; sa.n2 = n2; sa.count = cnt; sa.nsv = nsv; sa.dmin = dmin; sa.dmax = dmax;
    sa.trunc_err = trunc_err; sa.tcap = tcap; sa.tol = cx.jacobi_tol; sa.max_sweeps = cx.jacobi_max_sweeps;
    sa.out = C0; sa.wo = wsC; sa.kept = kept; sa.sweeps = nullptr; sa.W = W;
    be_svd_small(sa);
    const bool mapC = (rb % 64 == 0) && be_make_tile_map(&tmC, C0, wsC, tcap, rb, tcap, W, rb / 8, 8);
    for (int p = npanel - 1; p >= 0; --p) {
      ApplyArgs ap;
      ap.A = C0; ap.ws = wsC; ap.lda = tcap; ap.rowtab = rowtab; ap.R = rb; ap.NI = 1; ap.col1 = 0; ap.ntrail = tcap;
      ap.nbw = nb; ap.Vw = Vall + (size_t)p * W * rb * nb; ap.Tw = Tall + (size_t)p * W * nb * nb; ap.W = W; ap.notrans = 1;
      if (mapC) { ap.tmap = &tmC; ap.row0 = 0; }
      be_apply_reflector(ap);
    }
    be_transpose_permute(C0, wsC, nc, tcap, presort ? cord : nullptr, B, wb, W);
    for (void *p : {(void *)GT, (void *)Vall, (void *)Tall, (void *)C0, (void *)n2a, (void *)ord, (void *)cnt}) cx.pool->put(p);
    if (presort) { cx.pool->put(cord); cx.pool->put(G); }
    return;
  }
  JacobiLayout J = jacobi_layout(nr_eff, nc);
  double *G2 = (double *)cx.pool->get(sizeof(double) * (size_t)W * J.nr_pad * nc);
  const long ws2 = (long)J.nr_pad * nc;
  be_gather_rows(G, ws, nc, nc, kk, ord, cnt, G2, ws2, J.nr_pad, W);
  long ws2cur = ws2;
  int32_t *bsec = nullptr, *cwin = nullptr, *cord2 = nullptr;
  const bool sectors = cx.z2_sectors && nr_eff > 2 * J.bs;
  if (sectors) {
    JacobiLayout Jz = J;
    Jz.nblk = (nr_eff + J.bs - 1) / J.bs + 1;
    if (Jz.nblk & 1) ++Jz.nblk;
    Jz.nr_pad = Jz.nblk * J.bs;
    double *Gz = (double *)cx.pool->get(sizeof(double) * (size_t)W * Jz.nr_pad * nc);
    be_memset0(Gz, sizeof(double) * (size_t)W * Jz.nr_pad * nc);
    bsec = (int32_t *)cx.pool->get(sizeof(int32_t) * (size_t)W * Jz.nblk);
    cwin = (int32_t *)cx.pool->get(sizeof(int32_t) * (size_t)W * 4);
    cord2 = (int32_t *)cx.pool->get(sizeof(int32_t) * (size_t)W * nc);
    be_sector_arrange(G2, ws2, nc, nc, cnt, J.bs, Jz.nblk, Gz, (long)Jz.nr_pad * nc, bsec, presort ? cord : nullptr, cord2, cwin, W);
    cx.pool->put(G2);
    G2 = Gz; J = Jz; ws2cur = (long)Jz.nr_pad * nc; nr_eff = Jz.nr_pad;
  }
  if (nr_eff > 1) {
    ++cx.jacobi_calls;
    be_fill(cx.offmax, 0.0, W);
    be_memset0(cx.done, sizeof(int32_t) * W);
    JacobiArgs ja;
    ja.G = G2; ja.ws = ws2cur; ja.ld = nc; ja.nr_pad = J.nr_pad; ja.nc = nc; ja.bs = J.bs; ja.nblk = J.nblk;
    ja.tol = cx.jacobi_tol; ja.inner_sweeps = cx.jacobi_inner_sweeps; ja.offmax = cx.offmax; ja.done = cx.done; ja.W = W;
    ja.nactive = W;
    ja.bsec = bsec; ja.cwin = cwin;
    for (int sweep = 0; sweep < cx.jacobi_max_sweeps; ++sweep) {
      for (int round = 0; round < ja.nblk - 1; ++round) {
        ja.round = round;
        be_jacobi_round(ja);
      }
      ++cx.jacobi_sweeps;
      cx.jacobi_rounds += ja.nblk - 1;
      be_jacobi_flags(cx.offmax, cx.done, ja.tol, W);
      be_d2h(cx.done_host.data(), cx.done, sizeof(int32_t) * W);
      int nact = 0;
      for (int w = 0; w < W; ++w) nact += cx.done_host[(size_t)w] ? 0 : 1;
      ja.nactive = nact;
      if (nact == 0 && ja.bsec) {
        ja.bsec = nullptr;
        ja.tol = std::max(cx.jacobi_tol, 1e-11);
        be_memset0(cx.done, sizeof(int32_t) * W);
        ja.nactive = W;
        continue;
      }
      if (nact == 0) break;
      if (!sectors && nr_eff > 2 * ja.bs && sweep + 1 < cx.jacobi_max_sweeps) {
        be_row_norms2(G2, ws2cur, nc, nr_eff, nc, n2a, W);
        be_rank_rows(n2a, nr_eff, cx.deflation_eps * cx.deflation_eps, ord, cnt, W);
        std::vector<int32_t> ch((size_t)W);
        be_d2h(ch.data(), cnt, sizeof(int32_t) * W);
        int ne = 1;
        for (int w = 0; w < W; ++w) ne = std::max(ne, (int)ch[(size_t)w]);
        JacobiLayout Jn = jacobi_layout(ne, nc);
        if (Jn.bs == ja.bs && Jn.nblk + 2 <= ja.nblk) {
          double *G3 = (double *)cx.pool->get(sizeof(double) * (size_t)W * Jn.nr_pad * nc);
          be_gather_rows(G2, ws2cur, nc, nc, nr_eff, ord, cnt, G3, (long)Jn.nr_pad * nc, Jn.nr_pad, W);
          cx.pool->put(G2);
          G2 = G3; ws2cur = (long)Jn.nr_pad * nc; nr_eff = ne;
          ja.G = G2; ja.ws = ws2cur; ja.nr_pad = Jn.nr_pad; ja.nblk = Jn.nblk;
        }
      }
    }
  }
  double *n2b = (double *)cx.pool->get(sizeof(double) * (size_t)W * nr_eff);
  int32_t *ord2 = (int32_t *)cx.pool->get(sizeof(int32_t) * (size_t)W * tcap);
  be_row_norms2(G2, ws2cur, nc, nr_eff, nc, n2b, W);
  be_select_truncate(n2b, nr_eff, nsv, dmin, dmax, trunc_err, tcap, ord2, kept, W);
  if (presort || cord2) {
    double *Bp = (double *)cx.pool->get(sizeof(double) * (size_t)W * tcap * nc);
    be_gather_rows_normalized(G2, ws2cur, nc, nc, n2b, nr_eff, ord2, kept, tcap, Bp, (long)tcap * nc, W);
    be_permute_cols(Bp, (long)tcap * nc, nc, tcap, nc, cord2 ? cord2 : cord, 0, B, wb, nc, W);
    cx.pool->put(Bp);
    if (presort) { cx.pool->put(cord); cx.pool->put(G); }
  } else {
    be_gather_rows_normalized(G2, ws2cur, nc, nc, n2b, nr_eff, ord2, kept, tcap, B, wb, W);
  }
  for (void *p : {(void *)n2a, (void *)ord, (void *)cnt, (void *)G2, (void *)n2b, (void *)ord2}) cx.pool->put(p);
  if (bsec) { cx.pool->put(bsec); cx.pool->put(cwin); cx.pool->put(cord2); }
}

}
```

Baseline: 29.63.

## Fuse QR early-stop trailing norm into apply-reflector and panel kernels

The separate trailing-norm and decide kernels that checked for early stopping of the column-pivoted QR are removed. The apply-reflector kernels now write per-block partial squared norms of the updated trailing rows, and the next panel QR kernel reduces them and decides whether to stop. Because the check no longer needs its own launches, it runs after every panel instead of every third panel past a first-column threshold, so stopping can happen earlier. In exchange, every apply and panel kernel does extra FMAs, shared reductions and partial-buffer writes.

```diff
diff --git a/include/peps_b200.h b/include/peps_b200.h
--- a/include/peps_b200.h
+++ b/include/peps_b200.h
@@ -117,6 +117,8 @@
 void *peps_stream(peps_ctx *ctx);
 
 int peps_test_qr_r(int32_t device, int32_t W, int32_t m, int32_t n, const double *a, double *r_out);
+int peps_test_qr_stop(int32_t device, int32_t W, int32_t m, int32_t n, double eps, const double *a, double *r_out,
+                      int32_t *stop_col_out);
 int peps_test_truncate(int32_t device, int32_t W, int32_t nr, int32_t nc, int32_t dmin, int32_t dmax, double trunc_err,
                        const double *theta, double *b_out, int32_t *kept_out, int32_t *sweeps_out);
 int peps_test_einsum(int32_t device, int32_t W, const char *spec, const int32_t *dims_a, int32_t rank_a,
diff --git a/peps_b200/_lib.py b/peps_b200/_lib.py
--- a/peps_b200/_lib.py
+++ b/peps_b200/_lib.py
@@ -98,6 +98,7 @@
     "peps_profile_get": (C.c_int, [_P, _D, C.POINTER(C.c_int64), _D, C.c_int32]),
     "peps_stream": (C.c_void_p, [_P]),
     "peps_test_qr_r": (C.c_int, [C.c_int32, C.c_int32, C.c_int32, C.c_int32, _D, _D]),
+    "peps_test_qr_stop": (C.c_int, [C.c_int32, C.c_int32, C.c_int32, C.c_int32, C.c_double, _D, _D, _I]),
     "peps_test_truncate": (C.c_int, [C.c_int32, C.c_int32, C.c_int32, C.c_int32, C.c_int32, C.c_int32, C.c_double,
                                      _D, _D, _I, _I]),
     "peps_test_einsum": (C.c_int, [C.c_int32, C.c_int32, C.c_char_p, _I, C.c_int32, _I, C.c_int32, _D, _D, _D]),
diff --git a/peps_b200/csrc/backend.h b/peps_b200/csrc/backend.h
--- a/peps_b200/csrc/backend.h
+++ b/peps_b200/csrc/backend.h
@@ -58,6 +58,15 @@
 void be_copy2d(double *dst, long wd, long ldd, const double *src, long ws, long lds, int rows, int cols, int W);
 void be_set_identity(double *dst, long wd, int rows, int cols, int W);
 
+struct QRStopTest {
+  const double *part = nullptr;
+  int ld = 0, nslot = 0;
+  const double *colnorm2 = nullptr;
+  const int32_t *colorder = nullptr;
+  int n = 0;
+  double thresh2 = 0.0;
+  int32_t *stop_col = nullptr;
+};
 struct PanelArgs {
   double *A; long ws; int lda;
   const int32_t *rowtab; int R; int skip0; int NI;
@@ -66,11 +75,10 @@
   int W;
   const int32_t *row_cnt = nullptr;
   int row_scale = 0;
-  const int32_t *stopped = nullptr;
+  int32_t *stopped = nullptr;
+  QRStopTest stop;
 };
 void be_panel_qr(const PanelArgs &a);
-void be_trailing_check(const double *A, long ws, int lda, int row0, int nrows, int col0, int ncols, const double *colnorm2,
-                       const int32_t *colorder, int n, double thresh2, double *acc, int32_t *stopped, int W);
 
 struct TileMap { alignas(64) unsigned char blob[128]; };
 bool be_make_tile_map(TileMap *tm, const double *A, long ws, int lda, int rows, int cols, int W, int box_rows, int box_cols);
@@ -87,6 +95,8 @@
   const int32_t *row_cnt = nullptr;
   int row_scale = 0;
   const int32_t *stopped = nullptr;
+  double *norm_part = nullptr;
+  int norm_ld = 0, norm_off = 0, norm_skip = 0, norm_skip0 = 0;
 };
 void be_apply_reflector(const ApplyArgs &a);
 
diff --git a/peps_b200/csrc/backend_cuda.cu b/peps_b200/csrc/backend_cuda.cu
--- a/peps_b200/csrc/backend_cuda.cu
+++ b/peps_b200/csrc/backend_cuda.cu
@@ -1,5 +1,6 @@
 #include <cuda.h>
 #include <cuda_runtime.h>
+#include <climits>
 #include <cstdint>
 #include <cstdio>
 #include <cstdlib>
@@ -676,11 +677,34 @@
 
 constexpr int PQR_THREADS = 256;
 
+__device__ bool panel_stop_test(const PanelArgs &a, int it, int w) {
+  __shared__ double red[PQR_THREADS / 32];
+  __shared__ int was;
+  const QRStopTest &s = a.stop;
+  if (threadIdx.x == 0) was = a.stopped[w];
+  const double *pp = s.part + (long)w * s.ld;
+  double v = 0.0;
+  for (int i = threadIdx.x; i < s.nslot; i += PQR_THREADS) v += pp[i];
+  v = warp_sum(v);
+  if ((threadIdx.x & 31) == 0) red[threadIdx.x >> 5] = v;
+  __syncthreads();
+  if (was) return true;
+  double tot = 0.0;
+#pragma unroll
+  for (int i = 0; i < PQR_THREADS / 32; ++i) tot += red[i];
+  const bool stop = tot <= s.thresh2 * s.colnorm2[(long)w * s.n + s.colorder[(long)w * s.n]];
+  if (stop && it == 0 && threadIdx.x == 0) {
+    a.stopped[w] = 1;
+    if (s.stop_col) s.stop_col[w] = a.col0;
+  }
+  return stop;
+}
+
 __global__ void __launch_bounds__(PQR_THREADS) panel_qr_kernel(PanelArgs a) {
   extern __shared__ double sm[];
   const int it = blockIdx.x, w = blockIdx.y;
+  if (a.stop.part ? panel_stop_test(a, it, w) : (a.stopped && a.stopped[w])) return;
   if (a.row_cnt && a.rowtab[(long)it * a.R] >= a.row_cnt[w] * a.row_scale) return;
-  if (a.stopped && a.stopped[w]) return;
   const int R = a.R, pw = a.pw, nbw = a.nbw;
   const int skip = (it == 0) ? a.skip0 : 0;
   const int nact = R - skip;
@@ -811,8 +835,8 @@
   constexpr int LDT = NBW + 1, LDSS = NBW + 1;
   constexpr int RP = RPL * 32;
   const int it = blockIdx.x, w = blockIdx.y;
+  if (a.stop.part ? panel_stop_test(a, it, w) : (a.stopped && a.stopped[w])) return;
   if (a.row_cnt && a.rowtab[(long)it * a.R] >= a.row_cnt[w] * a.row_scale) return;
-  if (a.stopped && a.stopped[w]) return;
   const int R = a.R, pw = a.pw, nbw = a.nbw;
   const int skip = (it == 0) ? a.skip0 : 0;
   const int nact = R - skip;
@@ -1121,8 +1145,16 @@
   APPLY_CLK(0);
   constexpr int TN = NBW, MT = NBW / 8, NT = NBW / 8, LDC = TN + 4, LDW = TN + 4, NTILE = MT * NT;
   const int ct = blockIdx.x, it = blockIdx.y, w = blockIdx.z;
-  if (a.row_cnt && a.rowtab[(long)it * a.R] >= a.row_cnt[w] * a.row_scale) return;
   if (a.stopped && a.stopped[w]) return;
+  auto norm_slot = [&](int k) -> double * {
+    const int nchunk = (a.ntrail + 7) / 8, k0 = ct * (NBW / 8);
+    return k < min(NBW / 8, nchunk - k0) ? a.norm_part + (long)w * a.norm_ld + a.norm_off + (long)it * nchunk + k0 + k : nullptr;
+  };
+  if (a.row_cnt && a.rowtab[(long)it * a.R] >= a.row_cnt[w] * a.row_scale) {
+    if (a.norm_part)
+      if (double *slot = norm_slot(threadIdx.x)) *slot = 0.0;
+    return;
+  }
   const int R = a.R, R8 = (R + 7) & ~7, nbw = a.nbw;
   double *Cs = sm;
   auto csi = [&](int r, int c) -> size_t {
@@ -1297,6 +1329,8 @@
   }
 
   APPLY_CLK(4);
+  const int nskip = a.norm_part ? a.norm_skip + (it == 0 ? a.norm_skip0 : 0) : INT_MAX;
+  if (a.norm_part) part[t] = 0.0;
   {
     double bw[NBW / 4][NT];
 #pragma unroll
@@ -1340,7 +1374,29 @@
             if (c + 1 < ncols) dst[c + 1] = acc[j][1];
           }
         }
-      }
+        if (r >= nskip) {
+          double nrm = part[t];
+#pragma unroll
+          for (int j = 0; j < NT; ++j) {
+            const int c = j * 8 + 2 * (lane & 3);
+            if (c < ncols) nrm = fma(acc[j][0], acc[j][0], nrm);
+            if (c + 1 < ncols) nrm = fma(acc[j][1], acc[j][1], nrm);
+          }
+          part[t] = nrm;
+        }
+      }
+    }
+  }
+  if (a.norm_part) {
+    const double nrm = warp_sum(part[t]);
+    if (lane == 0) part[t] = nrm;
+    __syncthreads();
+    if (double *slot = norm_slot(t)) {
+      double s = 0.0;
+      if (t == 0)
+#pragma unroll
+        for (int i = 0; i < 8; ++i) s += part[32 * i];
+      *slot = s;
     }
   }
   APPLY_CLK(5);
@@ -1362,13 +1418,19 @@
   double *Ww = Cw + (size_t)R * 8;
   uint64_t *bars = reinterpret_cast<uint64_t *>(wbase + (size_t)8 * wstride);
   const int cs = blockIdx.x, it = blockIdx.y, w = blockIdx.z;
-  if (a.row_cnt && a.row0 + it * R >= a.row_cnt[w] * a.row_scale) return;
   if (a.stopped && a.stopped[w]) return;
+  const int c_lo = cs * cper, c_hi = min(nchunk, c_lo + cper);
+  double *nslot = a.norm_part ? a.norm_part + (long)w * a.norm_ld + a.norm_off + (long)it * nchunk + c_lo : nullptr;
+  if (a.row_cnt && a.row0 + it * R >= a.row_cnt[w] * a.row_scale) {
+    if (nslot) for (int k = t; k < c_hi - c_lo; k += 256) nslot[k] = 0.0;
+    return;
+  }
+  const int nskip = a.norm_skip + (it == 0 ? a.norm_skip0 : 0);
+  double nrm = 0.0;
   const double *V = a.Vw + ((long)w * a.NI + it) * (long)R * 32;
   const double *Tg = a.Tw + ((long)w * a.NI + it) * 1024L;
   double *Aw = a.A + (long)w * a.ws;
   const int row_base = a.row0 + it * R;
-  const int c_lo = cs * cper, c_hi = min(nchunk, c_lo + cper);
   if (lane == 0) mbar_init(&bars[warp], 1);
   if (t == 0) mbar_init(&bars[8], 1);
   asm volatile("fence.mbarrier_init.release.cluster;\n" ::: "memory");
@@ -1435,6 +1497,10 @@
       if (colok) {
         *reinterpret_cast<double2 *>(Aw + (long)(row_base + r0) * a.lda + gcol) = c0;
         *reinterpret_cast<double2 *>(Aw + (long)(row_base + r1) * a.lda + gcol) = c1;
+        if (nslot) {
+          if (r0 >= nskip) nrm = fma(c0.x, c0.x, fma(c0.y, c0.y, nrm));
+          if (r1 >= nskip) nrm = fma(c1.x, c1.x, fma(c1.y, c1.y, nrm));
+        }
       }
     }
     __syncwarp();
@@ -1442,6 +1508,18 @@
       asm volatile("fence.proxy.async.shared::cta;\n" ::: "memory");
       mbar_expect_tx(&bars[warp], (unsigned)(R * 64));
       tma_load_3d(Cw, &tm, a.col1 + 8 * (chunk + 8), row_base, w, &bars[warp]);
+    }
+  }
+  if (nslot) {
+    nrm = warp_sum(nrm);
+    if (lane == 0) Ww[0] = nrm;
+    __syncthreads();
+    for (int k = t; k < c_hi - c_lo; k += 256) {
+      double s = 0.0;
+      if (k == 0)
+#pragma unroll
+        for (int i = 0; i < 8; ++i) s += wbase[(size_t)i * wstride + (size_t)R * 8];
+      nslot[k] = s;
     }
   }
 }
@@ -1518,47 +1596,6 @@
             h[6] - h[0], h[7] - h[6], h[1] - h[7], h[2] - h[1], h[3] - h[2], h[4] - h[3], h[5] - h[4]);
   }
 #endif
-}
-
-__global__ void trailing_norm_kernel(const double *A, long ws, int lda, int row0, int nrows, int col0, int ncols, double *acc,
-                                     const int32_t *stopped) {
-  const int w = blockIdx.y;
-  if (stopped[w]) return;
-  const double *Aw = A + (long)w * ws;
-  const int lane = threadIdx.x & 31, warp = threadIdx.x >> 5, nwarp = blockDim.x >> 5;
-  double s0 = 0.0, s1 = 0.0;
-  for (int r = row0 + blockIdx.x * nwarp + warp; r < nrows; r += gridDim.x * nwarp) {
-    const double *x = Aw + (long)r * lda;
-    int c = col0 + lane;
-    for (; c + 32 < ncols; c += 64) { const double a = x[c], b = x[c + 32]; s0 = fma(a, a, s0); s1 = fma(b, b, s1); }
-    if (c < ncols) { const double a = x[c]; s0 = fma(a, a, s0); }
-  }
-  double s = warp_sum(s0 + s1);
-  __shared__ double red[8];
-  if (lane == 0) red[warp] = s;
-  __syncthreads();
-  if (threadIdx.x == 0) {
-    double t = 0.0;
-    for (int i = 0; i < nwarp; ++i) t += red[i];
-    if (t != 0.0) atomicAdd(acc + w, t);
-  }
-}
-__global__ void trailing_decide_kernel(const double *colnorm2, const int32_t *colorder, int n, double thresh2, double *acc,
-                                       int32_t *stopped, int W) {
-  const int w = blockIdx.x * blockDim.x + threadIdx.x;
-  if (w >= W || stopped[w]) return;
-  stopped[w] = (acc[w] <= thresh2 * colnorm2[(long)w * n + colorder[(long)w * n]]) ? 1 : 0;
-  acc[w] = 0.0;
-}
-void be_trailing_check(const double *A, long ws, int lda, int row0, int nrows, int col0, int ncols, const double *colnorm2,
-                       const int32_t *colorder, int n, double thresh2, double *acc, int32_t *stopped, int W) {
-  if (nrows <= row0 || ncols <= col0) return;
-  LaunchScope scope(KC_SMALL, 0.0);
-  const int bx = std::max(1, std::min(16, (nrows - row0 + 63) / 64));
-  trailing_norm_kernel<<<dim3(bx, W), 256, 0, g_stream>>>(A, ws, lda, row0, nrows, col0, ncols, acc, stopped);
-  ++cx().launches;
-  trailing_decide_kernel<<<(W + 127) / 128, 128, 0, g_stream>>>(colnorm2, colorder, n, thresh2, acc, stopped, W);
-  post_launch();
 }
 
 constexpr int JAC_THREADS = 256;
diff --git a/peps_b200/csrc/c_api.cpp b/peps_b200/csrc/c_api.cpp
--- a/peps_b200/csrc/c_api.cpp
+++ b/peps_b200/csrc/c_api.cpp
@@ -258,6 +258,39 @@
     double *R = (double *)pool.get(sizeof(double) * (size_t)W * kk * n);
     be_copy2d(R, (long)kk * n, n, A, (long)L.m_pad * n, n, kk, n, W);
     be_d2h(r_out, R, sizeof(double) * (size_t)W * kk * n);
+  })
+}
+
+int peps_test_qr_stop(int32_t device, int32_t W, int32_t m, int32_t n, double eps, const double *a, double *r_out,
+                      int32_t *stop_col_out) {
+  peps_ctx *nullctx = nullptr;
+  GUARD(nullctx, {
+    be_init(device);
+    Pool pool; Planner planner; LinalgCtx cx;
+    cx.W = W; cx.pool = &pool; cx.planner = &planner;
+    QRLayout L = qr_layout(m, n);
+    const long ws = (long)L.m_pad * n;
+    double *tmp = (double *)pool.get(sizeof(double) * (size_t)W * m * n);
+    be_h2d(tmp, a, sizeof(double) * (size_t)W * m * n);
+    double *cn2 = (double *)pool.get(sizeof(double) * (size_t)W * n);
+    int32_t *cord = (int32_t *)pool.get(sizeof(int32_t) * (size_t)W * n);
+    int32_t *ccnt = (int32_t *)pool.get(sizeof(int32_t) * (size_t)W);
+    be_col_norms2(tmp, (long)m * n, n, m, n, cn2, W);
+    be_rank_rows(cn2, n, 0.0, cord, ccnt, W);
+    double *A = (double *)pool.get(sizeof(double) * (size_t)W * ws);
+    be_memset0(A, sizeof(double) * (size_t)W * ws);
+    be_permute_cols(tmp, (long)m * n, n, m, n, cord, 1, A, ws, n, W);
+    std::vector<int32_t> none((size_t)W, -1);
+    int32_t *scol = (int32_t *)pool.get(sizeof(int32_t) * (size_t)W);
+    be_h2d(scol, none.data(), sizeof(int32_t) * (size_t)W);
+    QRStop st;
+    st.colnorm2 = cn2; st.colorder = cord; st.eps = eps; st.stop_col = scol;
+    caqr(cx, A, ws, m, n, L, nullptr, 0, &st);
+    int kk = std::min(m, n);
+    double *R = (double *)pool.get(sizeof(double) * (size_t)W * kk * n);
+    be_copy2d(R, (long)kk * n, n, A, ws, n, kk, n, W);
+    be_d2h(r_out, R, sizeof(double) * (size_t)W * kk * n);
+    be_d2h(stop_col_out, scol, sizeof(int32_t) * (size_t)W);
   })
 }
 
diff --git a/peps_b200/csrc/engine.cpp b/peps_b200/csrc/engine.cpp
--- a/peps_b200/csrc/engine.cpp
+++ b/peps_b200/csrc/engine.cpp
@@ -26,7 +26,6 @@
   if (const char *e = std::getenv("PEPS_CHAIN_EPS")) chain_eps_ = std::atof(e);
   if (const char *e = std::getenv("PEPS_SMALL_SVD")) la_.small_svd = std::atoi(e) != 0;
   if (const char *e = std::getenv("PEPS_QR_EARLY_STOP")) la_.qr_early_stop = std::atoi(e) != 0;
-  if (const char *e = std::getenv("PEPS_QR_STOP_STRIDE")) la_.qr_stop_stride = std::max(1, std::atoi(e));
   la_.offmax = (double *)be_malloc(sizeof(double) * W_);
   la_.done = (int32_t *)be_malloc(sizeof(int32_t) * W_);
   tps_off_h_.resize((size_t)nsites_);
@@ -344,7 +343,7 @@
   return absorb_svd(mps, sites_in, post);
 }
 template <class Write>
-Engine::ChainStep Engine::chain_step(int m_in, int n_in, Write &&write, const int32_t *rc, int o, int rk, double eps,
+Engine::ChainStep Engine::chain_step(int m_in, int n_in, Write &&write, const int32_t *rc, int o, double eps,
                                      bool reduce_tall) {
   ChainStep out;
   int m = complex_ ? 2 * m_in : m_in;
@@ -370,7 +369,7 @@
     A = padded();
     be_embed_complex(Ar, Ai, wa, m_in, n_in, A, wsA, W_);
     pool_.put(Ar); pool_.put(Ai);
-    rc = nullptr; o = 0; rk *= 2;
+    rc = nullptr; o = 0;
   }
   auto reduce = [&](double *&Ap) {
     if (!reduce_tall) return;
@@ -418,7 +417,7 @@
     pool_.put(A);
     reduce(Ap);
     QRStop st;
-    st.colnorm2 = cn2; st.colorder = cord; st.eps = eps; st.first_col = std::max(0, std::min(rk, kk) - 96);
+    st.colnorm2 = cn2; st.colorder = cord; st.eps = eps;
     caqr(la_, Ap, wsA, m, n, L, rc, o, &st);
     be_row_norms2(Ap, wsA, n, kk, n, cn2, W_);
     be_rank_rows(cn2, kk, eps * eps, ord, cnt, W_);
@@ -532,7 +531,7 @@
     ChainStep cs = chain_step(k * o, f * b, [&](Operand c, const Operand *c_im) {
       einsum_into("kepb," + sl + "->kofb", ref(tmp1), sref, c, nullptr, 1.0, 0.0, (tri || rc) ? &h2 : nullptr, c_im);
       release(tmp1);
-    }, rc, o, rk, chain_eps_, true);
+    }, rc, o, chain_eps_, true);
     BT &rn = r[(size_t)i + 1] = cs.r;
     rn.rank = 3; rn.d[1] = f; rn.d[2] = b;
     r_cnt[(size_t)i + 1] = cs.cnt;
@@ -585,7 +584,7 @@
   for (int i = 0; i < N - 1; ++i) {
     r[(size_t)i + 1] = chain_step(r[(size_t)i].d[0] * mps[(size_t)i].d[1], mps[(size_t)i].d[2], [&](Operand c, const Operand *c_im) {
       einsum_into("ka,apb->kpb", ref(r[(size_t)i]), ref(mps[(size_t)i]), c, nullptr, 1.0, 0.0, nullptr, c_im);
-    }, nullptr, 0, 0, 0.0, false).r;
+    }, nullptr, 0, 0.0, false).r;
   }
   BMPSv res((size_t)N);
   BT E = alloc({1, 1});
diff --git a/peps_b200/csrc/engine.h b/peps_b200/csrc/engine.h
--- a/peps_b200/csrc/engine.h
+++ b/peps_b200/csrc/engine.h
@@ -209,7 +209,7 @@
   }
   struct ChainStep { BT r; int32_t *cnt = nullptr; bool tri = false; };
   template <class Write>
-  ChainStep chain_step(int m, int n, Write &&write, const int32_t *rc, int o, int rk, double eps, bool reduce_tall);
+  ChainStep chain_step(int m, int n, Write &&write, const int32_t *rc, int o, double eps, bool reduce_tall);
   void bond_energy(int s1, int s2, const double *psi_ex, const double *psi, double jz, double jxy, double *target);
   bool jastrow_on_ = false, tables_exchange_only_ = true;
   double *jastrow_v_ = nullptr, *jr_ = nullptr;
diff --git a/peps_b200/csrc/linalg.h b/peps_b200/csrc/linalg.h
--- a/peps_b200/csrc/linalg.h
+++ b/peps_b200/csrc/linalg.h
@@ -21,7 +21,6 @@
   bool presort_columns = true;
   bool qr_early_stop = true;
   bool z2_sectors = false;
-  int qr_stop_stride = 3;
   bool small_svd = true;
   long small_svd_calls = 0;
   double jacobi_tol = 1e-14;
@@ -87,7 +86,7 @@
   const double *colnorm2 = nullptr;
   const int32_t *colorder = nullptr;
   double eps = 0.0;
-  int first_col = 0;
+  int32_t *stop_col = nullptr;
 };
 
 inline void caqr(LinalgCtx &cx, double *A, long ws, int m, int n, const QRLayout &L, const int32_t *row_cnt = nullptr,
@@ -110,13 +109,18 @@
   const int npanel = (kk + nb - 1) / nb;
   const bool stopping = stop && stop->eps > 0.0 && cx.qr_early_stop && npanel > 2;
   int32_t *stopped = nullptr;
-  double *stop_acc = nullptr;
+  double *part = nullptr;
+  const int part_ld = (nrb + 1) * ((n + 7) / 8);
+  QRStopTest test;
   if (stopping) {
     stopped = (int32_t *)cx.pool->get(sizeof(int32_t) * (size_t)W);
-    stop_acc = (double *)cx.pool->get(sizeof(double) * (size_t)W);
+    part = (double *)cx.pool->get(sizeof(double) * (size_t)W * part_ld);
     be_memset0(stopped, sizeof(int32_t) * (size_t)W);
-    be_memset0(stop_acc, sizeof(double) * (size_t)W);
-  }
+    test.part = part; test.ld = part_ld;
+    test.colnorm2 = stop->colnorm2; test.colorder = stop->colorder; test.n = n; test.thresh2 = 0.01 * stop->eps * stop->eps;
+    test.stop_col = stop->stop_col;
+  }
+  int nslot = 0;
   for (int p = 0; p < npanel; ++p) {
     const int col0 = p * nb, pw = std::min(nb, kk - col0), c1 = col0 + pw, ntrail = n - c1;
     const int b0 = col0 / rb, nact = nrb - b0;
@@ -125,7 +129,10 @@
     pa.col0 = col0; pa.pw = pw; pa.nbw = nb; pa.Vw = Vw; pa.Tw = Tw; pa.W = W;
     pa.row_cnt = row_cnt; pa.row_scale = row_scale;
     pa.stopped = stopped;
+    if (nslot > 0) { pa.stop = test; pa.stop.nslot = nslot; }
     be_panel_qr(pa);
+    const bool tested = stopping && ntrail > 0 && c1 < m && p + 1 < npanel;
+    nslot = 0;
     if (ntrail > 0) {
       ApplyArgs ap;
       ap.A = A; ap.ws = ws; ap.lda = lda; ap.rowtab = pa.rowtab; ap.R = rb; ap.NI = nact; ap.col1 = c1; ap.ntrail = ntrail;
@@ -133,7 +140,9 @@
       if (have_tmap) { ap.tmap = &tmap; ap.row0 = b0 * rb; }
       if (have_tmapc) { ap.tmap_cols = &tmapc; ap.row0 = b0 * rb; }
       ap.row_cnt = row_cnt; ap.row_scale = row_scale; ap.stopped = stopped;
+      if (tested) { ap.norm_part = part; ap.norm_ld = part_ld; ap.norm_skip = pw; ap.norm_skip0 = pa.skip0; }
       be_apply_reflector(ap);
+      if (tested) nslot = nact * ((ntrail + 7) / 8);
     }
     if (nact > 1) {
       const int R2 = nact * pw;
@@ -141,19 +150,19 @@
       for (int b = 0; b < nact; ++b)
         for (int i = 0; i < pw; ++i) rowtab2[(size_t)b * pw + i] = (b0 + b) * rb + (b == 0 ? pa.skip0 : 0) + i;
       PanelArgs p2 = pa;
-      p2.rowtab = pl.upload(rowtab2); p2.R = R2; p2.skip0 = 0; p2.NI = 1; p2.row_cnt = nullptr;
+      p2.rowtab = pl.upload(rowtab2); p2.R = R2; p2.skip0 = 0; p2.NI = 1; p2.row_cnt = nullptr; p2.stop = QRStopTest();
       be_panel_qr(p2);
       if (ntrail > 0) {
         ApplyArgs ap;
         ap.A = A; ap.ws = ws; ap.lda = lda; ap.rowtab = p2.rowtab; ap.R = R2; ap.NI = 1; ap.col1 = c1; ap.ntrail = ntrail;
         ap.nbw = nb; ap.Vw = Vw; ap.Tw = Tw; ap.W = W; ap.stopped = stopped;
+        if (tested) { ap.norm_part = part; ap.norm_ld = part_ld; ap.norm_off = nslot; ap.norm_skip = pw; }
         be_apply_reflector(ap);
-      }
-    }
-    if (stopping && ntrail > 0 && c1 < m && c1 >= stop->first_col && p + 1 < npanel && (p % cx.qr_stop_stride) == cx.qr_stop_stride - 1)
-      be_trailing_check(A, ws, lda, c1, m, c1, n, stop->colnorm2, stop->colorder, n, 0.01 * stop->eps * stop->eps, stop_acc, stopped, W);
-  }
-  if (stopping) { cx.pool->put(stopped); cx.pool->put(stop_acc); }
+        if (tested) nslot += (ntrail + 7) / 8;
+      }
+    }
+  }
+  if (stopping) { cx.pool->put(stopped); cx.pool->put(part); }
   cx.pool->put(Vw);
   cx.pool->put(Tw);
 }
@@ -213,7 +222,7 @@
     ws = (long)brows * nc;
     cx.pool->put(ccnt);
     QRStop st;
-    st.colnorm2 = cn2; st.colorder = cord; st.eps = cx.deflation_eps; st.first_col = std::max(0, std::min(dmax, nsv) - 32);
+    st.colnorm2 = cn2; st.colorder = cord; st.eps = cx.deflation_eps;
     if (nr > 1) caqr(cx, G, ws, nr, nc, qr_layout(nr, nc), nullptr, 0, &st);
     cx.pool->put(cn2);
   } else if (nr > 1) {
```

After: 29.93 (median of 6 runs). No clear change (+1.0%).
